# fasion-image-generator-project/discogan_modernized

Measured on AMD Instinct MI355X. Metric: images/sec per DiscoGAN train step, higher is better.
Workload: dtype f32x3; 1 GPU; tops2hanbok discogan image_size=512 batch_size=32 per GPU (BASELINE configs[3]); D,G,G cycle, fwd+bwd+Adam, dead backward work skipped; fp32-accurate conv products on the bf16 matrix path: every fp32 operand carried as three bf16 planes (24 significand bits), exact bf16 x bf16 products, fp32 accumulation (no operand rounding); image_size=512, global_batch=32, parallelism=dp1, hipgraph=True, hip_streams=2, allreduce_overlap=False

## Files before the change

discogan_modernized_amd/_lib.py:

```python
from __future__ import annotations

import ctypes as C
import os

_HERE = os.path.dirname(os.path.abspath(__file__))
LIB_PATH = os.environ.get("DG_LIB") or os.path.join(_HERE, "libdiscogan_hip.so")

_p = C.c_void_p
_i = C.c_int
_f = C.c_float
_d = C.c_double
_z = C.c_size_t
_l = C.c_int64

SIGNATURES = {
    "dg_version": (_i, []),
    "dg_build_flags": (_i, []),
    "dg_last_error": (C.c_char_p, []),
    "dg_set_option": (_i, [C.c_char_p, _i]),
    "dg_conv_workspace_bytes": (_z, [_i, _i, _i, _i, _i, _i, _i, _i]),
    "dg_conv_fwd": (_i, [_p, _p, _p, _i, _i, _i, _i, _i, _i, _i, _p, _z, _p]),
    "dg_conv_dgrad": (_i, [_p, _p, _p, _i, _i, _i, _i, _i, _i, _i, _p, _z, _p]),
    "dg_conv_wgrad": (_i, [_p, _p, _p, _i, _i, _i, _i, _i, _i, _i, _i, _p, _z, _p]),
    "dg_conv_workspace_bytes_p": (_z, [_i, _i, _i, _i, _i, _i, _i, _i, _i, _i]),
    "dg_conv_bnstats_rows_p": (_i, [_i, _i, _i, _i, _i, _i, _i, _i, _i]),
    "dg_conv_plan_splits_p": (_i, [_i, _i, _i, _i, _i, _i, _i, _i, _i, _i]),
    "dg_conv_plan_describe": (_i, [_i, _i, _i, _i, _i, _i, _i, _i, _i, _i, _i, _i, C.POINTER(_i), _i]),
    "dg_conv_fwd_g": (_i, [_i, _p, _p, _p, _i, _i, _i, _i, _i, _i, _i, _i, _i, _p, _z, _p, _z, _p]),
    "dg_conv_dgrad_g": (_i, [_i, _p, _p, _p, _i, _i, _i, _i, _i, _i, _i, _i, _i, _p, _z, _p, _z, _p]),
    "dg_conv_wgrad_g": (_i, [_i, _i, _p, _p, _p, _i, _i, _i, _i, _i, _i, _i, _i, _i, _i, _p, _z, _p]),
    "dg_conv4x4s2_c3_fwd_p": (_i, [_p, _p, _p, _i, _i, _i, _i, _i, _i, _f, _i, _p]),
    "dg_conv4x4s2_c3_dgrad_p": (_i, [_p, _i, _p, _p, _i, _i, _i, _i, _i, _i, _p, _z, _p]),
    "dg_c3_dgrad_act_ok": (_i, [_i, _i, _i, _i, _i]),
    "dg_conv4x4s2_c3_dgrad_act_p": (_i, [_p, _i, _p, _i, _f, _p, _p, _i, _i, _i, _i, _i, _i, _p, _z, _p]),
    "dg_conv4x4s2_c3_wgrad_p": (_i, [_p, _p, _i, _i, _f, _p, _p, _i, _i, _i, _i, _i, _i, _p, _z, _p]),
    "dg_c3_dgrad_bn_ok": (_i, [_i, _i, _i, _i, _i]),
    "dg_conv4x4s2_c3_dgrad_bn_p": (_i, [_p, _p, _p, _p, _i, _p, _p, _i, _i, _i, _i, _i, _i, _p]),
    "dg_c3_wgrad_bn_ok": (_i, [_i, _i, _i, _i, _i]),
    "dg_conv4x4s2_c3_wgrad_bn_p": (_i, [_p, _p, _p, _p, _i, _p, _p, _i, _i, _i, _i, _i, _i, _p, _z, _p]),
    "dg_conv4x4s2_c3_fwd_g": (_i, [_i, _p, _p, _p, _i, _i, _i, _i, _i, _f, _i, _p]),
    "dg_conv4x4s2_c3_dgrad_g": (_i, [_i, _p, _p, _p, _i, _i, _i, _i, _i, _i, _p]),
    "dg_conv4x4s2_c3_wgrad_g": (_i, [_i, _i, _p, _p, _i, _f, _p, _p, _i, _i, _i, _i, _i, _i, _p, _z, _p]),
    "dg_bn_train_stats_g": (_i, [_i, _i, _p, _i, _i, _f, _f, _p, _p, _p, _p, _p, _z, _p]),
    "dg_bn_act_fwd_g": (_i, [_i, _p, _p, _i, _i, _p, _p, _p, _i, _f, _p]),
    "dg_bn_act_bwd_g": (_i, [_i, _i, _p, _p, _p, _i, _i, _p, _p, _p, _i, _f, _p, _p, _i, _p, _z, _p]),
    "dg_act_fwd_g": (_i, [_i, _p, _p, _z, _i, _f, _p]),
    "dg_act_bwd_g": (_i, [_i, _p, _p, _p, _z, _i, _f, _p]),
    "dg_mse_fwd_g": (_i, [_i, _p, _p, _z, _p, _p, _z, _p]),
    "dg_mse_bwd_g": (_i, [_i, _p, _p, _z, _p, _p, _p]),
    "dg_bce_fwd_g": (_i, [_i, _p, _i, _p, _p, _p]),
    "dg_bce_bwd_g": (_i, [_i, _p, _i, _p, _p, _p, _p]),
    "dg_fm_fwd_g": (_i, [_i, _p, _p, _i, _z, _p, _p, _p, _z, _p]),
    "dg_fm_bwd_g": (_i, [_i, _p, _i, _z, _p, _p, _p, _p]),
    "dg_conv_fwd_bias_act": (_i, [_p, _p, _p, _p, _i, _i, _i, _i, _i, _i, _i, _i, _f, _p, _z, _p]),
    "dg_conv_dgrad_bias_act": (_i, [_p, _p, _p, _p, _i, _i, _i, _i, _i, _i, _i, _i, _f, _p, _z, _p]),
    "dg_conv_plan_splits": (_i, [_i, _i, _i, _i, _i, _i, _i, _i]),
    "dg_conv_bnstats_rows": (_i, [_i, _i, _i, _i, _i, _i, _i, _i]),
    "dg_conv_fwd_bnstats": (_i, [_p, _p, _p, _i, _i, _i, _i, _i, _p, _z, _p, _z, _p]),
    "dg_conv_dgrad_bnstats": (_i, [_p, _p, _p, _i, _i, _i, _i, _i, _p, _z, _p, _z, _p]),
    "dg_conv4x4s2_fwd": (_i, [_p, _p, _p, _i, _i, _i, _i, _i, _p, _z, _p]),
    "dg_conv4x4s2_dgrad": (_i, [_p, _p, _p, _i, _i, _i, _i, _i, _p, _z, _p]),
    "dg_conv4x4s2_wgrad": (_i, [_p, _p, _p, _i, _i, _i, _i, _i, _i, _p, _z, _p]),
    "dg_conv4x4_valid_fwd": (_i, [_p, _p, _p, _i, _i, _i, _p, _z, _p]),
    "dg_conv4x4_valid_dgrad": (_i, [_p, _p, _p, _i, _i, _i, _p, _z, _p]),
    "dg_conv4x4_valid_wgrad": (_i, [_p, _p, _p, _i, _i, _i, _i, _p, _z, _p]),
    "dg_convT4x4s2_fwd": (_i, [_p, _p, _p, _i, _i, _i, _i, _i, _p, _z, _p]),
    "dg_convT4x4s2_dgrad": (_i, [_p, _p, _p, _i, _i, _i, _i, _i, _p, _z, _p]),
    "dg_convT4x4s2_wgrad": (_i, [_p, _p, _p, _i, _i, _i, _i, _i, _i, _p, _z, _p]),
    "dg_convT4x4_1to4_fwd": (_i, [_p, _p, _p, _i, _i, _i, _p, _z, _p]),
    "dg_convT4x4_1to4_dgrad": (_i, [_p, _p, _p, _i, _i, _i, _p, _z, _p]),
    "dg_convT4x4_1to4_wgrad": (_i, [_p, _p, _p, _i, _i, _i, _i, _p, _z, _p]),
    "dg_conv4x4s2_c3_fwd": (_i, [_p, _p, _p, _i, _i, _i, _i, _i, _f, _p]),
    "dg_c3_dgrad_workspace_bytes": (_z, [_i]),
    "dg_conv4x4s2_c3_dgrad": (_i, [_p, _p, _p, _i, _i, _i, _i, _i, _p, _z, _p]),
    "dg_c3_wgrad_workspace_bytes": (_z, [_i, _i, _i, _i]),
    "dg_conv4x4s2_c3_wgrad": (_i, [_p, _p, _p, _i, _i, _i, _i, _i, _p, _z, _p]),
    "dg_conv4x4s2_c3_wgrad_act": (_i, [_p, _p, _i, _f, _p, _p, _i, _i, _i, _i, _i, _p, _z, _p]),
    "dg_bn_workspace_bytes": (_z, [_i, _i]),
    "dg_bn_train_stats": (_i, [_p, _i, _i, _f, _f, _p, _p, _p, _p, _p, _z, _p]),
    "dg_bn_partials_workspace_bytes": (_z, [_i, _i]),
    "dg_bn_stats_from_partials": (_i, [_p, _i, _i, _i, _f, _f, _p, _p, _p, _p, _p, _z, _p]),
    "dg_bn_act_fwd": (_i, [_p, _p, _i, _i, _p, _p, _p, _i, _f, _p]),
    "dg_bn_act_bwd": (_i, [_p, _p, _p, _i, _i, _p, _p, _p, _i, _f, _p, _p, _i, _p, _z, _p]),
    "dg_act_fwd": (_i, [_p, _p, _z, _i, _f, _p]),
    "dg_act_bwd": (_i, [_p, _p, _p, _z, _i, _f, _p]),
    "dg_loss_workspace_bytes": (_z, []),
    "dg_mse_fwd": (_i, [_p, _p, _z, _p, _p, _z, _p]),
    "dg_mse_bwd": (_i, [_p, _p, _z, _p, _p, _p]),
    "dg_bce_fwd": (_i, [_p, _i, _f, _p, _p, _z, _p]),
    "dg_bce_bwd": (_i, [_p, _i, _f, _p, _p, _p]),
    "dg_fm_workspace_bytes": (_z, [_i, _z]),
    "dg_fm_fwd": (_i, [_p, _p, _i, _z, _p, _p, _p, _z, _p]),
    "dg_fm_bwd": (_i, [_p, _i, _z, _p, _p, _p, _p]),
    "dg_debug_igemm_stamps": (_i, [_p, _z]),
    "dg_device_cu_count": (_i, []),
    "dg_loss_mix_fwd": (_i, [_p, _p, _i, _f, _i, _p]),
    "dg_loss_mix_bwd": (_i, [_p, _p, _i, _f, _i, _i, _p]),
    "dg_adam_advance": (_i, [_p, _d, _d, _d, _p]),
    "dg_adam_step_flat": (_i, [_p, _p, _p, _p, _z, _p, _f, _f, _f, _f, _f, _p]),
    "dg_ema_update_flat": (_i, [_p, _p, _z, _f, _p]),
    "dg_swap_flat": (_i, [_p, _p, _z, _p]),
    "dg_grad_stats_workspace_bytes": (_z, []),
    "dg_grad_sumsq_partial": (_i, [_p, _z, _p, _z, _i, C.POINTER(_i), _p]),
    "dg_grad_clip_finalize": (_i, [_p, _i, _d, _d, _i, _p, _p]),
    "dg_adam_advance_c": (_i, [_p, _d, _d, _d, _p, _p]),
    "dg_adam_step_flat_c": (_i, [_p, _p, _p, _p, _z, _p, _f, _f, _f, _f, _p, _p, _i, _z, _p]),
    "dg_bce_target_fwd": (_i, [_p, _p, _i, _p, _p]),
    "dg_bce_target_bwd": (_i, [_p, _p, _i, _p, _p, _p]),
    "dg_hinge_fwd": (_i, [_p, _p, _z, _f, _p, _p, _z, _p]),
    "dg_hinge_bwd": (_i, [_p, _p, _z, _f, _p, _p, _p]),
    "dg_dp_ready": (_i, [_p]),
    "dg_dp_unique_id_bytes": (_i, []),
    "dg_dp_get_unique_id": (_i, [_p, _z]),
    "dg_dp_init": (_i, [_i, _i, _p, _z]),
    "dg_dp_world_size": (_i, []),
    "dg_dp_rank": (_i, []),
    "dg_dp_allreduce_sum": (_i, [_p, _z, _p]),
    "dg_dp_allreduce_max": (_i, [_p, _z, _p]),
    "dg_dp_broadcast": (_i, [_p, _z, _i, _p]),
    "dg_dp_barrier": (_i, [_p, _p]),
    "dg_dp_destroy": (_i, []),
    "dg_u8hwc_to_f32chw": (_i, [_p, _p, _i, _i, _i, _i, _p]),
    "dg_image_prep": (_i, [_p, _p, _i, _i, _i, _i, _i, _i, _i, _i, _p]),
    "dg_sample_grid_u8": (_i, [_p, _i, _i, _i, _i, _i, _p, _p]),
    "dg_image_metrics_workspace_bytes": (_z, [_i, _i]),
    "dg_image_metrics": (_i, [_p, _p, _i, _i, _p, _p, _z, _p]),
    "dg_adam_step_flat_bf16": (_i, [_p, _p, _p, _p, _z, _p, _f, _f, _f, _f, _f, _p, _p]),
    "dg_f32_to_bf16": (_i, [_p, _p, _z, _p]),
    "dg_bn_act_fwd_bf16": (_i, [_p, _p, _p, _i, _i, _p, _p, _p, _i, _f, _p]),
    "dg_bn_act_bwd_bf16": (_i, [_p, _p, _p, _p, _i, _i, _p, _p, _p, _i, _f, _p, _p, _i, _p, _z, _p]),
    "dg_conv_bf16_operands_ok": (_i, [_i, _i, _i, _i, _i, _i, _i, _i]),
    "dg_f32_to_bf16x3": (_i, [_p, _p, _z, _z, _p]),
    "dg_adam_step_flat_x3": (_i, [_p, _p, _p, _p, _z, _p, _f, _f, _f, _f, _f, _p, _z, _p]),
    "dg_conv4x4s2_c3_fwd_x3": (_i, [_p, _p, _p, _p, _z, _i, _i, _i, _i, _i, _f, _p]),
    "dg_conv_x3_planes_ok": (_i, [_i, _i, _i, _i, _i, _i, _i, _i]),
    "dg_bn_act_fwd_x3": (_i, [_p, _p, _p, _z, _i, _i, _i, _p, _p, _p, _i, _f, _p]),
    "dg_bn_act_bwd_x3": (_i, [_p, _p, _p, _p, _z, _i, _i, _i, _p, _p, _p, _i, _f, _p, _p, _i, _p, _z, _p]),
    "dg_conv_x3_bnstats_rows": (_i, [_i, _i, _i, _i, _i, _i, _i, _i]),
    "dg_conv_fwd_x3": (_i, [_p, _l, _p, _l, _i, _p, _i, _i, _i, _i, _i, _i, _i, _p, _z, _p, _z, _p]),
    "dg_x3_transpose_planes": (_i, [_p, _p, _z, _p, _p, _p, _i, _p]),
    "dg_conv_dgrad_x3": (_i, [_p, _l, _i, _p, _l, _p, _i, _i, _i, _i, _i, _i, _i, _p, _z, _p, _z, _p]),
    "dg_conv_wgrad_x3": (_i, [_p, _l, _i, _p, _l, _p, _i, _i, _i, _i, _i, _i, _i, _i, _p, _z, _p]),
    "dg_conv_mixed_bnstats_rows": (_i, [_i, _i, _i, _i, _i, _i, _i, _i, _i, _i]),
    "dg_conv_fwd_mixed": (_i, [_p, _i, _p, _i, _p, _i, _i, _i, _i, _i, _i, _i, _i, _p, _z, _p, _z, _p]),
    "dg_conv_dgrad_mixed": (_i, [_p, _i, _p, _i, _p, _i, _i, _i, _i, _i, _i, _i, _i, _p, _z, _p, _z, _p]),
    "dg_bn_train_stats_t": (_i, [_p, _i, _i, _i, _f, _f, _p, _p, _p, _p, _p, _z, _p]),
    "dg_bn_act_fwd_t": (_i, [_p, _p, _i, _i, _i, _p, _p, _p, _i, _f, _p]),
    "dg_bn_act_bwd_t": (_i, [_p, _p, _p, _i, _i, _i, _p, _p, _p, _i, _f, _p, _p, _i, _p, _z, _p]),
    "dg_act_bwd_t": (_i, [_p, _p, _p, _i, _z, _i, _f, _p]),
    "dg_conv4x4s2_c3_fwd_t": (_i, [_p, _p, _p, _i, _i, _i, _i, _i, _i, _f, _p]),
    "dg_conv4x4s2_c3_dgrad_t": (_i, [_p, _i, _p, _p, _i, _i, _i, _i, _i, _p, _z, _p]),
    "dg_conv4x4s2_c3_wgrad_t": (_i, [_p, _p, _i, _i, _f, _p, _p, _i, _i, _i, _i, _i, _p, _z, _p]),
    "dg_fm_fwd_t": (_i, [_p, _p, _i, _i, _z, _p, _p, _p, _z, _p]),
    "dg_fm_bwd_t": (_i, [_p, _i, _z, _p, _p, _p, _i, _p]),
    "dg_conv_wgrad_mixed": (_i, [_p, _i, _p, _i, _p, _i, _i, _i, _i, _i, _i, _i, _i, _p, _z, _p]),
    "dg_nchw_to_nhwc": (_i, [_p, _p, _i, _i, _i, _i, _p]),
    "dg_nhwc_to_nchw": (_i, [_p, _p, _i, _i, _i, _i, _p]),
}

_lib = None


class DiscoganHipError(RuntimeError):
    pass


def load():
    global _lib
    if _lib is not None:
        return _lib
    if not os.path.exists(LIB_PATH):
        raise DiscoganHipError(
            f"{LIB_PATH} not found: the HIP kernel library is not built. "
            "Run `python -m discogan_modernized_amd.build` (hipcc --offload-arch=gfx950). "
            "There is no CPU fallback for the product path.")
    import torch
    lib = C.CDLL(LIB_PATH)
    for name, (res, args) in SIGNATURES.items():
        fn = getattr(lib, name)
        fn.restype = res
        fn.argtypes = args
    _lib = lib
    for key, val in os.environ.items():
        if key.startswith("DG_OPT_"):
            rc = lib.dg_set_option(key[7:].lower().encode(), int(val))
            if rc != 0:
                raise DiscoganHipError(f"bad option {key}: " + lib.dg_last_error().decode())
    return lib


def check(rc, what=""):
    if rc != 0:
        msg = load().dg_last_error().decode("utf-8", "replace")
        raise DiscoganHipError(f"{what} failed (code {rc}): {msg}")


def set_option(name: str, value: int):
    check(load().dg_set_option(name.encode(), int(value)), "dg_set_option")
```

discogan_modernized_amd/csrc/igemm_dma_x3.hip:

```cpp
#include "igemm_args.h"
#include <type_traits>
#include <utility>

typedef __bf16 bf16x8 __attribute__((ext_vector_type(8)));
typedef __bf16 bf16x4 __attribute__((ext_vector_type(4)));
typedef __attribute__((address_space(3))) bf16x4* lds_bf4_ptr;
typedef __attribute__((address_space(3))) void* lds_void_ptr;

template <int... Q, typename F>
__device__ __forceinline__ void dg_x3_static_for(std::integer_sequence<int, Q...>, F&& f) {
    (f(std::integral_constant<int, Q>{}), ...);
}
#define DG_X3T_MAX 48
constexpr int G16_I[24] = {0, 0, 0, 1, 1, 1, 2, 2, 2, 3, 3, 3, 4, 4, 4, 5, 5, 5, 6, 7, 6, 6, 7, 7};
constexpr int G16_T[24] = {0, 1, 2, 0, 1, 2, 0, 1, 2, 0, 1, 2, 0, 1, 2, 0, 1, 2, 0, 0, 1, 2, 1, 2};

template <int MODE, bool BT, int WM, int WN, int NS, bool M16 = false>
__global__ __launch_bounds__(64 * WM * WN, 2) void igemm_dma_x3_kernel(const IgemmArgs p) {
    static_assert(MODE == MODE_FWD || MODE == MODE_DGRAD_S2 || MODE == MODE_WGRAD, "modes with an LDS-DMA form");
    static_assert(!BT || MODE == MODE_FWD, "the transposed weight copy serves the forward form");
    constexpr int NW = WM * WN, FM = 4, FN = 2;
    constexpr int BM = 32 * FM * WM, BN = 32 * FN * WN, KT = 16;
    static_assert((BM == 256 || BM == 128) && (BN == 256 || BN == 128), "tile");
    constexpr bool A_KM = MODE == MODE_WGRAD;
    constexpr bool B_KM = MODE != MODE_FWD || BT;
    constexpr int PLA = BM * KT * 2, PLB = BN * KT * 2;
    constexpr int OPA = 3 * PLA, STAGE = OPA + 3 * PLB;
    constexpr int NPA = PLA / 1024 / NW, NPB = PLB / 1024 / NW;
    static_assert(NPA * NW * 1024 == PLA && NPB * NW * 1024 == PLB, "pieces must divide over the waves");
    constexpr int NPC = 3 * (NPA + NPB);
    constexpr int LDS_BYTES = NS * STAGE;
    static_assert((NS == 2 || NS == 3) && LDS_BYTES <= 160 * 1024, "LDS");
    static_assert(!M16 || (NS == 3 && WM == 2 && WN == 4), "the 16x16x32 body: 256 x 256 tile, three stages");
    constexpr int EPI_BYTES = NW * 32 * 68 * 4;
    static_assert(EPI_BYTES <= LDS_BYTES, "epilogue transpose regions live in the operand stages");
    __shared__ __attribute__((aligned(1024))) char smem[LDS_BYTES];

    const int tid = threadIdx.x;
    const int lane = tid & 63;
    const int wave = __builtin_amdgcn_readfirstlane(tid >> 6);
    long long* const stp = (p.stamps != nullptr && tid == 0) ? p.stamps + (long)blockIdx.x * 8 : nullptr;
    if (stp) {
        stp[0] = wall_clock64();
        stp[1] = clock64();
        unsigned hwid, xcc;
        asm volatile("s_getreg_b32 %0, hwreg(HW_REG_HW_ID)" : "=s"(hwid));
        asm volatile("s_getreg_b32 %0, hwreg(HW_REG_XCC_ID)" : "=s"(xcc));
        stp[6] = ((long long)xcc << 32) | hwid;
    }
    const int wm = wave / WN, wn = wave % WN;
    const int l31 = lane & 31, lh = lane >> 5;

    int bid = blockIdx.x;
    int tn, tm, parity = 0, split;
    if (p.xcd_group == 2) {
        const int G = p.tilesM;
        tm = (bid >> 3) % G;
        int rest = (bid / (8 * G)) * 8 + (bid & 7);
        if (MODE == MODE_DGRAD_S2) {
            parity = rest & 3;
            rest >>= 2;
        }
        tn = rest % p.tilesN;
        split = rest / p.tilesN;
    } else if (p.xcd_group) {
        const int G = p.tilesN * (MODE == MODE_DGRAD_S2 ? 4 : 1);
        int inner = (bid >> 3) % G;
        int rest = (bid / (8 * G)) * 8 + (bid & 7);
        if (MODE == MODE_DGRAD_S2) {
            parity = inner & 3;
            inner >>= 2;
        }
        tn = inner;
        tm = rest % p.tilesM;
        split = rest / p.tilesM;
    } else {
        tn = bid % p.tilesN;
        bid /= p.tilesN;
        tm = bid % p.tilesM;
        bid /= p.tilesM;
        split = bid;
        if (MODE == MODE_DGRAD_S2) {
            parity = bid & 3;
            split = bid >> 2;
        }
    }
    const int ph = parity >> 1, pw = parity & 1;
    const int m0 = tm * BM, n0 = tn * BN;
    const int it_begin = split * p.itPerSplit;
    const int it_end = min(p.nIt, it_begin + p.itPerSplit);

    const int H = p.H, W = p.W, Cc = p.Cc, K = p.K, Ho = p.Ho, Wo = p.Wo;
    const int lgWo = p.lgWo, lgHW = p.lgWo + p.lgHo;

    constexpr int OOR = (int)0x80000000;
    __amdgpu_buffer_rsrc_t rA[3], rB[3];
#pragma unroll
    for (int pl = 0; pl < 3; ++pl) {
        rA[pl] = __builtin_amdgcn_make_buffer_rsrc((void*)((const char*)p.A + pl * p.a_plane), 0, (p.dbg_zero & 1) ? 0 : (int)p.abytes, 0x00020000);
        rB[pl] = __builtin_amdgcn_make_buffer_rsrc((void*)((const char*)p.B + pl * p.b_plane), 0, (p.dbg_zero & 2) ? 0 : (int)p.bbytes, 0x00020000);
    }

    auto kmswz = [](int k) -> int { return M16 ? (((k & 3) << 2) | (((k >> 3) & 1) << 1)) : ((k & 3) << 2); };
    int a_ob[NPA], a_inv[NPA];
#pragma unroll
    for (int i = 0; i < NPA; ++i) {
        const int pq = wave * NPA + i;
        a_ob[i] = 0;
        a_inv[i] = 0;
        if (!A_KM) {
            const int row = pq * 32 + (lane >> 1);
            const int g = (lane & 1) ^ (M16 ? 0 : ((row >> 3) & 1));
            const int m = m0 + row;
            if (MODE == MODE_FWD) {
                a_inv[i] = 0xFFFF;
                if (m < p.M) {
                    const int ox = m & (Wo - 1), oy = (m >> lgWo) & (Ho - 1), n = m >> lgHW;
                    const int ay = oy * p.stride - p.pad, ax = ox * p.stride - p.pad;
                    a_ob[i] = (((n * H + ay) * W + ax) * Cc + g * 8) * 2;
#ifdef DG_TIMING_KNOBS
                    if (p.dbg_zero & 16) a_ob[i] = (m * 16 + g * 8) * 2;
#endif
                    int colok = 0, okmask = 0;
#pragma unroll
                    for (int sx = 0; sx < 4; ++sx) colok |= ((unsigned)(ax + sx) < (unsigned)W) ? (1 << sx) : 0;
#pragma unroll
                    for (int r = 0; r < 4; ++r) okmask |= ((unsigned)(ay + r) < (unsigned)H) ? (colok << (4 * r)) : 0;
                    a_inv[i] = ~okmask & 0xFFFF;
                }
            } else {
                a_inv[i] = 0xF;
                if (m < p.M) {
                    const int bx = m & (Wo - 1), ay = (m >> lgWo) & (Ho - 1);
                    a_ob[i] = (m * K + g * 8) * 2;
                    a_inv[i] = 0;
#pragma unroll
                    for (int t = 0; t < 4; ++t) {
                        const int ty = t >> 1, tx = t & 1;
                        const int dyo = ph == 0 ? (ty == 0 ? 0 : -1) : (ty == 0 ? 0 : 1);
                        const int dxo = pw == 0 ? (tx == 0 ? 0 : -1) : (tx == 0 ? 0 : 1);
                        const bool ok = (unsigned)(ay + dyo) < (unsigned)Ho && (unsigned)(bx + dxo) < (unsigned)Wo;
                        a_inv[i] |= ok ? 0 : (1 << t);
                    }
                }
            }
        } else {
            constexpr int GR = BM / 8, RP = 64 / GR;
            const int krow = pq * RP + lane / GR;
            const int gc = (lane % GR) ^ kmswz(krow);
            const int col = m0 + gc * 8;
            a_ob[i] = col < K ? (p.a_cm ? (((krow >> 2) * (K >> 4) + (col >> 4)) * 64 + (krow & 3) * 16 + (col & 15)) * 2 : (krow * K + col) * 2) : OOR;
        }
    }
    int b_ob[NPB];
    int wg_c[NPB], wg_cst[NPB], wg_ybad[NPB], wg_xbad[NPB], wg_colbad[NPB], wg_krow[NPB];
    const bool wg_s2 = p.stride == 2;
    const int wg_lpm = wg_s2 ? 2 : 4, wg_pxm = wg_s2 ? -1 : 0;
#pragma unroll
    for (int i = 0; i < NPB; ++i) {
        const int pq = wave * NPB + i;
        b_ob[i] = 0;
        wg_c[i] = wg_cst[i] = wg_colbad[i] = wg_krow[i] = 0;
        wg_ybad[i] = wg_xbad[i] = -1;
        if (MODE == MODE_FWD && !BT) {
            const int row = pq * 32 + (lane >> 1);
            const int g = (lane & 1) ^ (M16 ? 0 : ((row >> 3) & 1));
// ... 284 lines not shown
        });
    }
    asm volatile("s_waitcnt vmcnt(0) lgkmcnt(0)" ::: "memory");
    __builtin_amdgcn_s_barrier();
    if (stp) stp[3] = clock64();

    if ((MODE == MODE_FWD || MODE == MODE_DGRAD_S2) && p.stat != nullptr && p.part == nullptr) {
        const int row0 = m0 + wm * (32 * FM);
        const int nrows = min(32 * FM, p.M - row0);
        const int prow = ((MODE == MODE_DGRAD_S2 ? parity : 0) * p.tilesM + tm) * WM + wm;
        float* srow = p.stat + (long)prow * p.stat_rs;
        if (wn == 0 && tn == 0 && lane == 0) srow[0] = (float)max(nrows, 0);
        if constexpr (M16) {
            if (nrows > 0) {
#pragma unroll
                for (int bj = 0; bj < BNB; ++bj) {
                    const float sh = __shfl(acc16[0][bj][0], l15, 64);
                    float ssum = 0.f, ssq = 0.f;
#pragma unroll
                    for (int bi = 0; bi < AM; ++bi)
#pragma unroll
                        for (int e = 0; e < 4; ++e) {
                            const int lr = bi * 16 + 4 * l4 + e;
                            if (lr < nrows) {
                                const float d = acc16[bi][bj][e] - sh;
                                ssum += d;
                                ssq += d * d;
                            }
                        }
                    ssum += __shfl_xor(ssum, 16, 64);
                    ssq += __shfl_xor(ssq, 16, 64);
                    ssum += __shfl_xor(ssum, 32, 64);
                    ssq += __shfl_xor(ssq, 32, 64);
                    const int n = n0 + wn * (32 * FN) + bj * 16 + l15;
                    if (l4 == 0 && n < p.Ng) {
                        srow[4 + n] = sh;
                        srow[4 + p.Ng + n] = ssum;
                        srow[4 + 2 * p.Ng + n] = ssq;
                    }
                }
            }
        } else
        if (nrows > 0) {
#pragma unroll
            for (int jn = 0; jn < FN; ++jn) {
                const float sh = __shfl(acc[0][jn][0], l31, 64);
                float ssum = 0.f, ssq = 0.f;
#pragma unroll
                for (int i = 0; i < FM; ++i)
#pragma unroll
                    for (int r = 0; r < 16; ++r) {
                        const int lr = i * 32 + (r & 3) + 8 * (r >> 2) + 4 * lh;
                        if (lr < nrows) {
                            const float d = acc[i][jn][r] - sh;
                            ssum += d;
                            ssq += d * d;
                        }
                    }
                ssum += __shfl_xor(ssum, 32, 64);
                ssq += __shfl_xor(ssq, 32, 64);
                const int n = n0 + wn * (32 * FN) + jn * 32 + l31;
                if (lh == 0 && n < p.Ng) {
                    srow[4 + n] = sh;
                    srow[4 + p.Ng + n] = ssum;
                    srow[4 + 2 * p.Ng + n] = ssq;
                }
            }
        }
    }

    const bool to_part = p.part != nullptr;
    float* const eps = (float*)smem + wave * (32 * 68);
    const int erow = lane >> 4, ec4 = (lane & 15) * 4;
    const int ncol = n0 + wn * (32 * FN) + ec4;
#pragma unroll
    for (int i = 0; i < FM; ++i) {
        if constexpr (M16) {
#pragma unroll
            for (int bi = 0; bi < 2; ++bi)
#pragma unroll
                for (int bj = 0; bj < BNB; ++bj)
#pragma unroll
                    for (int e = 0; e < 4; ++e) eps[(bi * 16 + 4 * l4 + e) * 68 + bj * 16 + l15] = acc16[2 * i + bi][bj][e];
        } else {
#pragma unroll
            for (int r = 0; r < 16; ++r) {
                const int lr = (r & 3) + 8 * (r >> 2) + 4 * lh;
                eps[lr * 68 + l31] = acc[i][0][r];
                eps[lr * 68 + 32 + l31] = acc[i][1][r];
            }
        }
#pragma unroll
        for (int t = 0; t < 8; ++t) {
            const int row = t * 4 + erow;
            f32x4 v = *(const f32x4*)(eps + row * 68 + ec4);
            const int m = m0 + wm * (32 * FM) + i * 32 + row;
            if (m >= p.M || ncol >= p.Ng) continue;
            float* dst;
            long eoff;
            if (to_part) {
                const long srow = (MODE == MODE_DGRAD_S2) ? ((long)split * 4 + parity) * p.M + m : (long)split * p.M + m;
                dst = p.part;
                eoff = srow * p.Ng + ncol;
            } else if (MODE == MODE_DGRAD_S2) {
                const int b = m & (Wo - 1), a = (m >> lgWo) & (Ho - 1), n = m >> lgHW;
                dst = p.C;
                eoff = (long)((n * H + 2 * a + ph) * W + 2 * b + pw) * Cc + ncol;
            } else {
                dst = p.C;
                eoff = (long)m * p.Ng + ncol;
            }
            if (!to_part && p.accumulate) v += *(const f32x4*)(dst + eoff);
            *(f32x4*)(dst + eoff) = v;
        }
    }
    if (stp) {
        stp[4] = clock64();
        asm volatile("s_waitcnt vmcnt(0)" ::: "memory");
        stp[5] = wall_clock64();
        stp[7] = clock64();
    }
}

template <int WM, int WN, int NS, bool M16>
static int x3_launch_tile(int mode, const IgemmArgs& a, int grid, hipStream_t st) {
    const dim3 blk(64 * WM * WN);
    switch (mode) {
        case MODE_FWD:
            if (a.b_transposed) hipLaunchKernelGGL((igemm_dma_x3_kernel<MODE_FWD, true, WM, WN, NS, M16>), dim3(grid), blk, 0, st, a);
            else hipLaunchKernelGGL((igemm_dma_x3_kernel<MODE_FWD, false, WM, WN, NS, M16>), dim3(grid), blk, 0, st, a);
            return 1;
        case MODE_DGRAD_S2: hipLaunchKernelGGL((igemm_dma_x3_kernel<MODE_DGRAD_S2, false, WM, WN, NS, M16>), dim3(grid), blk, 0, st, a); return 1;
        case MODE_WGRAD: hipLaunchKernelGGL((igemm_dma_x3_kernel<MODE_WGRAD, false, WM, WN, NS, M16>), dim3(grid), blk, 0, st, a); return 1;
        default: return 0;
    }
}
int dg_igemm_dma_x3_launch(int mode, int wm, int wn, const IgemmArgs& a, int zmul, hipStream_t st) {
    const int grid = a.tilesM * a.tilesN * zmul * a.splits;
#ifdef DG_EXPERIMENTS
    const int body = dg_get_option(DG_OPT_X3_MFMA) == 16 ? 16 : 32;
    if (wm == 2 && wn == 4 && body == 16) return x3_launch_tile<2, 4, 3, true>(mode, a, grid, st);
#endif
    if (wm == 2 && wn == 4) return x3_launch_tile<2, 4, 2, false>(mode, a, grid, st);
#ifdef DG_TIMING_KNOBS
    if (wm == 2 && wn == 2 && mode == MODE_FWD) return x3_launch_tile<2, 2, 2, false>(mode, a, grid, st);
#endif
    if (wm == 1 && wn == 4 && mode == MODE_WGRAD) {
        hipLaunchKernelGGL((igemm_dma_x3_kernel<MODE_WGRAD, false, 1, 4, 2>), dim3(grid), dim3(256), 0, st, a);
        return 1;
    }
    return 0;
}

struct X3TransposeTable {
    int n;
    int tile0[DG_X3T_MAX + 1];
    int K[DG_X3T_MAX], J[DG_X3T_MAX];
    long off[DG_X3T_MAX];
};
__global__ __launch_bounds__(256) void x3_transpose_kernel(const __bf16* __restrict__ src, __bf16* __restrict__ dst, long plane, X3TransposeTable t) {
    __shared__ unsigned tile[64][33];
    typedef unsigned u32x4 __attribute__((ext_vector_type(4)));
    int wi = 0;
    while (wi + 1 < t.n && (int)blockIdx.x >= t.tile0[wi + 1]) ++wi;
    const int K = t.K[wi], J = t.J[wi];
    const int tj = (J + 63) / 64;
    const int b = blockIdx.x - t.tile0[wi];
    const int k0 = (b / tj) * 64, j0 = (b % tj) * 64;
    const bool vec = (K % 8 == 0) && (J % 8 == 0) && (t.off[wi] % 8 == 0);
    const int lk = threadIdx.x >> 2, lv = threadIdx.x & 3;
    const int sq = threadIdx.x & 7, sjp = threadIdx.x >> 3;
    for (int pl = 0; pl < 3; ++pl) {
        const unsigned short* s = (const unsigned short*)src + pl * plane + t.off[wi];
        unsigned short* d = (unsigned short*)dst + pl * plane + t.off[wi];
#pragma unroll
        for (int h = 0; h < 2; ++h) {
            const int k = k0 + lk, j = j0 + (lv + 4 * h) * 8;
            u32x4 v = (u32x4){0u, 0u, 0u, 0u};
            if (k < K) {
                if (vec && j < J) v = *(const u32x4*)(s + (long)k * J + j);
                else if (!vec) {
#pragma unroll
                    for (int e = 0; e < 8; ++e)
                        if (j + e < J) v[e >> 1] |= (unsigned)s[(long)k * J + j + e] << (16 * (e & 1));
                }
            }
#pragma unroll
            for (int e = 0; e < 4; ++e) tile[lk][(lv + 4 * h) * 4 + e] = v[e];
        }
        __syncthreads();
        unsigned w[8];
#pragma unroll
        for (int e = 0; e < 8; ++e) w[e] = tile[8 * sq + e][sjp];
        u32x4 lo, hi;
#pragma unroll
        for (int e = 0; e < 4; ++e) {
            lo[e] = (w[2 * e] & 0xffffu) | (w[2 * e + 1] << 16);
            hi[e] = (w[2 * e] >> 16) | (w[2 * e + 1] & 0xffff0000u);
        }
        const int j = j0 + 2 * sjp, k = k0 + 8 * sq;
        if (vec) {
            if (k < K && j < J) {
                *(u32x4*)(d + (long)j * K + k) = lo;
                *(u32x4*)(d + (long)(j + 1) * K + k) = hi;
            }
        } else {
#pragma unroll
            for (int e = 0; e < 8; ++e) {
                if (k + e < K && j < J) d[(long)j * K + k + e] = (unsigned short)(lo[e >> 1] >> (16 * (e & 1)));
                if (k + e < K && j + 1 < J) d[(long)(j + 1) * K + k + e] = (unsigned short)(hi[e >> 1] >> (16 * (e & 1)));
            }
        }
        __syncthreads();
    }
}
extern "C" int dg_x3_transpose_planes(const void* src_planes, void* dst_planes, size_t plane_elems, const int64_t* w_off,
                                      const int* w_K, const int* w_J, int n, dg_stream_t stream) {
    DG_CHECK_ARG(src_planes && dst_planes && w_off && w_K && w_J, "dg_x3_transpose_planes: null pointer");
    DG_CHECK_ARG(n >= 0, "dg_x3_transpose_planes: n=%d", n);
    for (int i0 = 0; i0 < n; i0 += DG_X3T_MAX) {
        X3TransposeTable t;
        t.n = n - i0 < DG_X3T_MAX ? n - i0 : DG_X3T_MAX;
        int tiles = 0;
        for (int i = 0; i < t.n; ++i) {
            const int K = w_K[i0 + i], J = w_J[i0 + i];
            DG_CHECK_ARG(K >= 1 && J >= 1 && w_off[i0 + i] >= 0 && (size_t)(w_off[i0 + i] + (long)K * J) <= plane_elems,
                         "dg_x3_transpose_planes: weight %d (K=%d, J=%d, offset %ld) outside the plane", i0 + i, K, J, (long)w_off[i0 + i]);
            t.tile0[i] = tiles;
            t.K[i] = K; t.J[i] = J; t.off[i] = w_off[i0 + i];
            tiles += ((K + 63) / 64) * ((J + 63) / 64);
        }
        t.tile0[t.n] = tiles;
        if (tiles == 0) continue;
        hipLaunchKernelGGL(x3_transpose_kernel, dim3(tiles), dim3(256), 0, (hipStream_t)stream, (const __bf16*)src_planes,
                           (__bf16*)dst_planes, (long)plane_elems, t);
        DG_CHECK_LAUNCH("x3_transpose");
    }
    return DG_OK;
}
```

discogan_modernized_amd/csrc/optim.hip:

```cpp
#include "dg_common.h"

__global__ void adam_advance_kernel(double* state, double lr, double b1, double b2, const double* ctl) {
    if (ctl != nullptr && ctl[3] != 0.0) return;
    const double t = state[0] + 1.0;
    state[0] = t;
    state[1] = lr / (1.0 - pow(b1, t));
    state[2] = sqrt(1.0 - pow(b2, t));
}

typedef __bf16 bf16x4_t __attribute__((ext_vector_type(4)));
__device__ __forceinline__ void adam_one(float& p, float g, float& m, float& v, float gscale, float wd, float omb1, float b2, float omb2,
                                         float bc2_sqrt, float eps, float step_size) {
#pragma clang fp contract(off)
    const float gr = g * gscale + wd * p;
    m = m + (gr - m) * omb1;
    v = v * b2 + omb2 * gr * gr;
    const float denom = sqrtf(v) / bc2_sqrt + eps;
    p = p - step_size * (m / denom);
}
template <int P16>
__global__ __launch_bounds__(256) void adam_step_kernel(float* __restrict__ p, const float* __restrict__ g,
                                                        float* __restrict__ m, float* __restrict__ v, long n,
                                                        const double* __restrict__ state, float b1, float b2, float eps,
                                                        float wd, float gscale, __bf16* __restrict__ p16, long pstride,
                                                        const double* __restrict__ ctl) {
    if (ctl != nullptr) {
        if (ctl[3] != 0.0) return;
        gscale = (float)ctl[2];
    }
    const float step_size = (float)state[1];
    const float bc2_sqrt = (float)state[2];
    const float omb1 = 1.f - b1, omb2 = 1.f - b2;
    const long n4 = n >> 2;
    long i0 = (long)blockIdx.x * 256 + threadIdx.x;
    if constexpr (P16 == 3) {
        typedef __bf16 bf16x8_a __attribute__((ext_vector_type(8)));
        const long n8 = (((size_t)p16 | (size_t)(pstride * 2)) & 15) == 0 ? n >> 3 : 0;
        for (long i = i0; i < n8; i += (long)gridDim.x * 256) {
            f32x4 pp[2], gg[2], mm[2], vv[2];
#pragma unroll
            for (int h = 0; h < 2; ++h) {
                pp[h] = *(const f32x4*)(p + i * 8 + 4 * h);
                gg[h] = *(const f32x4*)(g + i * 8 + 4 * h);
                mm[h] = *(const f32x4*)(m + i * 8 + 4 * h);
                vv[h] = *(const f32x4*)(v + i * 8 + 4 * h);
            }
            dg_bf16x4_t hh[2], md[2], ll[2];
#pragma unroll
            for (int h = 0; h < 2; ++h) {
#pragma unroll
                for (int j = 0; j < 4; ++j) {
                    float a = pp[h][j], b = mm[h][j], c = vv[h][j];
                    adam_one(a, gg[h][j], b, c, gscale, wd, omb1, b2, omb2, bc2_sqrt, eps, step_size);
                    pp[h][j] = a; mm[h][j] = b; vv[h][j] = c;
                }
                *(f32x4*)(p + i * 8 + 4 * h) = pp[h];
                *(f32x4*)(m + i * 8 + 4 * h) = mm[h];
                *(f32x4*)(v + i * 8 + 4 * h) = vv[h];
                dg_split3(pp[h], hh[h], md[h], ll[h]);
            }
            *(bf16x8_a*)(p16 + i * 8) = __builtin_shufflevector(hh[0], hh[1], 0, 1, 2, 3, 4, 5, 6, 7);
            *(bf16x8_a*)(p16 + pstride + i * 8) = __builtin_shufflevector(md[0], md[1], 0, 1, 2, 3, 4, 5, 6, 7);
            *(bf16x8_a*)(p16 + 2 * pstride + i * 8) = __builtin_shufflevector(ll[0], ll[1], 0, 1, 2, 3, 4, 5, 6, 7);
        }
        i0 += n8 * 2;
    }
    for (long i = i0; i < n4; i += (long)gridDim.x * 256) {
        f32x4 pp = *(const f32x4*)(p + i * 4);
        const f32x4 gg = *(const f32x4*)(g + i * 4);
        f32x4 mm = *(const f32x4*)(m + i * 4);
        f32x4 vv = *(const f32x4*)(v + i * 4);
#pragma unroll
        for (int j = 0; j < 4; ++j) {
            float a = pp[j], b = mm[j], c = vv[j];
            adam_one(a, gg[j], b, c, gscale, wd, omb1, b2, omb2, bc2_sqrt, eps, step_size);
            pp[j] = a; mm[j] = b; vv[j] = c;
        }
        *(f32x4*)(p + i * 4) = pp;
        *(f32x4*)(m + i * 4) = mm;
        *(f32x4*)(v + i * 4) = vv;
        if (P16 == 1) *(bf16x4_t*)(p16 + i * 4) = __builtin_convertvector(pp, bf16x4_t);
        if (P16 == 3) {
            dg_bf16x4_t h, md, l;
            dg_split3(pp, h, md, l);
            *(dg_bf16x4_t*)(p16 + i * 4) = h;
            *(dg_bf16x4_t*)(p16 + pstride + i * 4) = md;
            *(dg_bf16x4_t*)(p16 + 2 * pstride + i * 4) = l;
        }
    }
    if (blockIdx.x == 0 && threadIdx.x == 0) {
        for (long e = n4 * 4; e < n; ++e) {
            float a = p[e], b = m[e], c = v[e];
            adam_one(a, g[e], b, c, gscale, wd, omb1, b2, omb2, bc2_sqrt, eps, step_size);
            p[e] = a; m[e] = b; v[e] = c;
            if (P16 == 1) p16[e] = (__bf16)p[e];
            if (P16 == 3) {
                const __bf16 h = (__bf16)p[e];
                const float r = p[e] - (float)h;
                const __bf16 md = (__bf16)r;
                p16[e] = h;
                p16[pstride + e] = md;
                p16[2 * pstride + e] = (__bf16)(r - (float)md);
            }
        }
    }
}

extern "C" int dg_adam_advance(double* state, double lr, double beta1, double beta2, dg_stream_t stream) {
    DG_CHECK_ARG(state, "dg_adam_advance: null state");
    hipLaunchKernelGGL(adam_advance_kernel, dim3(1), dim3(1), 0, (hipStream_t)stream, state, lr, beta1, beta2, (const double*)nullptr);
    DG_CHECK_LAUNCH("adam_advance");
    return DG_OK;
}
extern "C" int dg_adam_step_flat(float* p, const float* g, float* m, float* v, size_t n, const double* state, float beta1,
                                 float beta2, float eps, float weight_decay, float grad_scale, dg_stream_t stream) {
    DG_CHECK_ARG(p && g && m && v && state, "dg_adam_step_flat: null pointer");
    if (n == 0) return DG_OK;
    long grid = ((long)(n / 4) + 255) / 256;
    if (grid > 4096) grid = 4096;
    if (grid < 1) grid = 1;
    hipLaunchKernelGGL(adam_step_kernel<0>, dim3((int)grid), dim3(256), 0, (hipStream_t)stream, p, g, m, v, (long)n, state,
                       beta1, beta2, eps, weight_decay, grad_scale, (__bf16*)nullptr, 0L, (const double*)nullptr);
    DG_CHECK_LAUNCH("adam_step");
    return DG_OK;
}
extern "C" int dg_adam_step_flat_bf16(float* p, const float* g, float* m, float* v, size_t n, const double* state, float beta1,
                                      float beta2, float eps, float weight_decay, float grad_scale, void* p16, dg_stream_t stream) {
    DG_CHECK_ARG(p && g && m && v && state && p16, "dg_adam_step_flat_bf16: null pointer");
    if (n == 0) return DG_OK;
    long grid = ((long)(n / 4) + 255) / 256;
    if (grid > 4096) grid = 4096;
    if (grid < 1) grid = 1;
    hipLaunchKernelGGL(adam_step_kernel<1>, dim3((int)grid), dim3(256), 0, (hipStream_t)stream, p, g, m, v, (long)n, state,
                       beta1, beta2, eps, weight_decay, grad_scale, (__bf16*)p16, 0L, (const double*)nullptr);
    DG_CHECK_LAUNCH("adam_step_bf16");
    return DG_OK;
}
extern "C" int dg_adam_step_flat_x3(float* p, const float* g, float* m, float* v, size_t n, const double* state, float beta1,
                                    float beta2, float eps, float weight_decay, float grad_scale, void* p3, size_t plane_elems,
                                    dg_stream_t stream) {
    DG_CHECK_ARG(p && g && m && v && state && p3, "dg_adam_step_flat_x3: null pointer");
    DG_CHECK_ARG(plane_elems >= n && plane_elems % 8 == 0, "dg_adam_step_flat_x3: plane distance %zu for %zu parameters", plane_elems, n);
    if (n == 0) return DG_OK;
    long grid = ((long)(n / 4) + 255) / 256;
    if (grid > 4096) grid = 4096;
    if (grid < 1) grid = 1;
    hipLaunchKernelGGL(adam_step_kernel<3>, dim3((int)grid), dim3(256), 0, (hipStream_t)stream, p, g, m, v, (long)n, state,
                       beta1, beta2, eps, weight_decay, grad_scale, (__bf16*)p3, (long)plane_elems, (const double*)nullptr);
    DG_CHECK_LAUNCH("adam_step_x3");
    return DG_OK;
}
__global__ __launch_bounds__(256) void f32_to_bf16_kernel(const float* __restrict__ x, __bf16* __restrict__ y, long n) {
    const long n4 = n >> 2;
    for (long i = (long)blockIdx.x * 256 + threadIdx.x; i < n4; i += (long)gridDim.x * 256)
        *(bf16x4_t*)(y + i * 4) = __builtin_convertvector(*(const f32x4*)(x + i * 4), bf16x4_t);
    if (blockIdx.x == 0 && threadIdx.x == 0)
        for (long e = n4 * 4; e < n; ++e) y[e] = (__bf16)x[e];
}
extern "C" int dg_f32_to_bf16(const float* x, void* y, size_t n, dg_stream_t stream) {
    DG_CHECK_ARG(x && y, "dg_f32_to_bf16: null pointer");
    if (n == 0) return DG_OK;
    long grid = ((long)(n / 4) + 255) / 256;
    if (grid > 4096) grid = 4096;
    if (grid < 1) grid = 1;
    hipLaunchKernelGGL(f32_to_bf16_kernel, dim3((int)grid), dim3(256), 0, (hipStream_t)stream, x, (__bf16*)y, (long)n);
    DG_CHECK_LAUNCH("f32_to_bf16");
    return DG_OK;
}
__global__ __launch_bounds__(256) void f32_to_bf16x3_kernel(const float* __restrict__ x, __bf16* __restrict__ y, long n, long pstride) {
    const long n4 = n >> 2;
    for (long i = (long)blockIdx.x * 256 + threadIdx.x; i < n4; i += (long)gridDim.x * 256) {
        dg_bf16x4_t h, md, l;
        dg_split3(*(const f32x4*)(x + i * 4), h, md, l);
        *(dg_bf16x4_t*)(y + i * 4) = h;
        *(dg_bf16x4_t*)(y + pstride + i * 4) = md;
        *(dg_bf16x4_t*)(y + 2 * pstride + i * 4) = l;
    }
    if (blockIdx.x == 0 && threadIdx.x == 0)
        for (long e = n4 * 4; e < n; ++e) {
            const __bf16 h = (__bf16)x[e];
            const float r = x[e] - (float)h;
            const __bf16 md = (__bf16)r;
            y[e] = h;
            y[pstride + e] = md;
            y[2 * pstride + e] = (__bf16)(r - (float)md);
        }
}
extern "C" int dg_f32_to_bf16x3(const float* x, void* y3, size_t n, size_t plane_elems, dg_stream_t stream) {
    DG_CHECK_ARG(x && y3, "dg_f32_to_bf16x3: null pointer");
    DG_CHECK_ARG(plane_elems >= n && plane_elems % 8 == 0, "dg_f32_to_bf16x3: plane distance %zu for %zu elements", plane_elems, n);
    if (n == 0) return DG_OK;
    long grid = ((long)(n / 4) + 255) / 256;
    if (grid > 8192) grid = 8192;
    if (grid < 1) grid = 1;
    hipLaunchKernelGGL(f32_to_bf16x3_kernel, dim3((int)grid), dim3(256), 0, (hipStream_t)stream, x, (__bf16*)y3, (long)n, (long)plane_elems);
    DG_CHECK_LAUNCH("f32_to_bf16x3");
    return DG_OK;
}

__device__ __forceinline__ float ema_one(float e, float p, float w) {
#pragma clang fp contract(off)
    const float d = p - e;
    const float s = d * w;
    return e + s;
}
__global__ __launch_bounds__(256) void ema_update_kernel(float* __restrict__ ema, const float* __restrict__ p, long n, float w) {
    const long n4 = n >> 2;
    for (long i = (long)blockIdx.x * 256 + threadIdx.x; i < n4; i += (long)gridDim.x * 256) {
        f32x4 ee = *(const f32x4*)(ema + i * 4);
        const f32x4 pp = *(const f32x4*)(p + i * 4);
#pragma unroll
        for (int j = 0; j < 4; ++j) ee[j] = ema_one(ee[j], pp[j], w);
        *(f32x4*)(ema + i * 4) = ee;
    }
    if (blockIdx.x == 0 && threadIdx.x == 0)
        for (long e = n4 * 4; e < n; ++e) ema[e] = ema_one(ema[e], p[e], w);
}
typedef unsigned int u32x4 __attribute__((ext_vector_type(4)));
__global__ __launch_bounds__(256) void swap_flat_kernel(unsigned int* __restrict__ a, unsigned int* __restrict__ b, long n) {
    const long n4 = n >> 2;
    for (long i = (long)blockIdx.x * 256 + threadIdx.x; i < n4; i += (long)gridDim.x * 256) {
        const u32x4 x = *(const u32x4*)(a + i * 4);
        const u32x4 y = *(const u32x4*)(b + i * 4);
        *(u32x4*)(a + i * 4) = y;
        *(u32x4*)(b + i * 4) = x;
    }
    if (blockIdx.x == 0 && threadIdx.x == 0)
        for (long e = n4 * 4; e < n; ++e) {
            const unsigned int x = a[e];
            a[e] = b[e];
            b[e] = x;
        }
}
static inline int flat_grid(size_t n) {
    size_t grid = (n / 4 + 255) / 256;
    if (grid > 4096) grid = 4096;
    if (grid < 1) grid = 1;
    return (int)grid;
}
extern "C" int dg_ema_update_flat(float* ema, const float* p, size_t n, float w, dg_stream_t stream) {
    DG_CHECK_ARG(ema && p, "dg_ema_update_flat: null pointer");
    DG_CHECK_ARG((((size_t)ema | (size_t)p) & 15) == 0, "dg_ema_update_flat: pointers must be 16-byte aligned (ema %p, p %p)", (void*)ema,
                 (const void*)p);
    DG_CHECK_ARG(w >= 0.f && w <= 1.f, "dg_ema_update_flat: weight %g outside [0, 1]", (double)w);
    if (n == 0) return DG_OK;
    hipLaunchKernelGGL(ema_update_kernel, dim3(flat_grid(n)), dim3(256), 0, (hipStream_t)stream, ema, p, (long)n, w);
    DG_CHECK_LAUNCH("ema_update");
    return DG_OK;
}
extern "C" int dg_swap_flat(float* a, float* b, size_t n, dg_stream_t stream) {
    DG_CHECK_ARG(a && b, "dg_swap_flat: null pointer");
    DG_CHECK_ARG((((size_t)a | (size_t)b) & 15) == 0, "dg_swap_flat: pointers must be 16-byte aligned (a %p, b %p)", (void*)a, (void*)b);
    if (n == 0 || a == b) return DG_OK;
    const size_t lo = (size_t)a < (size_t)b ? (size_t)a : (size_t)b, hi = (size_t)a < (size_t)b ? (size_t)b : (size_t)a;
    DG_CHECK_ARG((hi - lo) / sizeof(float) >= n, "dg_swap_flat: the two ranges of %zu floats overlap", n);
    hipLaunchKernelGGL(swap_flat_kernel, dim3(flat_grid(n)), dim3(256), 0, (hipStream_t)stream, (unsigned int*)a, (unsigned int*)b, (long)n);
    DG_CHECK_LAUNCH("swap_flat");
    return DG_OK;
}

#define DG_GRAD_STATS_SLOTS 16384
static_assert(DG_GRAD_STATS_SLOTS >= 4096, "one full-grid range must fit");

__device__ __forceinline__ void sumsq4(double (&a)[4], const f32x4& x) {
#pragma unroll
    for (int j = 0; j < 4; ++j) a[j] += (double)x[j] * (double)x[j];
}
__global__ __launch_bounds__(256) void grad_sumsq_partial_kernel(const float* __restrict__ g, long n, double* __restrict__ ws) {
    __shared__ double red[4];
    const long n4 = n >> 2;
    const long stride = (long)gridDim.x * 256;
    double a[4] = {0.0, 0.0, 0.0, 0.0};
    long i = (long)blockIdx.x * 256 + threadIdx.x;
    for (; i + 3 * stride < n4; i += 4 * stride) {
        const f32x4 x0 = *(const f32x4*)(g + i * 4);
        const f32x4 x1 = *(const f32x4*)(g + (i + stride) * 4);
        const f32x4 x2 = *(const f32x4*)(g + (i + 2 * stride) * 4);
        const f32x4 x3 = *(const f32x4*)(g + (i + 3 * stride) * 4);
        sumsq4(a, x0);
        sumsq4(a, x1);
        sumsq4(a, x2);
        sumsq4(a, x3);
    }
    for (; i < n4; i += stride) sumsq4(a, *(const f32x4*)(g + i * 4));
    double s = (a[0] + a[1]) + (a[2] + a[3]);
    if (blockIdx.x == 0 && threadIdx.x == 0)
        for (long e = n4 * 4; e < n; ++e) s += (double)g[e] * (double)g[e];
    s = dg_wave_sum_d(s);
    if ((threadIdx.x & 63) == 0) red[threadIdx.x >> 6] = s;
    __syncthreads();
    if (threadIdx.x == 0) ws[blockIdx.x] = (red[0] + red[1]) + (red[2] + red[3]);
}
__global__ __launch_bounds__(256) void grad_clip_finalize_kernel(const double* __restrict__ ws, int slots, double pre_scale,
                                                                 double max_norm, int guard, double* __restrict__ ctl) {
    __shared__ double red[4];
    double s = 0.0;
    for (int i = threadIdx.x; i < slots; i += 256) s += ws[i];
    s = dg_wave_sum_d(s);
    if ((threadIdx.x & 63) == 0) red[threadIdx.x >> 6] = s;
    __syncthreads();
    if (threadIdx.x != 0) return;
    const double sumsq = (red[0] + red[1]) + (red[2] + red[3]);
    const double norm = sqrt(sumsq) * pre_scale;
    double scale = pre_scale;
    bool clipped = false;
    if (max_norm > 0.0) {
        const double coef = max_norm / (norm + 1e-6);
        if (!(coef >= 1.0)) {
            scale = pre_scale * coef;
            clipped = coef < 1.0;
        }
    }
    const bool finite = (sumsq - sumsq) == 0.0;
    const bool skip = guard != 0 && !finite;
    ctl[0] = sumsq;
    ctl[1] = norm;
    ctl[2] = scale;
    ctl[3] = skip ? 1.0 : 0.0;
    ctl[4] += 1.0;
    if (clipped && !skip) ctl[5] += 1.0;
    if (skip) ctl[6] += 1.0;
    if ((norm - norm) == 0.0 && norm > ctl[7]) ctl[7] = norm;
}

extern "C" size_t dg_grad_stats_workspace_bytes(void) { return (size_t)DG_GRAD_STATS_SLOTS * sizeof(double); }
extern "C" int dg_grad_sumsq_partial(const float* g, size_t n, double* ws, size_t ws_bytes, int slot0, int* slots_used, dg_stream_t stream) {
    DG_CHECK_ARG(slots_used, "dg_grad_sumsq_partial: null slots_used");
    *slots_used = 0;
    if (n == 0) return DG_OK;
    DG_CHECK_ARG(g && ws, "dg_grad_sumsq_partial: null pointer");
    DG_CHECK_ARG(((size_t)g & 15) == 0, "dg_grad_sumsq_partial: the gradient must be 16-byte aligned (%p)", (const void*)g);
    DG_CHECK_ARG(((size_t)ws & 7) == 0, "dg_grad_sumsq_partial: the workspace must be 8-byte aligned (%p)", (void*)ws);
    DG_CHECK_ARG(slot0 >= 0, "dg_grad_sumsq_partial: first slot %d", slot0);
    const int grid = flat_grid(n);
    DG_CHECK_ARG(((size_t)slot0 + (size_t)grid) * sizeof(double) <= ws_bytes,
                 "dg_grad_sumsq_partial: workspace of %zu bytes too small for slots %d..%ld (dg_grad_stats_workspace_bytes)", ws_bytes, slot0,
                 (long)slot0 + grid - 1);
    hipLaunchKernelGGL(grad_sumsq_partial_kernel, dim3(grid), dim3(256), 0, (hipStream_t)stream, g, (long)n, ws + slot0);
    DG_CHECK_LAUNCH("grad_sumsq_partial");
    *slots_used = grid;
    return DG_OK;
}
extern "C" int dg_grad_clip_finalize(const double* ws, int slots, double pre_scale, double max_norm, int guard, double* ctl,
                                     dg_stream_t stream) {
    DG_CHECK_ARG(ctl, "dg_grad_clip_finalize: null ctl");
    DG_CHECK_ARG(slots >= 0 && slots <= DG_GRAD_STATS_SLOTS && (slots == 0 || ws), "dg_grad_clip_finalize: %d slots (workspace %p)", slots,
                 (const void*)ws);
    DG_CHECK_ARG(pre_scale == pre_scale && max_norm == max_norm, "dg_grad_clip_finalize: NaN pre_scale or max_norm");
    hipLaunchKernelGGL(grad_clip_finalize_kernel, dim3(1), dim3(256), 0, (hipStream_t)stream, ws, slots, pre_scale, max_norm, guard, ctl);
    DG_CHECK_LAUNCH("grad_clip_finalize");
    return DG_OK;
}
extern "C" int dg_adam_advance_c(double* state, double lr, double beta1, double beta2, const double* ctl, dg_stream_t stream) {
    DG_CHECK_ARG(state && ctl, "dg_adam_advance_c: null pointer");
    hipLaunchKernelGGL(adam_advance_kernel, dim3(1), dim3(1), 0, (hipStream_t)stream, state, lr, beta1, beta2, ctl);
    DG_CHECK_LAUNCH("adam_advance_c");
    return DG_OK;
}
extern "C" int dg_adam_step_flat_c(float* p, const float* g, float* m, float* v, size_t n, const double* state, float beta1, float beta2,
                                   float eps, float weight_decay, const double* ctl, void* out, int form, size_t plane_elems,
                                   dg_stream_t stream) {
    DG_CHECK_ARG(p && g && m && v && state && ctl, "dg_adam_step_flat_c: null pointer");
    DG_CHECK_ARG(form == 0 || form == 1 || form == 3, "dg_adam_step_flat_c: form %d (0 plain, 1 bf16 shadow, 3 planes)", form);
    DG_CHECK_ARG(form == 0 || out, "dg_adam_step_flat_c: form %d without an output", form);
    DG_CHECK_ARG(form != 3 || (plane_elems >= n && plane_elems % 8 == 0), "dg_adam_step_flat_c: plane distance %zu for %zu parameters",
                 plane_elems, n);
    if (n == 0) return DG_OK;
    const dim3 grid(flat_grid(n)), block(256);
    const hipStream_t s = (hipStream_t)stream;
    if (form == 0)
        hipLaunchKernelGGL(adam_step_kernel<0>, grid, block, 0, s, p, g, m, v, (long)n, state, beta1, beta2, eps, weight_decay, 1.f,
                           (__bf16*)nullptr, 0L, ctl);
    else if (form == 1)
        hipLaunchKernelGGL(adam_step_kernel<1>, grid, block, 0, s, p, g, m, v, (long)n, state, beta1, beta2, eps, weight_decay, 1.f,
                           (__bf16*)out, 0L, ctl);
    else
        hipLaunchKernelGGL(adam_step_kernel<3>, grid, block, 0, s, p, g, m, v, (long)n, state, beta1, beta2, eps, weight_decay, 1.f,
                           (__bf16*)out, (long)plane_elems, ctl);
    DG_CHECK_LAUNCH("adam_step_c");
    return DG_OK;
}
```

discogan_modernized_amd/functional.py:

```python
from __future__ import annotations

import functools

import torch
from torch.autograd import Function

from . import ops


def _fwd(f):
    @functools.wraps(f)
    def w(ctx, *a, **k):
        ctx.dgc = ops.current()
        return f(ctx, *a, **k)
    return staticmethod(w)


def _bwd(f):
    @functools.wraps(f)
    def w(ctx, *g):
        with ops.use(ctx.dgc):
            return f(ctx, *g)
    return staticmethod(w)


FUSE_C3_DGRAD_ACT = __import__("os").environ.get("DG_FUSE_C3_DGRAD_ACT", "1") != "0"


def _flat_grad_of(param):
    fg = getattr(param, "_dg_flat_grad", None)
    if fg is not None and param.grad is fg:
        return fg
    return None


FINAL_PASS = False
FINAL_HOOK = None


def _final(ctx_flag, *params):
    if ctx_flag and FINAL_HOOK is not None:
        for p in params:
            FINAL_HOOK(p)


def _release_unless_wgrad(ctx, x):
    if not ctx.needs_input_grad[1]:
        ops.derived_release(x)


def _release_after_backward(dy, x):
    ops.derived_release(dy, x)


def _conv_forward(ctx, transposed, x, w, stride, pad, want_stats):
    x = ops.as_nhwc(x)
    ctx.save_for_backward(x, w)
    ctx.sp = (stride, pad)
    ctx.wref = w
    ctx.final = FINAL_PASS
    if transposed:
        hw = ((x.shape[2] - 1) * stride - 2 * pad + 4, (x.shape[3] - 1) * stride - 2 * pad + 4)
        y = ops.conv_dgrad(x, w, hw, stride, pad, want_stats=want_stats)
    else:
        y = ops.conv_fwd(x, w, stride, pad, want_stats=want_stats)
    _release_unless_wgrad(ctx, x)
    if not want_stats:
        return y
    y, stat = y
    if stat is None:
        stat = torch.empty(0, device=y.device)
    ctx.mark_non_differentiable(stat)
    ctx.set_materialize_grads(False)
    return y, stat


def _conv_backward(ctx, transposed, dy):
    if dy is None:
        return None, None, None, None, None
    x, _ = ctx.saved_tensors
    w = ctx.wref
    stride, pad = ctx.sp
    dy = ops.as_nhwc(dy)
    dx = None
    if ctx.needs_input_grad[0]:
        dx = ops.conv_fwd(dy, w, stride, pad) if transposed else ops.conv_dgrad(dy, w, (x.shape[2], x.shape[3]), stride, pad)
    wg = (x, dy) if transposed else (dy, x)
    dw = None
    if ctx.needs_input_grad[1]:
        fg = _flat_grad_of(w)
        if fg is not None:
            ops.conv_wgrad(*wg, stride, pad, out=fg, accumulate=True)
            _final(ctx.final, w)
        else:
            dw = ops.conv_wgrad(*wg, stride, pad)
    _release_after_backward(dy, x)
    return dx, dw, None, None, None


class ConvFn(Function):

    @_fwd
    def forward(ctx, x, w, stride, pad, want_stats=False):
        return _conv_forward(ctx, False, x, w, stride, pad, want_stats)

    @_bwd
    def backward(ctx, dy, dstat=None):
        return _conv_backward(ctx, False, dy)


class ConvTransposeFn(Function):

    @_fwd
    def forward(ctx, x, w, stride, pad, want_stats=False):
        return _conv_forward(ctx, True, x, w, stride, pad, want_stats)

    @_bwd
    def backward(ctx, dy, dstat=None):
        return _conv_backward(ctx, True, dy)


class ConvC3Fn(Function):

    @_fwd
    def forward(ctx, x, w, act, slope, want_planes=False):
        y = ops.c3_fwd(x, w, act, slope, want_planes=want_planes)
        ctx.save_for_backward(x, w, y)
        ctx.act = (act, slope)
        ctx.wref = w
        ctx.final = FINAL_PASS
        return y

    @_bwd
    def backward(ctx, dy):
        x, w, y = ctx.saved_tensors
        act, slope = ctx.act
        fused_dgrad = FUSE_C3_DGRAD_ACT and act == ops.ACT_LEAKY and ops.c3_dgrad_act_ok(w.shape[0], x.shape[0], x.shape[2], x.shape[3],
                                                                                          dy.dtype == torch.bfloat16)
        if act == ops.ACT_NONE or (ctx.needs_input_grad[0] and not fused_dgrad):
            g = ops.act_bwd(dy, y, act, slope) if act != ops.ACT_NONE else ops.as_nhwc(dy)
            fuse = {}
        else:
            g = ops.as_nhwc(dy)
            fuse = dict(act_out=y, act=act, slope=slope)
        dx = None
        if ctx.needs_input_grad[0]:
            dx = ops.c3_dgrad(g, w, ops.ACT_NONE, act_out=y, in_act=act, slope=slope) if fuse else ops.c3_dgrad(g, w, ops.ACT_NONE)
        dw = None
        if ctx.needs_input_grad[1]:
            fg = _flat_grad_of(ctx.wref)
            if fg is not None and fg.is_contiguous():
                ops.c3_wgrad(g, x, out=fg, accumulate=True, **fuse)
                _final(ctx.final, ctx.wref)
            else:
                dw = ops.c3_wgrad(g, x, **fuse)
        return dx, dw, None, None, None


class ConvTransposeC3Fn(Function):

    @_fwd
    def forward(ctx, x, w, act):
        x = ops.as_nhwc(x)
        out = ops.c3_dgrad(x, w, act)
        ctx.save_for_backward(x, w, out)
        ctx.act = act
        ctx.wref = w
        ctx.final = FINAL_PASS
        return out

    @_bwd
    def backward(ctx, dout):
        x, w, out = ctx.saved_tensors
        g = ops.act_bwd(dout, out, ctx.act) if ctx.act != ops.ACT_NONE else dout.contiguous()
        dx = ops.c3_fwd(g, w, ops.ACT_NONE) if ctx.needs_input_grad[0] else None
        dw = None
        if ctx.needs_input_grad[1]:
            fg = _flat_grad_of(ctx.wref)
            if fg is not None and fg.is_contiguous():
                ops.c3_wgrad(x, g, out=fg, accumulate=True)
                _final(ctx.final, ctx.wref)
            else:
                dw = ops.c3_wgrad(x, g)
        return dx, dw, None


def _bn_saved(y, partials, running_mean, running_var, nbt, training, eps, momentum):
    if training and partials is not None and partials.numel() > 0:
        return ops.bn_stats_from_partials(partials, y, running_mean, running_var, nbt, eps, momentum)
    if training:
        return ops.bn_train_stats(y, running_mean, running_var, nbt, eps, momentum)
    return torch.stack([running_mean, torch.rsqrt(running_var + eps)])


class BatchNormActFn(Function):

    @_fwd
    def forward(ctx, y, gamma, beta, running_mean, running_var, nbt, training, eps, momentum, act, slope,
                partials=None, z_cm=False, dy_cm=False, z_po=False, dy_po=False):
        y = ops.as_nhwc(y)
        saved = _bn_saved(y, partials, running_mean, running_var, nbt, training, eps, momentum)
        z = ops.bn_act_fwd(y, saved, gamma, beta, act, slope, planes_cm=z_cm, planes_only=z_po and training)
        ctx.save_for_backward(y, saved, gamma, beta)
        ctx.cfg = (act, slope, training)
        ctx.dy_cm = bool(dy_cm)
        ctx.dy_po = bool(dy_po)
        ctx.prefs = (gamma, beta)
        ctx.final = FINAL_PASS
        return z

    @_bwd
    def backward(ctx, dz):
        y, saved, gamma, beta = ctx.saved_tensors
        act, slope, training = ctx.cfg
        if not training:
            raise RuntimeError("BatchNormActFn: backward in eval mode is not supported")
        need_p = ctx.needs_input_grad[1] or ctx.needs_input_grad[2]
        fg, fb = _flat_grad_of(ctx.prefs[0]), _flat_grad_of(ctx.prefs[1])
        if need_p and fg is not None and fb is not None:
            dy, _, _ = ops.bn_act_bwd(dz, y, saved, gamma, beta, act, slope, out_grads=(fg, fb), planes_cm=ctx.dy_cm, planes_only=ctx.dy_po)
            _final(ctx.final, ctx.prefs[0], ctx.prefs[1])
            return (dy,) + (None,) * 15
        dy, dgamma, dbeta = ops.bn_act_bwd(dz, y, saved, gamma, beta, act, slope, need_param_grads=need_p, planes_cm=ctx.dy_cm,
                                           planes_only=ctx.dy_po)
        return (dy, dgamma if ctx.needs_input_grad[1] else None, dbeta if ctx.needs_input_grad[2] else None,
                None, None, None, None, None, None, None, None, None, None, None, None, None)


class BatchNormActConvTransposeC3Fn(Function):

    @_fwd
    def forward(ctx, y, gamma, beta, running_mean, running_var, nbt, training, eps, momentum, bn_act, partials, w, act, dy_cm=False, dy_po=False):
        y = ops.as_nhwc(y)
        saved = _bn_saved(y, partials, running_mean, running_var, nbt, training, eps, momentum)
        out = ops.c3_dgrad_bn(y, saved, gamma, beta, w, act, bn_act)
        ctx.save_for_backward(y, saved, gamma, beta, w, out)
        ctx.cfg = (bn_act, act, training, bool(dy_cm), bool(dy_po))
        ctx.prefs = (gamma, beta)
        ctx.wref = w
        ctx.final = FINAL_PASS
        return out

    @_bwd
    def backward(ctx, dout):
        y, saved, gamma, beta, w, out = ctx.saved_tensors
        bn_act, act, training, dy_cm, dy_po = ctx.cfg
        if not training:
            raise RuntimeError("BatchNormActConvTransposeC3Fn: backward in eval mode is not supported")
        none = (None,) * 15
        g = ops.act_bwd(dout, out, act) if act != ops.ACT_NONE else dout.contiguous()
        need_p = ctx.needs_input_grad[1] or ctx.needs_input_grad[2]
        dz = ops.c3_fwd(g, w, ops.ACT_NONE) if ctx.needs_input_grad[0] or need_p else None
        dw = None
        if ctx.needs_input_grad[11]:
            fg = _flat_grad_of(ctx.wref)
            if fg is not None and fg.is_contiguous():
                ops.c3_wgrad_bn(y, saved, gamma, beta, g, out=fg, accumulate=True, bn_act=bn_act)
                _final(ctx.final, ctx.wref)
            else:
                dw = ops.c3_wgrad_bn(y, saved, gamma, beta, g, bn_act=bn_act)
        if dz is None:
            return none[:11] + (dw,) + none[12:]
        fgm, fb = _flat_grad_of(ctx.prefs[0]), _flat_grad_of(ctx.prefs[1])
        if need_p and fgm is not None and fb is not None:
            dy, _, _ = ops.bn_act_bwd(dz, y, saved, gamma, beta, bn_act, 0.0, out_grads=(fgm, fb), planes_cm=dy_cm, planes_only=dy_po)
            _final(ctx.final, ctx.prefs[0], ctx.prefs[1])
            return (dy,) + none[1:11] + (dw,) + none[12:]
        dy, dgamma, dbeta = ops.bn_act_bwd(dz, y, saved, gamma, beta, bn_act, 0.0, need_param_grads=need_p, planes_cm=dy_cm, planes_only=dy_po)
        return (dy, dgamma if ctx.needs_input_grad[1] else None, dbeta if ctx.needs_input_grad[2] else None) + none[3:11] + (dw,) + none[12:]


class ActFn(Function):

    @_fwd
    def forward(ctx, x, act, slope):
        out = ops.act_fwd(x, act, slope)
        ctx.save_for_backward(out)
        ctx.cfg = (act, slope)
        return out

    @_bwd
    def backward(ctx, dy):
        (out,) = ctx.saved_tensors
        act, slope = ctx.cfg
        return ops.act_bwd(dy, out, act, slope), None, None


class MSELossFn(Function):
    @_fwd
    def forward(ctx, x, t, out=None):
        loss, xd, td = ops.mse_fwd(x, t, out)
        ctx.save_for_backward(xd, td)
        ctx.in_strides = x.stride()
        return loss

    @_bwd
    def backward(ctx, gout):
        xd, td = ctx.saved_tensors
        gout = gout.contiguous()
        dx = ops.mse_bwd(xd, td, gout) if ctx.needs_input_grad[0] else None
        dt = None
        if ctx.needs_input_grad[1]:
            dt = ops.mse_bwd(td, xd, gout)
        return dx, dt, None


class BCELossFn(Function):

    @_fwd
    def forward(ctx, p, label, out=None):
        shape = p.shape
        loss, pc = ops.bce_fwd(p.reshape(-1), label, out)
        ctx.save_for_backward(pc)
        ctx.cfg = (label, shape)
        return loss

    @_bwd
    def backward(ctx, gout):
        (pc,) = ctx.saved_tensors
        label, shape = ctx.cfg
        return ops.bce_bwd(pc, label, gout.contiguous()).reshape(shape), None, None


class BCETargetLossFn(Function):

    @_fwd
    def forward(ctx, p, target):
        shape = p.shape
        loss, pc, tc = ops.bce_target_fwd(p.reshape(-1), target.detach().reshape(-1))
        ctx.save_for_backward(pc, tc)
        ctx.shape = shape
        return loss

    @_bwd
    def backward(ctx, gout):
        pc, tc = ctx.saved_tensors
        return ops.bce_target_bwd(pc, tc, gout.contiguous()).reshape(ctx.shape), None


class HingeEmbeddingLossFn(Function):

    @_fwd
    def forward(ctx, x, y, margin):
        loss, xd, yd = ops.hinge_fwd(x, y.detach(), margin)
        ctx.save_for_backward(xd, yd)
        ctx.margin = margin
        ctx.in_shape = x.shape
        return loss

    @_bwd
    def backward(ctx, gout):
        xd, yd = ctx.saved_tensors
        return ops.hinge_bwd(xd, yd, ctx.margin, gout.contiguous()), None, None


class FeatureMatchFn(Function):

    @_fwd
    def forward(ctx, real, fake, out=None):
        loss, diff, rd, fd = ops.fm_fwd(real, fake, out)
        ctx.save_for_backward(diff, rd, fd)
        return loss

    @_bwd
    def backward(ctx, gout):
        diff, rd, fd = ctx.saved_tensors
        dreal, dfake = ops.fm_bwd(diff, rd, fd, gout.contiguous(), ctx.needs_input_grad[0], ctx.needs_input_grad[1])
        return dreal, dfake, None


class LossMixFn(Function):

    @_fwd
    def forward(ctx, lossvec, nfm, rate, arch, which, idx, *slots):
        out = ops.loss_mix_fwd(lossvec, nfm, rate, arch)
        ctx.cfg = (lossvec.numel(), nfm, rate, arch, which, idx)
        ctx.set_materialize_grads(False)
        return tuple(out.unbind(0))

    @_bwd
    def backward(ctx, *gouts):
        nslots, nfm, rate, arch, which, idx = ctx.cfg
        gout = gouts[which]
        if gout is None:
            return (None,) * (6 + len(idx))
        gv = ops.loss_mix_bwd(gout.contiguous(), nslots, nfm, rate, arch, which)
        return (None, None, None, None, None, None) + tuple(gv[i] for i in idx)


def _all_or_none(grads, who):
    live = [g_ is not None for g_ in grads]
    if any(live) and not all(live):
        raise RuntimeError(f"{who}: gradients arrived for some problems of a grouped node only")
    return all(live)


def _flat_grads_of(params):
    fgs = [_flat_grad_of(p) for p in params]
    if any(f is None for f in fgs):
        raise RuntimeError("grouped launches need parameters whose .grad is the optimiser's flat gradient view (optim.Adam)")
    return fgs


class ConvGroupFn(Function):

    @_fwd
    def forward(ctx, g, stride, pad, transposed, *xw):
        xs = [ops.as_nhwc(x) for x in xw[:g]]
        ws = list(xw[g:])
        ctx.g, ctx.sp, ctx.tr = g, (stride, pad), transposed
        ctx.wrefs = ws
        ctx.final = FINAL_PASS
        ctx.save_for_backward(*xs, *ws)
        if transposed:
            hin, win = xs[0].shape[2], xs[0].shape[3]
            hw = ((hin - 1) * stride - 2 * pad + 4, (win - 1) * stride - 2 * pad + 4)
            ys = ops.conv_dgrad_g(xs, ws, hw, stride, pad)
        else:
            ys = ops.conv_fwd_g(xs, ws, stride, pad)
        ctx.set_materialize_grads(False)
        return tuple(ys)

    @_bwd
    def backward(ctx, *dys):
        g = ctx.g
        if not _all_or_none(dys, "ConvGroupFn"):
            return (None,) * (4 + 2 * g)
        saved = ctx.saved_tensors
        xs, ws = list(saved[:g]), ctx.wrefs
        stride, pad = ctx.sp
        dys = [ops.as_nhwc(d) for d in dys]
        need_x = [ctx.needs_input_grad[4 + i] for i in range(g)]
        need_w = [ctx.needs_input_grad[4 + g + i] for i in range(g)]
        if any(need_x) != all(need_x) or any(need_w) != all(need_w):
            raise RuntimeError("ConvGroupFn: the problems of a grouped node must need the same gradients")
        dxs = [None] * g
        if need_x[0]:
            dxs = ops.conv_fwd_g(dys, ws, stride, pad) if ctx.tr else ops.conv_dgrad_g(dys, ws, (xs[0].shape[2], xs[0].shape[3]), stride, pad)
        if need_w[0]:
            fgs = _flat_grads_of(ws)
            share = ops._share_of(ws)
            if ctx.tr:
                ops.conv_wgrad_g(xs, dys, stride, pad, fgs, True, share)
            else:
                ops.conv_wgrad_g(dys, xs, stride, pad, fgs, True, share)
            _final(ctx.final, *ws)
        return (None, None, None, None) + tuple(dxs) + (None,) * g


class ConvC3GroupFn(Function):

    @_fwd
    def forward(ctx, g, act, slope, *xw):
        xs, ws = list(xw[:g]), list(xw[g:])
        ys = ops.c3_fwd_g(xs, ws, act, slope)
        ctx.g, ctx.act = g, (act, slope)
        ctx.wrefs = ws
        ctx.final = FINAL_PASS
        ctx.save_for_backward(*xs, *ws, *ys)
        ctx.set_materialize_grads(False)
        return tuple(ys)

    @_bwd
    def backward(ctx, *dys):
        g = ctx.g
        if not _all_or_none(dys, "ConvC3GroupFn"):
            return (None,) * (3 + 2 * g)
        saved = ctx.saved_tensors
        xs, ws, ys = list(saved[:g]), ctx.wrefs, list(saved[2 * g:])
        act, slope = ctx.act
        need_x = [ctx.needs_input_grad[3 + i] for i in range(g)]
        need_w = [ctx.needs_input_grad[3 + g + i] for i in range(g)]
        if any(need_x) != all(need_x) or any(need_w) != all(need_w):
            raise RuntimeError("ConvC3GroupFn: the problems of a grouped node must need the same gradients")
        dxs = [None] * g
        if need_x[0] or act == ops.ACT_NONE:
            gs = ops.act_bwd_g(dys, ys, act, slope) if act != ops.ACT_NONE else [ops.as_nhwc(d) for d in dys]
            fuse = {}
        else:
            gs = [ops.as_nhwc(d) for d in dys]
            fuse = dict(act_outs=ys, act=act, slope=slope)
        if need_x[0]:
            dxs = ops.c3_dgrad_g(gs, ws, ops.ACT_NONE)
        if need_w[0]:
            fgs = _flat_grads_of(ws)
            ops.c3_wgrad_g(gs, xs, fgs, True, share=ops._share_of(ws), **fuse)
            _final(ctx.final, *ws)
        return (None, None, None) + tuple(dxs) + (None,) * g


class ConvTransposeC3GroupFn(Function):

    @_fwd
    def forward(ctx, g, act, *xw):
        xs = [ops.as_nhwc(x) for x in xw[:g]]
        ws = list(xw[g:])
        outs = ops.c3_dgrad_g(xs, ws, act)
        ctx.g, ctx.act = g, act
        ctx.wrefs = ws
        ctx.final = FINAL_PASS
        ctx.save_for_backward(*xs, *ws, *outs)
        ctx.set_materialize_grads(False)
        return tuple(outs)

    @_bwd
    def backward(ctx, *douts):
        g = ctx.g
        if not _all_or_none(douts, "ConvTransposeC3GroupFn"):
            return (None,) * (2 + 2 * g)
        saved = ctx.saved_tensors
        xs, ws, outs = list(saved[:g]), ctx.wrefs, list(saved[2 * g:])
        gs = ops.act_bwd_g(douts, outs, ctx.act) if ctx.act != ops.ACT_NONE else [d.contiguous() for d in douts]
        need_x = [ctx.needs_input_grad[2 + i] for i in range(g)]
        need_w = [ctx.needs_input_grad[2 + g + i] for i in range(g)]
        if any(need_x) != all(need_x) or any(need_w) != all(need_w):
            raise RuntimeError("ConvTransposeC3GroupFn: the problems of a grouped node must need the same gradients")
        dxs = [None] * g
        if need_x[0]:
            dxs = ops.c3_fwd_g(gs, ws, ops.ACT_NONE)
        if need_w[0]:
            fgs = _flat_grads_of(ws)
            ops.c3_wgrad_g(xs, gs, fgs, True, share=ops._share_of(ws))
            _final(ctx.final, *ws)
        return (None, None) + tuple(dxs) + (None,) * g


class BatchNormActGroupFn(Function):

    @_fwd
    def forward(ctx, g, eps, momentum, act, slope, *t):
        ys = [ops.as_nhwc(y) for y in t[:g]]
        gammas, betas = list(t[g:2 * g]), list(t[2 * g:3 * g])
        rms, rvs, nbts = list(t[3 * g:4 * g]), list(t[4 * g:5 * g]), list(t[5 * g:6 * g])
        share = ops._share_of(gammas)
        saved = ops.bn_train_stats_g(ys, rms, rvs, nbts, eps, momentum, share)
        zs = ops.bn_act_fwd_g(ys, saved, gammas, betas, act, slope)
        ctx.g, ctx.cfg, ctx.share = g, (act, slope), share
        ctx.prefs = (gammas, betas)
        ctx.final = FINAL_PASS
        ctx.save_for_backward(*ys, *saved, *gammas, *betas)
        ctx.set_materialize_grads(False)
        return tuple(zs)

    @_bwd
    def backward(ctx, *dzs):
        g = ctx.g
        if not _all_or_none(dzs, "BatchNormActGroupFn"):
            return (None,) * (5 + 6 * g)
        sv = ctx.saved_tensors
        ys, saved = list(sv[:g]), list(sv[g:2 * g])
        gammas, betas = ctx.prefs
        act, slope = ctx.cfg
        need_p = [ctx.needs_input_grad[5 + g + i] or ctx.needs_input_grad[5 + 2 * g + i] for i in range(g)]
# ... 98 lines not shown
```

discogan_modernized_amd/model.py:

```python
from __future__ import annotations

import math

import torch
import torch.nn as nn

from . import functional as F
from . import ops


FUSE_BN_STATS = {"auto": "auto", "0": False, "1": True, "split": "split"}[__import__("os").environ.get("DG_FUSE_BN", "auto")]
FUSE_BN_MIN_FLOP = 4e10


def _fuse_stats(conv=None, x=None):
    if ops.SHADOW or ops.ACT16:
        return True if ops.FUSE_STATS16 else False
    if FUSE_BN_STATS != "auto":
        return FUSE_BN_STATS
    if conv is None or x is None:
        return False
    n, _, h, w = x.shape
    pixels = h * w if isinstance(conv, ConvTranspose2d) else (h * w) // 4
    return 2.0 * n * pixels * 16 * conv.in_channels * conv.out_channels >= FUSE_BN_MIN_FLOP


def stage_channels(image_size: int):
    n = int(round(math.log2(image_size))) - 2
    if n < 1 or 2 ** (n + 2) != image_size:
        raise ValueError(f"image_size must be a power of two >= 8, got {image_size}")
    return [min(64 * 2 ** i, 2048) for i in range(n)]


def _init_weight(shape):
    w = torch.empty(shape)
    nn.init.kaiming_uniform_(w, a=math.sqrt(5))
    return w


class _FlatGradMixin:

    def zero_grad(self, set_to_none: bool = True):
        for p in self.parameters():
            flat = getattr(p, "_dg_flat_grad", None)
            if flat is not None:
                flat.zero_()
                p.grad = flat
            elif p.grad is not None:
                if set_to_none:
                    p.grad = None
                else:
                    p.grad.detach_()
                    p.grad.zero_()


class Conv2d(nn.Module):

    def __init__(self, in_channels, out_channels, kernel_size=4, stride=2, padding=1, bias=False):
        super().__init__()
        if kernel_size != 4 or bias or (stride, padding) not in ((2, 1), (1, 0)):
            raise ValueError("only Conv2d(k=4, (s,p) in {(2,1),(1,0)}, bias=False) exists in the DiscoGAN path")
        self.in_channels, self.out_channels = in_channels, out_channels
        self.stride, self.padding = stride, padding
        w = _init_weight((out_channels, in_channels, 4, 4))
        if in_channels != 3:
            w = ops.krsc_param(w)
        self.weight = nn.Parameter(w)

    def forward(self, x, fused_act=ops.ACT_NONE, slope=0.2, want_stats=False, want_planes=False):
        if self.in_channels == 3:
            return F.ConvC3Fn.apply(x, self.weight, fused_act, slope, want_planes)
        if want_stats:
            return F.ConvFn.apply(x, self.weight, self.stride, self.padding, want_stats)
        return F.ConvFn.apply(x, self.weight, self.stride, self.padding)

    @property
    def emits_bn_stats(self):
        return self.in_channels != 3 and self.stride == 2

    def extra_repr(self):
        return f"{self.in_channels}, {self.out_channels}, kernel_size=(4, 4), stride={self.stride}, padding={self.padding}, bias=False"


class ConvTranspose2d(nn.Module):

    def __init__(self, in_channels, out_channels, kernel_size=4, stride=2, padding=1, bias=False):
        super().__init__()
        if kernel_size != 4 or bias or (stride, padding) not in ((2, 1), (1, 0)):
            raise ValueError("only ConvTranspose2d(k=4, (s,p) in {(2,1),(1,0)}, bias=False) exists in the DiscoGAN path")
        self.in_channels, self.out_channels = in_channels, out_channels
        self.stride, self.padding = stride, padding
        w = _init_weight((in_channels, out_channels, 4, 4))
        if out_channels != 3:
            w = ops.krsc_param(w)
        self.weight = nn.Parameter(w)

    def forward(self, x, fused_act=ops.ACT_NONE, want_stats=False):
        if self.out_channels == 3:
            return F.ConvTransposeC3Fn.apply(x, self.weight, fused_act)
        if want_stats:
            return F.ConvTransposeFn.apply(x, self.weight, self.stride, self.padding, want_stats)
        return F.ConvTransposeFn.apply(x, self.weight, self.stride, self.padding)

    @property
    def emits_bn_stats(self):
        return self.out_channels != 3 and self.stride == 2

    def extra_repr(self):
        return f"{self.in_channels}, {self.out_channels}, kernel_size=(4, 4), stride={self.stride}, padding={self.padding}, bias=False"


class BatchNorm2d(nn.Module):

    def __init__(self, num_features, eps=1e-5, momentum=0.1):
        super().__init__()
        self.num_features, self.eps, self.momentum = num_features, eps, momentum
        self.weight = nn.Parameter(torch.ones(num_features))
        self.bias = nn.Parameter(torch.zeros(num_features))
        self.register_buffer("running_mean", torch.zeros(num_features))
        self.register_buffer("running_var", torch.ones(num_features))
        self.register_buffer("num_batches_tracked", torch.tensor(0, dtype=torch.long))

    def forward(self, y, fused_act=ops.ACT_NONE, slope=0.2, partials=None, z_cm=False, dy_cm=False, z_po=False, dy_po=False):
        if self.training and y.shape[0] * y.shape[2] * y.shape[3] <= 1:
            raise ValueError(f"Expected more than 1 value per channel when training, got input size {tuple(y.shape)}")
        return F.BatchNormActFn.apply(y, self.weight, self.bias, self.running_mean, self.running_var,
                                      self.num_batches_tracked, self.training, self.eps, self.momentum, fused_act, slope,
                                      partials, z_cm, dy_cm, z_po, dy_po)

    def extra_repr(self):
        return f"{self.num_features}, eps={self.eps}, momentum={self.momentum}, affine=True, track_running_stats=True"


class _Act(nn.Module):
    act = ops.ACT_NONE

    def __init__(self, slope=0.0, inplace=False):
        super().__init__()
        self.negative_slope, self.inplace = slope, inplace

    def forward(self, x):
        return F.ActFn.apply(x, self.act, self.negative_slope)


class LeakyReLU(_Act):
    act = ops.ACT_LEAKY

    def __init__(self, negative_slope=0.01, inplace=False):
        super().__init__(negative_slope, inplace)


class ReLU(_Act):
    act = ops.ACT_RELU

    def __init__(self, inplace=False):
        super().__init__(0.0, inplace)


class Sigmoid(_Act):
    act = ops.ACT_SIGMOID

    def __init__(self):
        super().__init__(0.0, False)


def _plane_hints(conv, x, nxt, z_is_output=False):
    if not ops.X3:
        return False, False, False, False
    n, _, h, w = x.shape
    dy_cm = z_cm = dy_po = z_po = False
    s2conv = isinstance(conv, Conv2d) and conv.stride == 2 and conv.in_channels != 3
    s2convT = isinstance(conv, ConvTranspose2d) and conv.stride == 2 and conv.out_channels != 3
    if s2conv:
        dy_cm = ops.x3_window_dgrad(n, h, w, conv.in_channels, conv.out_channels)
        dy_po = ops.x3_all_plane_readers(n, h, w, conv.in_channels, conv.out_channels, forward_is_dgrad=True)
        ho, wo = h // 2, w // 2
    elif s2convT:
        dy_po = ops.x3_all_plane_readers(n, 2 * h, 2 * w, conv.out_channels, conv.in_channels, forward_is_dgrad=False)
        ho, wo = 2 * h, 2 * w
    else:
        ho, wo = (4, 4) if isinstance(conv, ConvTranspose2d) else (1, 1)
    if not z_is_output and isinstance(nxt, ConvTranspose2d) and nxt.stride == 2 and nxt.out_channels != 3:
        z_cm = ops.x3_window_dgrad(n, 2 * ho, 2 * wo, nxt.out_channels, nxt.in_channels)
        z_po = ops.x3_all_plane_readers(n, 2 * ho, 2 * wo, nxt.out_channels, nxt.in_channels, forward_is_dgrad=True)
    elif not z_is_output and isinstance(nxt, Conv2d) and nxt.stride == 2 and nxt.in_channels != 3:
        z_po = ops.x3_all_plane_readers(n, ho, wo, nxt.in_channels, nxt.out_channels, forward_is_dgrad=False)
    return z_cm and ops.X3_CM, dy_cm and ops.X3_CM, z_po, dy_po


C3_PLANES = __import__("os").environ.get("DG_X3_C3_PLANES", "1") != "0"


def _first_layer_planes(x, nxt):
    if not (ops.X3 and C3_PLANES and isinstance(nxt, Conv2d) and nxt.stride == 2):
        return False
    n, _, h, w = x.shape
    geom = (n, h // 2, w // 2, nxt.in_channels, nxt.out_channels, 2, 1)
    planes = ops.x3_fwd_weight_planes(*geom, nxt.weight)
    if planes == 1 or (planes == 0 and ops.X3_RSP):
        return True
# ... 245 lines not shown
```

discogan_modernized_amd/ops.py:

```python
from __future__ import annotations

import collections
import ctypes
import os

import torch

from . import _lib

ACT_NONE, ACT_LEAKY, ACT_RELU, ACT_SIGMOID = 0, 1, 2, 3
PREC_DEFAULT, PREC_F32, PREC_BF16, PREC_F32X3 = -1, 0, 1, 2


class Context:

    def __init__(self, prec=None, shadow=False, act16=False, x3=False, group_plan="launch"):
        self.prec = prec
        self.group_plan = group_plan
        self.shadow, self.act16, self.x3 = bool(shadow), bool(act16), bool(x3)
        self.shadow_tab, self.plane_tab = {}, {}

    @property
    def cprec(self):
        return PREC_DEFAULT if self.prec is None else int(self.prec)
# ... 632 lines not shown
        ao = as_nhwc(act_out)
        if ao.shape != dy.shape or ao.dtype != dy.dtype or ao.stride() != dy.stride():
            raise _lib.DiscoganHipError("c3_dgrad: act_out must have dy's shape, type and layout")
        with _hbm("edge_c3_dgrad", 2.0 * dy.numel() * dy.element_size() + 4.0 * dx.numel()):
            _lib.check(L.dg_conv4x4s2_c3_dgrad_act_p(_ptr(dy), int(_is16(dy)), _ptr(ao), in_act, float(slope), _ptr(w), _ptr(dx), n, 2 * ho, 2 * wo, k,
                                                     act, _CUR.cprec, _ptr(ws), wsb, _stream()), "dg_conv4x4s2_c3_dgrad_act_p")
        return dx
    if _is16(dy) and not L.dg_c3_dgrad_act_ok(n, 2 * ho, 2 * wo, k, 1):
        dyf = torch.empty_like(dy, dtype=torch.float32)
        dyf.copy_(dy)
        dy = dyf
    with _hbm("edge_c3_dgrad", dy.numel() * dy.element_size() + 4.0 * dx.numel()):
        _lib.check(L.dg_conv4x4s2_c3_dgrad_p(_ptr(dy), int(_is16(dy)), _ptr(w), _ptr(dx), n, 2 * ho, 2 * wo, k, act, _CUR.cprec, _ptr(ws), wsb,
                                             _stream()), "dg_conv4x4s2_c3_dgrad_p")
    return dx


def c3_wgrad(dy, x_nchw, out=None, accumulate=False, act_out=None, act=ACT_NONE, slope=0.0):
    _check_dev(dy, act_out, allow16=True)
    _check_dev(x_nchw)
    dy = as_nhwc(dy)
    x = x_nchw.contiguous()
    n, k, ho, wo = dy.shape
    h, wd = x.shape[2], x.shape[3]
    dw = out if out is not None else torch.empty((k, 3, 4, 4), device=dy.device, dtype=torch.float32)
    L = _lib.load()
    ws, wsb = _ws(L.dg_c3_wgrad_workspace_bytes(n, h, wd, k), dy.device)
    fuse = act_out is not None and act != ACT_NONE
    ao = None
    if fuse:
        ao = as_nhwc(act_out)
        assert ao.shape == dy.shape and ao.dtype == dy.dtype
    with _hbm("edge_c3_wgrad", float(dy.element_size()) * ((2 if fuse else 1) * dy.numel()) + 4.0 * x.numel()):
        _lib.check(L.dg_conv4x4s2_c3_wgrad_p(_ptr(dy), _ptr(ao), int(_is16(dy)), act if fuse else ACT_NONE, float(slope), _ptr(x), _ptr(dw),
                                             n, h, wd, k, _CUR.cprec, int(accumulate), _ptr(ws), wsb, _stream()), "dg_conv4x4s2_c3_wgrad_p")
    return dw


def c3_tail_bn_ok(y, need_wgrad=True):
    if _is16(y) or _CUR.act16 or _CUR.shadow:
        return False
    n, k, ho, wo = y.shape
    L = _lib.load()
    return bool(L.dg_c3_dgrad_bn_ok(n, 2 * ho, 2 * wo, k, _CUR.cprec)) and \
        (not need_wgrad or bool(L.dg_c3_wgrad_bn_ok(n, 2 * ho, 2 * wo, k, _CUR.cprec)))


def c3_dgrad_bn(y, saved, gamma, beta, w, act=ACT_NONE, bn_act=ACT_RELU):
    _check_dev(y, saved, gamma, beta, w)
    y = as_nhwc(y)
    w = w.contiguous()
    n, k, ho, wo = y.shape
    dx = torch.empty((n, 3, 2 * ho, 2 * wo), device=y.device, dtype=torch.float32)
    with _hbm("edge_c3_dgrad", 4.0 * y.numel() + 4.0 * dx.numel()):
        _lib.check(_lib.load().dg_conv4x4s2_c3_dgrad_bn_p(_ptr(y), _ptr(saved), _ptr(gamma), _ptr(beta), bn_act, _ptr(w), _ptr(dx), n, 2 * ho, 2 * wo,
                                                          k, act, _CUR.cprec, _stream()), "dg_conv4x4s2_c3_dgrad_bn_p")
    return dx


def c3_wgrad_bn(y, saved, gamma, beta, x_nchw, out=None, accumulate=False, bn_act=ACT_RELU):
    _check_dev(y, saved, gamma, beta, x_nchw)
    y = as_nhwc(y)
    x = x_nchw.contiguous()
    n, k, ho, wo = y.shape
    h, wd = x.shape[2], x.shape[3]
    dw = out if out is not None else torch.empty((k, 3, 4, 4), device=y.device, dtype=torch.float32)
    L = _lib.load()
    ws, wsb = _ws(L.dg_c3_wgrad_workspace_bytes(n, h, wd, k), y.device)
    with _hbm("edge_c3_wgrad", 4.0 * y.numel() + 4.0 * x.numel()):
        _lib.check(L.dg_conv4x4s2_c3_wgrad_bn_p(_ptr(y), _ptr(saved), _ptr(gamma), _ptr(beta), bn_act, _ptr(x), _ptr(dw), n, h, wd, k, _CUR.cprec,
                                                int(accumulate), _ptr(ws), wsb, _stream()), "dg_conv4x4s2_c3_wgrad_bn_p")
    return dw


def bn_train_stats(y, running_mean, running_var, nbt, eps, momentum):
    _check_dev(y, allow16=True)
    y = as_nhwc(y)
    n, c, h, w = y.shape
    m = n * h * w
    saved = torch.empty((2, c), device=y.device, dtype=torch.float32)
    L = _lib.load()
    ws, wsb = _ws(L.dg_bn_workspace_bytes(m, c), y.device)
    with _hbm("bn_stats", float(y.element_size()) * m * c):
        _lib.check(L.dg_bn_train_stats_t(_ptr(y), int(_is16(y)), m, c, eps, momentum, _ptr(running_mean), _ptr(running_var), _ptr(nbt),
                                         _ptr(saved), _ptr(ws), wsb, _stream()), "dg_bn_train_stats")
    return saved


_PARTIALS_ONE_LAUNCH = _env_flag("DG_BN_PARTIALS_ONE_LAUNCH", False)


def bn_stats_from_partials(stat, y, running_mean, running_var, nbt, eps, momentum):
    _check_dev(stat)
    n, c, h, w = y.shape
    saved = torch.empty((2, c), device=y.device, dtype=torch.float32)
    L = _lib.load()
    ws, wsb = (None, 0) if _PARTIALS_ONE_LAUNCH else _ws(L.dg_bn_partials_workspace_bytes(stat.shape[0], c), y.device)
    _lib.check(L.dg_bn_stats_from_partials(_ptr(stat), stat.shape[0], n * h * w, c, eps, momentum,
                                           _ptr(running_mean), _ptr(running_var), _ptr(nbt), _ptr(saved),
                                           _ptr(ws), wsb, _stream()), "dg_bn_stats_from_partials")
    return saved


def _bn_out(y, planes_cm, planes_only):
    n, c, h, w = y.shape
    if _is16(y):
        return "bf16", empty_nhwc(n, c, h, w, y.device, torch.bfloat16), None, 0, False
    out = empty_nhwc(n, c, h, w, y.device)
    if _CUR.x3 and c % 8 == 0:
        extra = torch.empty((3, out.numel()), device=y.device, dtype=torch.bfloat16)
        cm = int(bool(planes_cm) and c % 64 == 0 and (n * h * w) % 4 == 0)
        return "planes", out, extra, cm, bool(planes_only) and X3_PLANES_ONLY
    if _CUR.shadow and c % 8 == 0:
        return "shadow", out, empty_nhwc_bf16(n, c, h, w, y.device), 0, False
    return "plain", out, None, 0, False


def _bn_publish(form, out, extra, cm, plane_only):
    if form == "planes":
        planes_put(out, extra, cm)
        if plane_only:
            out._dg_planes_only = True
            if POISON_PLANES_ONLY:
                out.fill_(float("nan"))
    elif form == "shadow":
        shadow_put(out, extra)
    return out


_BN_FWD_BYTES = {"bf16": 4.0, "planes": 14.0, "planes_only": 10.0, "shadow": 10.0, "plain": 8.0}
_BN_BWD_BYTES = {"bf16": 10.0, "planes": 26.0, "planes_only": 22.0, "shadow": 22.0, "plain": 20.0}


def bn_act_fwd(y, saved, gamma, beta, act, slope=0.2, planes_cm=False, planes_only=False):
    _check_dev(y, allow16=True)
    y = as_nhwc(y)
    n, c, h, w = y.shape
    m = n * h * w
    form, z, extra, cm, po = _bn_out(y, planes_cm, planes_only)
    L = _lib.load()
    rest = (m, c, _ptr(saved), _ptr(gamma), _ptr(beta), act, slope, _stream())
    with _hbm("bn_apply", _BN_FWD_BYTES["planes_only" if po else form] * m * c):
        if form == "bf16":
            _lib.check(L.dg_bn_act_fwd_t(_ptr(y), _ptr(z), 1, *rest), "dg_bn_act_fwd_t")
        elif form == "planes":
            _lib.check(L.dg_bn_act_fwd_x3(_ptr(y), None if po else _ptr(z), _ptr(extra), extra.stride(0), cm, *rest), "dg_bn_act_fwd_x3")
        elif form == "shadow":
            _lib.check(L.dg_bn_act_fwd_bf16(_ptr(y), _ptr(z), _ptr(extra), *rest), "dg_bn_act_fwd_bf16")
        else:
            _lib.check(L.dg_bn_act_fwd(_ptr(y), _ptr(z), *rest), "dg_bn_act_fwd")
    return _bn_publish(form, z, extra, cm, po)


def bn_act_bwd(dz, y, saved, gamma, beta, act, slope=0.2, need_param_grads=True, out_grads=None, planes_cm=False, planes_only=False):
    _check_dev(dz, y, allow16=True)
    dz = as_nhwc(dz)
    y = as_nhwc(y)
    n, c, h, w = y.shape
    m = n * h * w
    acc = 0
    if out_grads is not None:
        dgamma, dbeta = out_grads
        acc = 1
    else:
        dgamma = torch.empty(c, device=y.device, dtype=torch.float32) if need_param_grads else None
        dbeta = torch.empty(c, device=y.device, dtype=torch.float32) if need_param_grads else None
    L = _lib.load()
    ws, wsb = _ws(L.dg_bn_workspace_bytes(m, c), y.device)
    if _is16(y) and not _is16(dz):
        raise _lib.DiscoganHipError("bn_act_bwd: bf16 y needs a bf16 dz")
    form, dy, extra, cm, po = _bn_out(y, planes_cm, planes_only)
    rest = (m, c, _ptr(saved), _ptr(gamma), _ptr(beta), act, slope, _ptr(dgamma), _ptr(dbeta), acc, _ptr(ws), wsb, _stream())
    with _hbm("bn_backward", _BN_BWD_BYTES["planes_only" if po else form] * m * c):
        if form == "bf16":
            _lib.check(L.dg_bn_act_bwd_t(_ptr(dz), _ptr(y), _ptr(dy), 1, *rest), "dg_bn_act_bwd_t")
        elif form == "planes":
            _lib.check(L.dg_bn_act_bwd_x3(_ptr(dz), _ptr(y), None if po else _ptr(dy), _ptr(extra), extra.stride(0), cm, *rest), "dg_bn_act_bwd_x3")
        elif form == "shadow":
            _lib.check(L.dg_bn_act_bwd_bf16(_ptr(dz), _ptr(y), _ptr(dy), _ptr(extra), *rest), "dg_bn_act_bwd_bf16")
        else:
            _lib.check(L.dg_bn_act_bwd(_ptr(dz), _ptr(y), _ptr(dy), *rest), "dg_bn_act_bwd")
    return _bn_publish(form, dy, extra, cm, po), dgamma, dbeta


def _dense_like(x):
    return torch.empty_like(x, memory_format=torch.preserve_format)


def _dense(x):
    if x.is_contiguous() or is_nhwc(x):
        return x
    return x.contiguous()


def act_fwd(x, act, slope=0.2):
    _check_dev(x)
    x = _dense(x)
    y = _dense_like(x)
    _lib.check(_lib.load().dg_act_fwd(_ptr(x), _ptr(y), x.numel(), act, slope, _stream()), "dg_act_fwd")
    return y


def act_bwd(dy, out, act, slope=0.2):
    _check_dev(dy, out, allow16=True)
    out = _dense(out)
    if dy.stride() != out.stride():
        dyl = _dense_like(out)
        dyl.copy_(dy)
        dy = dyl
    dx = _dense_like(out)
    if _is16(out) or _is16(dy):
        if dy.dtype != out.dtype:
            raise _lib.DiscoganHipError("act_bwd: dy and out must have the same dtype")
        _lib.check(_lib.load().dg_act_bwd_t(_ptr(dy), _ptr(out), _ptr(dx), 1, out.numel(), act, slope, _stream()), "dg_act_bwd_t")
        return dx
    _lib.check(_lib.load().dg_act_bwd(_ptr(dy), _ptr(out), _ptr(dx), out.numel(), act, slope, _stream()), "dg_act_bwd")
    return dx


def _loss_ws(device):
    L = _lib.load()
    return _ws(L.dg_loss_workspace_bytes(), device)


def same_layout_pair(a, b):
    a = _dense(a)
    if b.stride() != a.stride():
        bl = _dense_like(a)
        bl.copy_(b)
        b = bl
    return a, b


def mse_fwd(x, t, out=None):
    _check_dev(x, t)
    x, t = same_layout_pair(x, t)
    loss = out if out is not None else torch.empty((), device=x.device, dtype=torch.float32)
    ws, wsb = _loss_ws(x.device)
    _lib.check(_lib.load().dg_mse_fwd(_ptr(x), _ptr(t), x.numel(), _ptr(loss), _ptr(ws), wsb, _stream()), "dg_mse_fwd")
    return loss, x, t


def mse_bwd(x, t, gout):
    _check_dev(x, t, gout)
    dx = _dense_like(x)
    _lib.check(_lib.load().dg_mse_bwd(_ptr(x), _ptr(t), x.numel(), _ptr(gout), _ptr(dx), _stream()), "dg_mse_bwd")
    return dx


def bce_fwd(p, label, out=None):
    _check_dev(p)
    p = p.contiguous()
    loss = out if out is not None else torch.empty((), device=p.device, dtype=torch.float32)
    _lib.check(_lib.load().dg_bce_fwd(_ptr(p), p.numel(), float(label), _ptr(loss), None, 0, _stream()), "dg_bce_fwd")
    return loss, p


def bce_bwd(p, label, gout):
    dp = torch.empty_like(p)
    _lib.check(_lib.load().dg_bce_bwd(_ptr(p), p.numel(), float(label), _ptr(gout), _ptr(dp), _stream()), "dg_bce_bwd")
    return dp


def bce_target_fwd(p, target, out=None):
    _check_dev(p, target)
    p, target = p.contiguous(), target.contiguous()
    if p.numel() != target.numel():
        raise ValueError(f"Using a target size ({tuple(target.shape)}) that is different to the input size ({tuple(p.shape)}) is deprecated. Please ensure they have the same size.")
    loss = out if out is not None else torch.empty((), device=p.device, dtype=torch.float32)
    _lib.check(_lib.load().dg_bce_target_fwd(_ptr(p), _ptr(target), p.numel(), _ptr(loss), _stream()), "dg_bce_target_fwd")
    return loss, p, target


def bce_target_bwd(p, target, gout):
    dp = torch.empty_like(p)
    _lib.check(_lib.load().dg_bce_target_bwd(_ptr(p), _ptr(target), p.numel(), _ptr(gout), _ptr(dp), _stream()), "dg_bce_target_bwd")
    return dp


def hinge_fwd(x, y, margin=1.0):
    _check_dev(x, y)
    x, y = same_layout_pair(x, y)
    loss = torch.empty((), device=x.device, dtype=torch.float32)
    ws, wsb = _loss_ws(x.device)
    _lib.check(_lib.load().dg_hinge_fwd(_ptr(x), _ptr(y), x.numel(), float(margin), _ptr(loss), _ptr(ws), wsb, _stream()), "dg_hinge_fwd")
    return loss, x, y


def hinge_bwd(x, y, margin, gout):
    dx = _dense_like(x)
    _lib.check(_lib.load().dg_hinge_bwd(_ptr(x), _ptr(y), x.numel(), float(margin), _ptr(gout), _ptr(dx), _stream()), "dg_hinge_bwd")
    return dx


def fm_fwd(real, fake, out=None):
    _check_dev(real, fake, allow16=True)
    real, fake = same_layout_pair(real, fake)
    n = real.shape[0]
    j = real.numel() // n
    diff = torch.empty(j, device=real.device, dtype=torch.float32)
    loss = out if out is not None else torch.empty((), device=real.device, dtype=torch.float32)
    ws, wsb = _ws(_lib.load().dg_fm_workspace_bytes(n, j), real.device)
    if real.dtype != fake.dtype:
        raise _lib.DiscoganHipError("fm_fwd: real and fake features must have the same dtype")
    _lib.check(_lib.load().dg_fm_fwd_t(_ptr(real), _ptr(fake), int(_is16(real)), n, j, _ptr(diff), _ptr(loss), _ptr(ws), wsb, _stream()),
               "dg_fm_fwd")
    return loss, diff, real, fake


def fm_bwd(diff, like_real, like_fake, gout, need_real, need_fake):
    n = like_fake.shape[0]
    j = diff.numel()
    dreal = _dense_like(like_real) if need_real else None
    dfake = _dense_like(like_fake) if need_fake else None
    _lib.check(_lib.load().dg_fm_bwd_t(_ptr(diff), n, j, _ptr(gout), _ptr(dreal), _ptr(dfake), int(_is16(like_fake)), _stream()), "dg_fm_bwd")
    return dreal, dfake


def loss_mix_fwd(lossvec, nfm, rate, arch):
    out = torch.empty(8, device=lossvec.device, dtype=torch.float32)
    _lib.check(_lib.load().dg_loss_mix_fwd(_ptr(lossvec), _ptr(out), nfm, float(rate), arch, _stream()), "dg_loss_mix_fwd")
    return out


def loss_mix_bwd(gout, nslots, nfm, rate, arch, which):
    gv = torch.empty(nslots, device=gout.device, dtype=torch.float32)
    _lib.check(_lib.load().dg_loss_mix_bwd(_ptr(gout), _ptr(gv), nfm, float(rate), arch, which, _stream()), "dg_loss_mix_bwd")
    return gv


def adam_advance(state, lr, beta1, beta2, ctl=None):
    if ctl is not None:
        _check_ctl(ctl, "adam_advance")
        _lib.check(_lib.load().dg_adam_advance_c(_ptr(state), lr, beta1, beta2, _ptr(ctl), _stream()), "dg_adam_advance_c")
        return
    _lib.check(_lib.load().dg_adam_advance(_ptr(state), lr, beta1, beta2, _stream()), "dg_adam_advance")


def adam_step_flat(p, g, m, v, state, beta1, beta2, eps, weight_decay, grad_scale=1.0, p16=None, p3=None, ctl=None):
    if ctl is not None:
        _check_ctl(ctl, "adam_step_flat")
        form, out, dist = (3, p3[0], p3[1]) if p3 is not None else ((1, _ptr(p16), 0) if p16 is not None else (0, None, 0))
        with _hbm("adam", (28.0 + 2.0 * form) * p.numel()):
            _lib.check(_lib.load().dg_adam_step_flat_c(_ptr(p), _ptr(g), _ptr(m), _ptr(v), p.numel(), _ptr(state), beta1, beta2, eps,
                                                       weight_decay, _ptr(ctl), out, form, dist, _stream()), "dg_adam_step_flat_c")
        return
    if p3 is not None:
        with _hbm("adam", 34.0 * p.numel()):
            _lib.check(_lib.load().dg_adam_step_flat_x3(_ptr(p), _ptr(g), _ptr(m), _ptr(v), p.numel(), _ptr(state), beta1, beta2,
                                                        eps, weight_decay, grad_scale, p3[0], p3[1], _stream()), "dg_adam_step_flat_x3")
        return
    if p16 is not None:
        with _hbm("adam", 30.0 * p.numel()):
            _lib.check(_lib.load().dg_adam_step_flat_bf16(_ptr(p), _ptr(g), _ptr(m), _ptr(v), p.numel(), _ptr(state), beta1, beta2,
                                                          eps, weight_decay, grad_scale, _ptr(p16), _stream()), "dg_adam_step_flat_bf16")
        return
    with _hbm("adam", 28.0 * p.numel()):
        _lib.check(_lib.load().dg_adam_step_flat(_ptr(p), _ptr(g), _ptr(m), _ptr(v), p.numel(), _ptr(state), beta1,
                                                 beta2,
                                                 eps, weight_decay, grad_scale, _stream()), "dg_adam_step_flat")


GRAD_STATS_MAX_GRID = 4096


def _check_ctl(ctl, who):
    if not (ctl.is_cuda and ctl.dtype == torch.float64 and ctl.dim() == 1 and ctl.numel() >= 8 and ctl.is_contiguous()):
        raise _lib.DiscoganHipError(f"{who}: ctl must be a contiguous float64 HIP tensor of 8 elements")


def grad_stats_workspace(device):
    return torch.zeros(_lib.load().dg_grad_stats_workspace_bytes() // 8, device=device, dtype=torch.float64)


def grad_sumsq_partial(g, ws, slot0=0):
    _check_dev(g)
    if g.dim() != 1 or not g.is_contiguous():
        raise _lib.DiscoganHipError(f"grad_sumsq_partial: a contiguous 1-D fp32 tensor required, got {tuple(g.shape)}")
    if not (ws.is_cuda and ws.dtype == torch.float64 and ws.dim() == 1 and ws.is_contiguous()):
        raise _lib.DiscoganHipError("grad_sumsq_partial: the workspace must be a contiguous float64 HIP tensor")
    import ctypes as C
    used = C.c_int(0)
    with _hbm("gradnorm", 4.0 * g.numel()):
        _lib.check(_lib.load().dg_grad_sumsq_partial(_ptr(g), g.numel(), _ptr(ws), ws.numel() * 8, int(slot0), C.byref(used), _stream()),
                   "dg_grad_sumsq_partial")
    return used.value


def grad_clip_finalize(ws, slots, pre_scale, max_norm, guard, ctl):
    _check_ctl(ctl, "grad_clip_finalize")
    if not (ws.is_cuda and ws.dtype == torch.float64 and ws.is_contiguous()) or slots > ws.numel():
        raise _lib.DiscoganHipError(f"grad_clip_finalize: {slots} slots of a float64 HIP workspace of {ws.numel()}")
    _lib.check(_lib.load().dg_grad_clip_finalize(_ptr(ws), int(slots), float(pre_scale), float(max_norm), int(bool(guard)), _ptr(ctl),
                                                 _stream()), "dg_grad_clip_finalize")


def _flat_pair(a, b, who):
    _check_dev(a, b)
    if a.dim() != 1 or b.dim() != 1 or a.numel() != b.numel() or not (a.is_contiguous() and b.is_contiguous()):
        raise _lib.DiscoganHipError(f"{who}: two contiguous 1-D fp32 tensors of one length required, got {tuple(a.shape)} and {tuple(b.shape)}")


def ema_update_flat(ema, p, w):
    _flat_pair(ema, p, "ema_update_flat")
    with _hbm("ema", 12.0 * p.numel()):
        _lib.check(_lib.load().dg_ema_update_flat(_ptr(ema), _ptr(p), p.numel(), float(w), _stream()), "dg_ema_update_flat")


def swap_flat(a, b):
    _flat_pair(a, b, "swap_flat")
    with _hbm("swap", 16.0 * a.numel()):
        _lib.check(_lib.load().dg_swap_flat(_ptr(a), _ptr(b), a.numel(), _stream()), "dg_swap_flat")


def group_ok():
    return not (_CUR.shadow or _CUR.act16 or _CUR.x3)


def _plan_groups(g):
    return 1 if getattr(_CUR, "group_plan", "launch") == "single" else g


def _same_shape(ts, who):
    for t in ts[1:]:
        if t.shape != ts[0].shape:
            raise _lib.DiscoganHipError(f"{who}: the problems of a grouped launch must have identical shapes")


def _ws_g(nbytes, g, device):
    if nbytes == 0:
        return [None] * g, 0
    per = (nbytes + 255) // 256 * 64
    t = torch.empty(g * per, device=device, dtype=torch.float32)
    return [t[i * per:(i + 1) * per] for i in range(g)], per * 4


def _share_of(params):
    g = len(params)
    run = 1
    while run < g and params[run] is params[0]:
        run += 1
    if g % run != 0 or any(params[i] is not params[i // run * run] for i in range(g)) or \
            any(params[i] is params[i - run] for i in range(run, g, run)):
        raise _lib.DiscoganHipError("grouped launch: problems sharing a parameter must form runs of equal length")
    return run


def _conv_g(op, as_, bs, stride, pad, x_hw=None, outs=None, accumulate=False, share=1):
    who = _CONV_NAME[op] + "_g"
    g = len(as_)
    _check_dev(*as_, *bs)
    as_ = [as_nhwc(t) for t in as_]
    bs = [as_nhwc(t) if op == 2 else _krsc(t) for t in bs]
    _same_shape(as_, who)
    _same_shape(bs, who)
    rq = _ConvReq(op, as_[0], bs[0], stride, pad, x_hw)
    pg = _plan_groups(g)
    wsl, wsb = _ws_g(rq.workspace_bytes(pg), g, as_[0].device)
    if outs is None:
        outs = [empty_nhwc(*rq.out_shape, as_[0].device) for _ in range(g)]
    _launch_g(rq, as_, bs, outs, pg, None, wsl, wsb, share, accumulate)
    return outs


def conv_fwd_g(xs, ws_, stride, pad):
    return _conv_g(0, xs, ws_, stride, pad)


def conv_dgrad_g(dys, ws_, x_hw, stride, pad):
    return _conv_g(1, dys, ws_, stride, pad, x_hw)


def conv_wgrad_g(dys, xs, stride, pad, outs, accumulate, share=1):
    _conv_g(2, dys, xs, stride, pad, None, outs, accumulate, share)


def c3_fwd_g(xs, ws_, act=ACT_NONE, slope=0.2):
    g = len(xs)
    _check_dev(*xs, *ws_)
    xs = [x.contiguous() for x in xs]
    ws_ = [w.contiguous() for w in ws_]
    _same_shape(xs, "c3_fwd_g")
    n, _, h, wd = xs[0].shape
    k = ws_[0].shape[0]
    ys = [empty_nhwc(n, k, h // 2, wd // 2, xs[0].device) for _ in range(g)]
    with _prof("c3_fwd", 2.0 * g * n * (h // 2) * (wd // 2) * k * 48), _hbm("edge_c3_fwd", g * (4.0 * xs[0].numel() + 4.0 * ys[0].numel())):
        _lib.check(_lib.load().dg_conv4x4s2_c3_fwd_g(g, _tab(xs), _tab(ws_), _tab(ys), n, h, wd, k, act, slope, _CUR.cprec, _stream()),
                   "dg_conv4x4s2_c3_fwd_g")
    return ys


def c3_dgrad_g(dys, ws_, act=ACT_NONE):
    g = len(dys)
    _check_dev(*dys, *ws_)
    dys = [as_nhwc(d) for d in dys]
    ws_ = [w.contiguous() for w in ws_]
    _same_shape(dys, "c3_dgrad_g")
    n, k, ho, wo = dys[0].shape
    dxs = [torch.empty((n, 3, 2 * ho, 2 * wo), device=dys[0].device, dtype=torch.float32) for _ in range(g)]
    with _hbm("edge_c3_dgrad", g * (4.0 * dys[0].numel() + 4.0 * dxs[0].numel())):
        _lib.check(_lib.load().dg_conv4x4s2_c3_dgrad_g(g, _tab(dys), _tab(ws_), _tab(dxs), n, 2 * ho, 2 * wo, k, act, _CUR.cprec, _stream()),
                   "dg_conv4x4s2_c3_dgrad_g")
    return dxs


def c3_wgrad_g(dys, xs, outs, accumulate, act_outs=None, act=ACT_NONE, slope=0.0, share=1):
    g = len(dys)
    _check_dev(*dys, *xs)
    dys = [as_nhwc(d) for d in dys]
    xs = [x.contiguous() for x in xs]
    _same_shape(dys, "c3_wgrad_g")
    n, k, ho, wo = dys[0].shape
    h, wd = xs[0].shape[2], xs[0].shape[3]
    fuse = act_outs is not None and act != ACT_NONE
    aos = [as_nhwc(a) for a in act_outs] if fuse else None
# ... 172 lines not shown
```

discogan_modernized_amd/optim.py:

```python
from __future__ import annotations

import torch

from . import ops

_ALIGN = 64


class Adam:
    def __init__(self, params, lr=1e-3, betas=(0.9, 0.999), eps=1e-8, weight_decay=0.0):
        self.params = [p for p in params]
        if not self.params:
            raise ValueError("optimizer got an empty parameter list")
        dev = self.params[0].device
        if dev.type != "cuda":
            raise RuntimeError("discogan_modernized_amd.optim.Adam needs parameters on a HIP device (no CPU fallback)")
        self.defaults = dict(lr=lr, betas=betas, eps=eps, weight_decay=weight_decay)
        self.param_groups = [dict(params=self.params, **self.defaults)]
        offs, total = [], 0
        for p in self.params:
            if p.dtype != torch.float32 or p.device != dev:
                raise RuntimeError("all parameters must be fp32 on one device")
            offs.append(total)
            total += (p.numel() + _ALIGN - 1) // _ALIGN * _ALIGN
        self.numel = total
        self.flat_p = torch.zeros(total, device=dev)
        self.flat_g = torch.zeros(total, device=dev)
        self.exp_avg = torch.zeros(total, device=dev)
        self.exp_avg_sq = torch.zeros(total, device=dev)
        self.state = torch.zeros(4, device=dev, dtype=torch.float64)
        self.offsets = offs
        self.ctl = None
        with torch.no_grad():
            for p, off in zip(self.params, offs):
                n = p.numel()
                view = self.flat_p[off:off + n].as_strided(p.shape, p.stride())
                view.copy_(p.data)
                p.data = view
                gview = self.flat_g[off:off + n].as_strided(p.shape, p.stride())
                p._dg_flat_grad = gview
                p.grad = gview

    def enable_bf16_shadow(self):
        if getattr(self, "flat_p16", None) is not None:
            return
        self.flat_p16 = torch.empty(self.numel, device=self.flat_p.device, dtype=torch.bfloat16)
        ops.f32_to_bf16(self.flat_p, self.flat_p16)
        for p, off in zip(self.params, self.offsets):
            p._dg_bf16 = self.flat_p16[off:off + p.numel()].as_strided(p.shape, p.stride())
            p._dg_bf16_ver = p._version

    def enable_x3_planes(self):
        if getattr(self, "flat_p3", None) is not None:
            return
        self.flat_p3 = torch.empty((3, self.numel), device=self.flat_p.device, dtype=torch.bfloat16)
        ops.f32_to_bf16x3(self.flat_p, self.flat_p3)
        convs = [(off, p.shape[0], 16 * p.shape[1]) for p, off in zip(self.params, self.offsets)
                 if p.dim() == 4 and tuple(p.shape[2:]) == (4, 4) and p.shape[0] > 1 and ops.is_krsc(p)]
        self.flat_p3t = torch.zeros((3, self.numel), device=self.flat_p.device, dtype=torch.bfloat16) if convs else None
        self._x3t_table = ops.x3_transpose_table(convs)
        conv_offs = {c[0] for c in convs}
        for p, off in zip(self.params, self.offsets):
            p._dg_x3 = (self.flat_p3, off, self.flat_p3t if off in conv_offs else None)
            p._dg_x3_ver = p._version
        if convs:
            ops.x3_transpose_planes(self.flat_p3, self.flat_p3t, self._x3t_table)

    def enable_grad_control(self, max_norm=0.0, guard=False):
        max_norm = float(max_norm)
        if not max_norm >= 0.0:
            raise ValueError(f"max_norm must be >= 0 (0 = no clipping), got {max_norm}")
        self.max_norm, self.guard = max_norm, bool(guard)
        if self.ctl is None:
            self.ctl = torch.zeros(8, device=self.flat_p.device, dtype=torch.float64)
            self._stats_ws = ops.grad_stats_workspace(self.flat_p.device)

    def grad_stats(self):
        if self.ctl is None:
            raise RuntimeError("grad_stats(): gradient control is off (enable_grad_control)")
        c = self.ctl.cpu().tolist()
        return dict(sumsq=c[0], norm=c[1], scale=c[2], skip=bool(c[3]), steps=int(c[4]), clipped=int(c[5]), skipped=int(c[6]),
                    max_norm=c[7])

    def refresh_derived(self):
        if getattr(self, "flat_p16", None) is not None:
            ops.f32_to_bf16(self.flat_p, self.flat_p16)
        if getattr(self, "flat_p3", None) is not None:
            ops.f32_to_bf16x3(self.flat_p, self.flat_p3)
            if self.flat_p3t is not None:
                ops.x3_transpose_planes(self.flat_p3, self.flat_p3t, self._x3t_table)

    def zero_grad(self, set_to_none: bool = True):
        self.flat_g.zero_()
        for p in self.params:
            if p.grad is not p._dg_flat_grad:
                p.grad = p._dg_flat_grad

    def _sync_foreign_grads(self):
        for p in self.params:
            if p.grad is None:
                p._dg_flat_grad.zero_()
                p.grad = p._dg_flat_grad
            elif p.grad is not p._dg_flat_grad and p.grad.data_ptr() != p._dg_flat_grad.data_ptr():
                p._dg_flat_grad.copy_(p.grad)
                p.grad = p._dg_flat_grad

    def ranges_of(self, modules):
        ids = {id(p) for m in modules for p in m.parameters()}
        out = []
        for p, off in zip(self.params, self.offsets):
            if id(p) in ids:
                end = off + (p.numel() + _ALIGN - 1) // _ALIGN * _ALIGN
                if out and out[-1][1] == off:
                    out[-1][1] = end
                else:
                    out.append([off, end])
        return [tuple(r) for r in out]

    @torch.no_grad()
    def step(self, grad_scale: float = 1.0, active=None):
        g = self.param_groups[0]
        self._sync_foreign_grads()
        ranges = active if active is not None else [(0, self.numel)]
        ctl = self.ctl
        if ctl is not None:
            slots = 0
            for b, e in ranges:
                slots += ops.grad_sumsq_partial(self.flat_g[b:e], self._stats_ws, slots)
            ops.grad_clip_finalize(self._stats_ws, slots, float(grad_scale), self.max_norm, self.guard, ctl)
        ops.adam_advance(self.state, float(g["lr"]), float(g["betas"][0]), float(g["betas"][1]), ctl=ctl)
        p16 = getattr(self, "flat_p16", None)
        p3 = getattr(self, "flat_p3", None)
        for b, e in ranges:
            ops.adam_step_flat(self.flat_p[b:e], self.flat_g[b:e], self.exp_avg[b:e], self.exp_avg_sq[b:e], self.state,
                               float(g["betas"][0]), float(g["betas"][1]), float(g["eps"]), float(g["weight_decay"]),
                               float(grad_scale), p16=None if p16 is None else p16[b:e],
                               p3=None if p3 is None else (p3.data_ptr() + 2 * b, self.numel), ctl=ctl)
        if p3 is not None and self.flat_p3t is not None:
            ops.x3_transpose_planes(p3, self.flat_p3t, self._x3t_table)

    def state_dict(self):
        sd = dict(step=self.state[0:1].clone(), exp_avg=self.exp_avg.clone(), exp_avg_sq=self.exp_avg_sq.clone(),
                  param_groups=[{k: v for k, v in self.param_groups[0].items() if k != "params"}])
        if self.ctl is not None:
            sd["grad_control"] = self.ctl[4:8].clone()
        return sd

    def load_state_dict(self, sd):
        self.state.zero_()
        self.state[0:1].copy_(sd["step"])
        self.exp_avg.copy_(sd["exp_avg"])
        self.exp_avg_sq.copy_(sd["exp_avg_sq"])
        if self.ctl is not None:
            self.ctl.zero_()
            if "grad_control" in sd:
                self.ctl[4:8].copy_(sd["grad_control"])
        for k, v in sd["param_groups"][0].items():
            self.param_groups[0][k] = v


class EMA:

    def __init__(self, opt, decay):
        decay = float(decay)
        if not 0.0 < decay < 1.0:
            raise ValueError(f"EMA decay must be in (0, 1), got {decay}")
        self.opt = opt
        self.decay = decay
        self.flat = torch.zeros_like(opt.flat_p)
        self.updates = 0
        self.ready = False

    @torch.no_grad()
    def update(self):
        if not self.ready:
            self.flat.copy_(self.opt.flat_p)
            self.ready = True
            return
        ops.ema_update_flat(self.flat, self.opt.flat_p, float(1.0 - self.decay))
        self.updates += 1

    @torch.no_grad()
    def swap(self):
        ops.swap_flat(self.flat, self.opt.flat_p)
        self.opt.refresh_derived()

    def view_of(self, param):
        for p, off in zip(self.opt.params, self.opt.offsets):
            if p is param:
                return self.flat[off:off + p.numel()].as_strided(p.shape, p.stride())
        raise KeyError("not a parameter of this EMA's optimiser")

    def state_dict(self):
        return dict(flat=self.flat.clone(), updates=int(self.updates), ready=bool(self.ready), decay=float(self.decay))

    def load_state_dict(self, sd):
        self.flat.copy_(sd["flat"])
        self.updates = int(sd["updates"])
        self.ready = bool(sd["ready"])
        self.decay = float(sd["decay"])
```

discogan_modernized_amd/trainer.py:

```python
from __future__ import annotations

import contextlib
from itertools import chain
from types import SimpleNamespace

import torch

from . import dp
from . import functional as F_
from . import losses as L
from . import optim
from .model import Discriminator, Generator

LOG_KEYS = ("gen_loss_A", "gen_loss_B", "fm_loss_A", "fm_loss_B", "recon_loss_A", "recon_loss_B",
            "dis_loss_A", "dis_loss_B", "gen_loss", "dis_loss")

DEFAULTS = dict(learning_rate=2e-4, beta1=0.5, beta2=0.999, weight_decay=0.00001, gan_curriculum=10000,
                starting_rate=0.01, default_rate=0.5, update_interval=3, model_arch="discogan",
                ema_decay=0.0, ema_start_iter=0, grad_clip=0.0, nonfinite_guard=False, log_grad_norm=False)


def check_ema_decay(decay):
    decay = float(decay)
    if not 0.0 <= decay < 1.0:
# ... 224 lines not shown
            dis_loss_A=dis_loss_A, dis_loss_B=dis_loss_B, AB=AB, BA=BA, ABA=ABA, BAB=BAB,
            A_dis_real=A_dis_real, A_dis_fake=A_dis_fake, B_dis_real=B_dis_real, B_dis_fake=B_dis_fake,
            A_feats_real=A_feats_real, B_feats_fake=B_feats_fake, lossvec=lv)

    def _two_chain_forward(self, A, B, lv, pair, gen_ctx, main, side, want_recon):
        F_.FINAL_PASS = True
        try:
            with gen_ctx():
                BA, AB = pair(self.generator_A.forward_steps(B), self.generator_B.forward_steps(A))
        finally:
            F_.FINAL_PASS = False
        if self.two_streams:
            AB.record_stream(side)
            BA.record_stream(main)
        if self.graph_overlap:
            if self.two_streams:
                main.wait_stream(side)
            self._cut("dis_ready")
            if self.two_streams:
                side.wait_stream(main)
        elif self.two_streams:
            ev_ab, ev_ba = torch.cuda.Event(), torch.cuda.Event()
            ev_ab.record(main)
            ev_ba.record(side)
            side.wait_event(ev_ab)
            main.wait_event(ev_ba)
        if self._ev_dis_ready is not None:
            main.wait_event(self._ev_dis_ready)
            if self.two_streams:
                side.wait_event(self._ev_dis_ready)
            self._ev_dis_ready = None
        ABA = BAB = None
        if want_recon:
            with gen_ctx():
                ABA, BAB = pair(self.generator_A.forward_steps(AB), self.generator_B.forward_steps(BA))
        else:
            lv[:2].fill_(float("nan"))
        (A_dis_real, A_feats_real), (B_dis_real, B_feats_real) = pair(
            self.discriminator_A.forward_steps(A), self.discriminator_B.forward_steps(B))
        (A_dis_fake, A_feats_fake), (B_dis_fake, B_feats_fake) = pair(
            self.discriminator_A.forward_steps(BA), self.discriminator_B.forward_steps(AB))
        return BA, AB, ABA, BAB, A_dis_real, A_feats_real, B_dis_real, B_feats_real, A_dis_fake, A_feats_fake, B_dis_fake, B_feats_fake

    def _forward_losses_grouped(self, A, B, iters, need_losses=True):
        from .model import group_discriminators, group_generators
        a = self.args
        dstep = self.is_dis_step(iters)
        gen_ctx = torch.no_grad if dstep else torch.enable_grad
        main = torch.cuda.current_stream(self.device)
        side = self.side_stream if self.two_streams else main
        on_side = (lambda: torch.cuda.stream(side)) if self.two_streams else contextlib.nullcontext
        gA, gB, dA, dB = self.generator_A, self.generator_B, self.discriminator_A, self.discriminator_B
        nfm = dA.n_stages - 1
        lv = torch.empty(8 + 2 * nfm, device=self.device, dtype=torch.float32)
        sl = [lv[i] for i in range(8 + 2 * nfm)]
        terms = {}
        F_.FINAL_PASS = True
        try:
            cut = None
            with gen_ctx():
                if self.graph_overlap and not dstep and self._split_backward:
                    (BA, AB), hs, leaves = group_generators([gA, gB], [B, A], cut_at_bottleneck=True)
                    cut = (hs, leaves)
                else:
                    BA, AB = group_generators([gA, gB], [B, A])
        finally:
            F_.FINAL_PASS = False
        if self.graph_overlap:
            self._cut("dis_ready")
        elif self._ev_dis_ready is not None:
            main.wait_event(self._ev_dis_ready)
            self._ev_dis_ready = None
        if self.two_streams:
            side.wait_stream(main)
            for t_ in (A, B, lv, AB, BA):
                t_.record_stream(side)
        want_recon = need_losses or not dstep
        ABA = BAB = None
        if want_recon:
            with gen_ctx():
                ABA, BAB = group_generators([gA, gB], [AB, BA])
                terms[0], terms[1] = F_.MSELossGroupFn.apply(2, ABA, BAB, A, B, sl[0], sl[1])
        else:
            lv[:2].fill_(float("nan"))
            terms[0], terms[1] = sl[0], sl[1]
        with on_side():
            if dstep:
                (A_dis_real, A_feats_real), (A_dis_fake, A_feats_fake), (B_dis_real, B_feats_real), (B_dis_fake, B_feats_fake) = \
                    group_discriminators([dA, dA, dB, dB], [A, BA, B, AB])
            else:
                with torch.no_grad():
                    (A_dis_real, A_feats_real), (B_dis_real, B_feats_real) = group_discriminators([dA, dB], [A, B])
                (A_dis_fake, A_feats_fake), (B_dis_fake, B_feats_fake) = group_discriminators([dA, dB], [BA, AB])
            terms[2], terms[4], terms[5], terms[7] = F_.BCELossGroupFn.apply(
                4, (1.0, 1.0, 1.0, 1.0), A_dis_real, A_dis_fake, B_dis_real, B_dis_fake, sl[2], sl[4], sl[5], sl[7])
            terms[3], terms[6] = F_.BCELossGroupFn.apply(2, (0.0, 0.0), A_dis_fake, B_dis_fake, sl[3], sl[6])
            for l in range(nfm):
                terms[8 + l], terms[8 + nfm + l] = F_.FeatureMatchGroupFn.apply(
                    2, A_feats_real[l], B_feats_real[l], A_feats_fake[l], B_feats_fake[l], sl[8 + l], sl[8 + nfm + l])
        if self.two_streams:
            main.wait_stream(side)
        rate = self.rate(iters)
        fmA, fmB = list(range(8, 8 + nfm)), list(range(8 + nfm, 8 + 2 * nfm))
        which, idx = (7, (2, 3, 5, 6)) if dstep else (6, tuple([0, 1, 4, 7] + fmA + fmB))
        (gen_loss_A, gen_loss_B, fm_loss_A, fm_loss_B, dis_loss_A, dis_loss_B, gen_loss, dis_loss) = \
            F_.LossMixFn.apply(lv, nfm, rate, 0, which, idx, *[terms[i] for i in idx])
        return SimpleNamespace(
            gen_loss=gen_loss, dis_loss=dis_loss, gen_loss_A=gen_loss_A, gen_loss_B=gen_loss_B,
            fm_loss_A=fm_loss_A, fm_loss_B=fm_loss_B, recon_loss_A=terms[0], recon_loss_B=terms[1],
            dis_loss_A=dis_loss_A, dis_loss_B=dis_loss_B, AB=AB, BA=BA, ABA=ABA, BAB=BAB,
            A_dis_real=A_dis_real, A_dis_fake=A_dis_fake, B_dis_real=B_dis_real, B_dis_fake=B_dis_fake,
            A_feats_real=A_feats_real, B_feats_fake=B_feats_fake, lossvec=lv, backward_cut=cut)

    def _cut(self, name):
        if self._cap is not None:
            self._cap.cut(name)
        else:
            self._gap(name)

    def _gap(self, name):
        main = torch.cuda.current_stream(self.device)
        if name == "dis_ready":
            if self._ev_dis_ready is not None:
                main.wait_event(self._ev_dis_ready)
                self._ev_dis_ready = None
        elif name == "dec_bucket":
            opt = self.optim_gen
            ev = torch.cuda.Event()
            ev.record(main)
            self.comm_stream.wait_event(ev)
            with torch.cuda.stream(self.comm_stream):
                self._adam_begin(opt)
                self._exchange_and_step_ranges(opt, self._gen_ranges()[1], "G")
            self._dec_done = True
        else:
            raise ValueError(name)

    def _gen_ranges(self):
        if getattr(self, "_gen_rng", None) is None:
            enc = self.optim_gen.ranges_of([self.generator_A.encoder, self.generator_B.encoder])
            dec = self.optim_gen.ranges_of([self.generator_A.decoder, self.generator_B.decoder])
            self._gen_rng = (enc, dec)
        return self._gen_rng

    def _adam_begin(self, opt):
        g = opt.param_groups[0]
        opt._sync_foreign_grads()
        from . import ops
        ops.adam_advance(opt.state, float(g["lr"]), float(g["betas"][0]), float(g["betas"][1]))

    def _exchange_and_step_ranges(self, opt, ranges, kind):
        from . import ops
        g = opt.param_groups[0]
        for b, e in ranges:
            scale = 1.0
            if self.xg is not None:
                if self.time_comm:
                    e0, e1 = torch.cuda.Event(enable_timing=True), torch.cuda.Event(enable_timing=True)
                    e0.record()
                    scale = self.xg.all_reduce_sum_(opt.flat_g[b:e])
                    e1.record()
                    self.comm_events[kind].append((e0, e1))
                else:
                    scale = self.xg.all_reduce_sum_(opt.flat_g[b:e])
            ops.adam_step_flat(opt.flat_p[b:e], opt.flat_g[b:e], opt.exp_avg[b:e], opt.exp_avg_sq[b:e], opt.state,
                               float(g["betas"][0]), float(g["betas"][1]), float(g["eps"]), float(g["weight_decay"]), float(scale))

    def _fwd_bwd(self, A, B, iters, need_losses=True):
        dstep = self.is_dis_step(iters)
        self._set_requires_grad(dstep)
        if self.skip_dead_work:
            if dstep and self._ev_dis_ready is not None and self._cap is None:
                torch.cuda.current_stream(self.device).wait_event(self._ev_dis_ready)
            (self.optim_dis if dstep else self.optim_gen).zero_grad()
        else:
            self.optim_gen.zero_grad()
            self.optim_dis.zero_grad()
        from . import ops as _ops
        self.ctx.prec = {"f32": _ops.PREC_F32, "bf16": _ops.PREC_BF16, "f32x3": _ops.PREC_F32X3}[self.mfma_dtype]
        self.ctx.shadow, self.ctx.act16, self.ctx.x3 = bool(self.bf16_shadow), self.act_dtype == "bf16", bool(self.x3_planes)
        self.ctx.clear()
        try:
            with _ops.use(self.ctx):
                out = self.forward_losses(A, B, iters, need_losses)
                cut = getattr(out, "backward_cut", None)
                if cut is not None:
                    out.gen_loss.backward(gradient=self._one)
                    if self.two_streams:
                        torch.cuda.current_stream(self.device).wait_stream(self.side_stream)
                    self._cut("dec_bucket")
                    hs, leaves = cut
                    torch.autograd.backward(list(hs), [l.grad for l in leaves])
                    out.backward_cut = None
                else:
                    (out.dis_loss if dstep else out.gen_loss).backward(gradient=self._one)
        finally:
            self.ctx.clear()
        if self.skip_dead_work and not dstep:
            for p in self.optim_dis.params:
                p.requires_grad_(True)
        if self.two_streams:
            torch.cuda.current_stream(self.device).wait_stream(self.side_stream)
        return out

    def _graph_key(self, A, B, iters, need_losses=True):
        return ("D" if self.is_dis_step(iters) else "G", self.rate(iters), bool(need_losses) or not self.is_dis_step(iters),
                tuple(A.shape), tuple(B.shape))

    def _fwd_bwd_graphed(self, A, B, iters, need_losses=True):
        shp = (tuple(A.shape), tuple(B.shape))
        if self._static is None:
            self._static = {}
        if shp not in self._static:
            self._static[shp] = (torch.empty_like(A), torch.empty_like(B))
        sA, sB = self._static[shp]
        sA.copy_(A)
        sB.copy_(B)
        key = self._graph_key(A, B, iters, need_losses)
        ent = self._graphs.get(key)
        if ent is None:
            if self.graph_overlap:
                cap = _SegCapture(self)
                self._cap = cap
                try:
                    with cap:
                        out = self._fwd_bwd(sA, sB, iters, need_losses)
                finally:
                    self._cap = None
                ent = (cap, out)
            else:
                g = torch.cuda.CUDAGraph()
                torch.cuda.synchronize()
                with torch.cuda.graph(g):
                    out = self._fwd_bwd(sA, sB, iters, need_losses)
                ent = (g, out)
            self._graphs[key] = ent
        ent[0].replay()
        return ent[1]

    def _exchange(self, opt, kind):
        if self.xg is None:
            return 1.0
        if self.time_comm:
            e0, e1 = torch.cuda.Event(enable_timing=True), torch.cuda.Event(enable_timing=True)
            e0.record()
            scale = self.xg.all_reduce_sum_(opt.flat_g)
            e1.record()
            self.comm_events[kind].append((e0, e1))
            return scale
        return self.xg.all_reduce_sum_(opt.flat_g)

    def train_iteration(self, A, B, iters, do_step=True, need_losses=True):
        dstep = self.is_dis_step(iters)
        opt = self.optim_dis if dstep else self.optim_gen
        if self.graph_overlap:
            return self._train_iteration_graph_overlap(A, B, iters, do_step, need_losses)
        bucketed = self._buckets is not None and not dstep and do_step and self.xg is not None and not self.grad_control
        if self.time_comm:
            self.comm_steps["D" if dstep else "G"] += 1
        if bucketed:
            self._buckets.begin(opt, self.active_ranges(dstep))
        try:
            if self.use_graph and iters >= self._eager_until:
                out = self._fwd_bwd_graphed(A, B, iters, need_losses)
            else:
                out = self._fwd_bwd(A, B, iters, need_losses)
        finally:
            if bucketed:
                F_.FINAL_HOOK = None
        if bucketed:
            self._buckets.finish()
            self._ema_update(iters)
            return out
        if do_step:
            self.apply_step(iters)
        return out

    def apply_step(self, iters):
        dstep = self.is_dis_step(iters)
        opt = self.optim_dis if dstep else self.optim_gen
        if dstep and (self.overlap_comm or self.graph_overlap):
            main = torch.cuda.current_stream(self.device)
            ev = torch.cuda.Event()
            ev.record(main)
            self.comm_stream.wait_event(ev)
            with torch.cuda.stream(self.comm_stream):
                scale = self._exchange(opt, "D")
                opt.step(grad_scale=scale, active=self.active_ranges(dstep))
                self._ev_dis_ready = torch.cuda.Event()
                self._ev_dis_ready.record(self.comm_stream)
            return
        scale = self._exchange(opt, "D" if dstep else "G")
        opt.step(grad_scale=scale, active=self.active_ranges(dstep))
        if not dstep:
            self._ema_update(iters)

    def _ema_update(self, iters):
        if self.ema is not None and iters >= self.args.ema_start_iter:
            self.ema.update()

    def _train_iteration_graph_overlap(self, A, B, iters, do_step, need_losses):
        dstep = self.is_dis_step(iters)
        opt = self.optim_dis if dstep else self.optim_gen
        main = torch.cuda.current_stream(self.device)
        if self.time_comm:
            self.comm_steps["D" if dstep else "G"] += 1
        if dstep and self._ev_dis_ready is not None:
            main.wait_event(self._ev_dis_ready)
            self._ev_dis_ready = None
        self._split_backward, self._dec_done = bool(do_step) and not self.grad_control, False
        if self.use_graph and iters >= self._eager_until and do_step:
            out = self._fwd_bwd_graphed(A, B, iters, need_losses)
        else:
            out = self._fwd_bwd(A, B, iters, need_losses)
        if not do_step:
            return out
        if dstep or not self._dec_done:
            self.apply_step(iters)
            return out
        ev = torch.cuda.Event()
        ev.record(main)
        self.comm_stream.wait_event(ev)
        with torch.cuda.stream(self.comm_stream):
            self._exchange_and_step_ranges(opt, self._gen_ranges()[0], "G")
        main.wait_stream(self.comm_stream)
        self._ema_update(iters)
        return out

    def comm_ms(self):
        torch.cuda.synchronize(self.device)
        out = {}
        for k, evs in self.comm_events.items():
            if evs and self.comm_steps[k]:
                out[k] = sum(a.elapsed_time(b) for a, b in evs) / self.comm_steps[k]
        return out

    def finish(self):
        if self._ev_dis_ready is not None:
            torch.cuda.current_stream(self.device).wait_event(self._ev_dis_ready)

    def sample(self, test_A, test_B):
        if test_A.dim() != 4 or test_B.dim() != 4 or test_A.shape[0] < 2 or test_B.shape[0] < 2:
            raise ValueError("sample() needs two batches [n,3,S,S] with n >= 2 (train-mode BatchNorm needs more than one value per "
                             f"channel at the bottleneck), got {tuple(test_A.shape)} and {tuple(test_B.shape)}")
        self.finish()
        from . import ops as _ops
        self.ctx.prec = {"f32": _ops.PREC_F32, "bf16": _ops.PREC_BF16, "f32x3": _ops.PREC_F32X3}[self.mfma_dtype]
        self.ctx.shadow, self.ctx.act16, self.ctx.x3 = bool(self.bf16_shadow), self.act_dtype == "bf16", bool(self.x3_planes)
        self.ctx.clear()
        try:
            with torch.no_grad(), _ops.use(self.ctx):
                AB = self.generator_B(test_A)
                BA = self.generator_A(test_B)
                ABA = self.generator_A(AB)
                BAB = self.generator_B(BA)
        finally:
            self.ctx.clear()
        return AB, BA, ABA, BAB

    @contextlib.contextmanager
    def ema_weights(self):
        if self.ema is None:
            raise RuntimeError("ema_weights(): this trainer keeps no EMA (ema_decay = 0)")
        if not self.ema.ready:
            raise RuntimeError("ema_weights(): the EMA holds nothing yet (no generator step at iteration >= ema_start_iter so far)")
        self.finish()
        saved = [(b, b.clone()) for net in (self.generator_A, self.generator_B) for b in net.buffers()]
        self.ema.swap()
        try:
            yield self
        finally:
            self.ema.swap()
            with torch.no_grad():
                for b, old in saved:
                    b.copy_(old)

    def ema_state_dicts(self):
        if self.ema is None or not self.ema.ready:
            raise RuntimeError("ema_state_dicts(): no EMA weights (ema_decay = 0, or no qualifying generator step yet)")
        self.finish()
        out = {}
        for key, net in (("gen_A", self.generator_A), ("gen_B", self.generator_B)):
            params = dict(net.named_parameters())
            out[key] = {n: (self.ema.view_of(params[n]) if n in params else t).detach().contiguous().cpu()
                        for n, t in net.state_dict().items()}
        return out

    def losses_to_floats(self, out):
        vals = torch.stack([getattr(out, k).detach().reshape(()) for k in LOG_KEYS]).cpu().tolist()
        return dict(zip(LOG_KEYS, vals))

    def format_log(self, iters, total, out):
        f = self.losses_to_floats(out)
        return (f"Iter [{iters}/{total}] "
                f"GEN: {f['gen_loss_A']:.4f}/{f['gen_loss_B']:.4f}, "
                f"FM: {f['fm_loss_A']:.4f}/{f['fm_loss_B']:.4f}, "
                f"RECON: {f['recon_loss_A']:.4f}/{f['recon_loss_B']:.4f}, "
                f"DIS: {f['dis_loss_A']:.4f}/{f['dis_loss_B']:.4f}" + self.grad_log_suffix())

    def grad_log_suffix(self):
        if not self.grad_control:
            return ""
        self.finish()
        return format_grad_suffix(self.optim_dis.grad_stats(), self.optim_gen.grad_stats())

    def state_dicts(self):
        return {k: v.state_dict() for k, v in self.nets.items()}

    def train_state(self, next_iter, extra=None):
        self.finish()
        torch.cuda.synchronize(self.device)
        st = dict(iters=int(next_iter), nets={k: {n: t.detach().contiguous().cpu() for n, t in v.state_dict().items()}
                                              for k, v in self.nets.items()},
                  optim_gen=self.optim_gen.state_dict(), optim_dis=self.optim_dis.state_dict())
        if self.ema is not None:
            st["ema"] = self.ema.state_dict()
        if extra:
            st["loader"] = dict(extra)
        return st

    def load_train_state(self, st):
        for k, v in self.nets.items():
            v.load_state_dict(st["nets"][k])
        self.optim_gen.load_state_dict(st["optim_gen"])
        self.optim_dis.load_state_dict(st["optim_dis"])
        if self.ema is not None:
            if "ema" in st:
                self.ema.load_state_dict(st["ema"])
            else:
                self.ema.ready, self.ema.updates = False, 0
        self._graphs = {}
        start = int(st["iters"])
        self._eager_until = start + self.args.update_interval
        return start

    def close(self):
        if self.xg is not None:
            self.finish()
            torch.cuda.synchronize(self.device)
            self.xg.close()
            self.xg = None


class _SegCapture:

    def __init__(self, trainer):
        self.tr = trainer
        self.graphs, self.gaps = [], []
        self.pool = torch.cuda.graph_pool_handle()
        self.stream = torch.cuda.Stream(device=trainer.device)
        self._ctx = None

    def _begin(self):
        g = torch.cuda.CUDAGraph()
        g.capture_begin(pool=self.pool, capture_error_mode="global")
        self.graphs.append(g)

    def __enter__(self):
        import gc
        torch.cuda.synchronize(self.tr.device)
        gc.collect()
        torch.cuda.empty_cache()
        self.stream.wait_stream(torch.cuda.current_stream(self.tr.device))
        self._ctx = torch.cuda.stream(self.stream)
        self._ctx.__enter__()
        self._begin()
        return self

    def cut(self, name):
        self.graphs[-1].capture_end()
        self.gaps.append(name)
        self._begin()

    def __exit__(self, et, ev, tb):
        try:
            self.graphs[-1].capture_end()
        finally:
            self._ctx.__exit__(et, ev, tb)
        torch.cuda.current_stream(self.tr.device).wait_stream(self.stream)
        return False

    def replay(self):
        for i, g in enumerate(self.graphs):
            g.replay()
            if i < len(self.gaps):
                self.tr._gap(self.gaps[i])


class _GradBuckets:

    def __init__(self, trainer, bucket_mb):
        self.tr = trainer
        opt = trainer.optim_gen
        target = int(bucket_mb * 1024 * 1024 / 4)
        self.buckets = []
        self.of_param = {}
        for net in (trainer.generator_A, trainer.generator_B):
            ids = {id(p) for p in net.parameters()}
            cur = None
            for p, off in zip(opt.params, opt.offsets):
                if id(p) not in ids:
                    continue
                end = off + (p.numel() + optim._ALIGN - 1) // optim._ALIGN * optim._ALIGN
                if cur is None or cur["end"] - cur["begin"] >= target:
                    cur = dict(begin=off, end=end, nparams=0, pending=0, done=False)
                    self.buckets.append(cur)
                cur["end"] = end
                cur["nparams"] += 1
                self.of_param[id(p)] = cur
        self.opt = opt
        self.launched = 0
        self.active = None

    def begin(self, opt, active=None):
        assert opt is self.opt
        self.active = active
        tr = self.tr
        main = torch.cuda.current_stream(tr.device)
        for b in self.buckets:
            b["pending"], b["done"] = b["nparams"], False
        self.launched = 0
        tr.comm_stream.wait_stream(main)
        with torch.cuda.stream(tr.comm_stream):
            g = opt.param_groups[0]
            opt._sync_foreign_grads()
            from . import ops
            ops.adam_advance(opt.state, float(g["lr"]), float(g["betas"][0]), float(g["betas"][1]))
        F_.FINAL_HOOK = self.notify

    def notify(self, param):
        b = self.of_param.get(id(param))
        if b is None or b["done"]:
            return
        if param.grad is not param._dg_flat_grad:
            raise RuntimeError("bucketed exchange: a parameter's .grad was replaced during the backward pass "
                               "(it must stay the view of the optimiser's flat gradient buffer)")
        b["pending"] -= 1
        if b["pending"] == 0:
            self._launch(b, torch.cuda.current_stream(self.tr.device), early=True, active=self.active)

    def _launch(self, b, producer_stream, early, active=None):
        tr, opt = self.tr, self.opt
        b["done"] = True
        ev = torch.cuda.Event()
        ev.record(producer_stream)
        tr.comm_stream.wait_event(ev)
        with torch.cuda.stream(tr.comm_stream):
            sl = slice(b["begin"], b["end"])
            scale = 1.0
            if tr.xg is not None:
                if tr.time_comm:
                    e0, e1 = torch.cuda.Event(enable_timing=True), torch.cuda.Event(enable_timing=True)
                    e0.record()
                    scale = tr.xg.all_reduce_sum_(opt.flat_g[sl])
                    e1.record()
                    tr.comm_events["G"].append((e0, e1))
                else:
                    scale = tr.xg.all_reduce_sum_(opt.flat_g[sl])
            if active is None or any(lo <= b["begin"] and b["end"] <= hi for lo, hi in active):
                g = opt.param_groups[0]
                from . import ops
                p16 = getattr(opt, "flat_p16", None)
                p3 = getattr(opt, "flat_p3", None)
                ops.adam_step_flat(opt.flat_p[sl], opt.flat_g[sl], opt.exp_avg[sl], opt.exp_avg_sq[sl], opt.state,
                                   float(g["betas"][0]), float(g["betas"][1]), float(g["eps"]), float(g["weight_decay"]),
                                   float(scale), p16=None if p16 is None else p16[sl],
                                   p3=None if p3 is None else (p3.data_ptr() + 2 * b["begin"], opt.numel))
        if early:
            self.launched += 1

    def finish(self):
        tr = self.tr
        main = torch.cuda.current_stream(tr.device)
        for b in self.buckets:
            if not b["done"]:
                self._launch(b, main, early=False, active=self.active)
        opt = tr.optim_gen
        if getattr(opt, "flat_p3t", None) is not None:
            from . import ops
            with torch.cuda.stream(tr.comm_stream):
                ops.x3_transpose_planes(opt.flat_p3, opt.flat_p3t, opt._x3t_table)
        main.wait_stream(tr.comm_stream)


def synthetic_batch(n, image_size, seed, device):
    g = torch.Generator().manual_seed(seed)
    A = torch.rand(n, 3, image_size, image_size, generator=g)
    B = torch.rand(n, 3, image_size, image_size, generator=g)
    return A.to(device), B.to(device)
```

include/discogan_hip.h:

```cpp
#ifndef DISCOGAN_HIP_H
#define DISCOGAN_HIP_H

#include <stddef.h>
#include <stdint.h>

#ifdef __cplusplus
extern "C" {
#endif

#define DG_OK 0
#define DG_ERR_INVALID (-1)
#define DG_ERR_WORKSPACE (-2)
#define DG_ERR_HIP (-3)

#define DG_ACT_NONE 0
#define DG_ACT_LEAKY 1
#define DG_ACT_RELU 2
#define DG_ACT_SIGMOID 3

typedef void* dg_stream_t;

#define DG_PREC_DEFAULT (-1)
#define DG_PREC_F32 0
#define DG_PREC_BF16 1
// ... 67 lines not shown
                           int accumulate, void* ws, size_t ws_bytes, dg_stream_t s);

int dg_conv4x4s2_c3_fwd(const float* x_nchw, const float* w, float* y_nhwc, int N, int H, int W, int K,
                        int act, float slope, dg_stream_t s);
size_t dg_c3_dgrad_workspace_bytes(int K);
int dg_conv4x4s2_c3_dgrad(const float* dy_nhwc, const float* w, float* dx_nchw, int N, int H, int W, int K,
                          int act, void* ws, size_t ws_bytes, dg_stream_t s);
size_t dg_c3_wgrad_workspace_bytes(int N, int H, int W, int K);
int dg_conv4x4s2_c3_wgrad(const float* dy_nhwc, const float* x_nchw, float* dw, int N, int H, int W, int K,
                          int accumulate, void* ws, size_t ws_bytes, dg_stream_t s);
int dg_conv4x4s2_c3_wgrad_act(const float* dy_nhwc, const float* act_out_nhwc, int act, float slope,
                              const float* x_nchw, float* dw, int N, int H, int W, int K, int accumulate,
                              void* ws, size_t ws_bytes, dg_stream_t s);

int dg_conv4x4s2_c3_fwd_p(const float* x_nchw, const float* w, void* y_nhwc, int y_bf16, int N, int H, int W, int K,
                          int act, float slope, int prec, dg_stream_t s);
int dg_conv4x4s2_c3_dgrad_p(const void* dy_nhwc, int dy_bf16, const float* w, float* dx_nchw, int N, int H, int W, int K,
                            int act, int prec, void* ws, size_t ws_bytes, dg_stream_t s);
int dg_conv4x4s2_c3_wgrad_p(const void* dy_nhwc, const void* act_out_nhwc, int io_bf16, int act, float slope,
                            const float* x_nchw, float* dw, int N, int H, int W, int K, int prec, int accumulate,
                            void* ws, size_t ws_bytes, dg_stream_t s);
int dg_c3_dgrad_act_ok(int N, int H, int W, int K, int dy_bf16);
int dg_conv4x4s2_c3_dgrad_act_p(const void* dy_nhwc, int dy_bf16, const void* act_out_nhwc, int in_act, float slope, const float* w,
                                float* dx_nchw, int N, int H, int W, int K, int act, int prec, void* ws, size_t ws_bytes, dg_stream_t s);
int dg_c3_dgrad_bn_ok(int N, int H, int W, int K, int prec);
int dg_conv4x4s2_c3_dgrad_bn_p(const float* y_nhwc, const float* saved, const float* gamma, const float* beta, int bn_act, const float* w,
                               float* dx_nchw, int N, int H, int W, int K, int act, int prec, dg_stream_t s);
int dg_c3_wgrad_bn_ok(int N, int H, int W, int K, int prec);
int dg_conv4x4s2_c3_wgrad_bn_p(const float* y_nhwc, const float* saved, const float* gamma, const float* beta, int bn_act, const float* x_nchw,
                               float* dw, int N, int H, int W, int K, int prec, int accumulate, void* ws, size_t ws_bytes, dg_stream_t s);
int dg_conv4x4s2_c3_fwd_g(int groups, const float* const* x_nchw, const float* const* w, float* const* y_nhwc, int N, int H, int W, int K,
                          int act, float slope, int prec, dg_stream_t s);
int dg_conv4x4s2_c3_dgrad_g(int groups, const float* const* dy_nhwc, const float* const* w, float* const* dx_nchw, int N, int H, int W, int K,
                            int act, int prec, dg_stream_t s);
int dg_conv4x4s2_c3_wgrad_g(int groups, int share, const float* const* dy_nhwc, const float* const* act_out_nhwc, int act, float slope,
                            const float* const* x_nchw, float* const* dw, int N, int H, int W, int K, int prec, int accumulate,
                            void* const* ws, size_t ws_bytes, dg_stream_t s);

size_t dg_bn_workspace_bytes(int M, int C);
int dg_bn_train_stats(const float* y, int M, int C, float eps, float momentum,
                      float* running_mean, float* running_var, int64_t* num_batches_tracked,
                      float* saved, void* ws, size_t ws_bytes, dg_stream_t s);
size_t dg_bn_partials_workspace_bytes(int P, int C);
int dg_bn_stats_from_partials(const float* stat, int P, int M, int C, float eps, float momentum,
                              float* running_mean, float* running_var, int64_t* num_batches_tracked,
                              float* saved, void* ws, size_t ws_bytes, dg_stream_t s);
int dg_bn_act_fwd(const float* y, float* z, int M, int C, const float* saved, const float* gamma,
                  const float* beta, int act, float slope, dg_stream_t s);
int dg_bn_act_bwd(const float* dz, const float* y, float* dy, int M, int C, const float* saved,
                  const float* gamma, const float* beta, int act, float slope,
                  float* dgamma, float* dbeta, int accumulate, void* ws, size_t ws_bytes, dg_stream_t s);

int dg_bn_train_stats_g(int groups, int share, const float* const* y, int M, int C, float eps, float momentum, float* const* running_mean,
                        float* const* running_var, int64_t* const* num_batches_tracked, float* const* saved, void* const* ws, size_t ws_bytes,
                        dg_stream_t s);
int dg_bn_act_fwd_g(int groups, const float* const* y, float* const* z, int M, int C, const float* const* saved, const float* const* gamma,
                    const float* const* beta, int act, float slope, dg_stream_t s);
int dg_bn_act_bwd_g(int groups, int share, const float* const* dz, const float* const* y, float* const* dy, int M, int C,
                    const float* const* saved, const float* const* gamma, const float* const* beta, int act, float slope,
                    float* const* dgamma, float* const* dbeta, int accumulate, void* const* ws, size_t ws_bytes, dg_stream_t s);

int dg_act_fwd(const float* x, float* y, size_t n, int act, float slope, dg_stream_t s);
int dg_act_bwd(const float* dy, const float* out, float* dx, size_t n, int act, float slope, dg_stream_t s);
int dg_act_fwd_g(int groups, const float* const* x, float* const* y, size_t n, int act, float slope, dg_stream_t s);
int dg_act_bwd_g(int groups, const float* const* dy, const float* const* out, float* const* dx, size_t n, int act, float slope, dg_stream_t s);

size_t dg_loss_workspace_bytes(void);
int dg_mse_fwd(const float* x, const float* t, size_t n, float* loss, void* ws, size_t ws_bytes, dg_stream_t s);
int dg_mse_bwd(const float* x, const float* t, size_t n, const float* gout, float* dx, dg_stream_t s);
int dg_bce_fwd(const float* p, int n, float label, float* loss, void* ws, size_t ws_bytes, dg_stream_t s);
int dg_bce_bwd(const float* p, int n, float label, const float* gout, float* dp, dg_stream_t s);
size_t dg_fm_workspace_bytes(int N, size_t J);
int dg_fm_fwd(const float* real, const float* fake, int N, size_t J, float* diff, float* loss,
              void* ws, size_t ws_bytes, dg_stream_t s);
int dg_fm_bwd(const float* diff, int N, size_t J, const float* gout, float* dreal, float* dfake, dg_stream_t s);
int dg_mse_fwd_g(int groups, const float* const* x, const float* const* t, size_t n, float* const* loss, void* const* ws, size_t ws_bytes, dg_stream_t s);
int dg_mse_bwd_g(int groups, const float* const* x, const float* const* t, size_t n, const float* const* gout, float* const* dx, dg_stream_t s);
int dg_bce_fwd_g(int groups, const float* const* p, int n, const float* label, float* const* loss, dg_stream_t s);
int dg_bce_bwd_g(int groups, const float* const* p, int n, const float* label, const float* const* gout, float* const* dp, dg_stream_t s);
int dg_fm_fwd_g(int groups, const float* const* real, const float* const* fake, int N, size_t J, float* const* diff, float* const* loss,
                void* const* ws, size_t ws_bytes, dg_stream_t s);
int dg_fm_bwd_g(int groups, const float* const* diff, int N, size_t J, const float* const* gout, float* const* dreal, float* const* dfake,
                dg_stream_t s);

int dg_debug_igemm_stamps(void* buf, size_t bytes);

int dg_device_cu_count(void);

int dg_loss_mix_fwd(const float* lossvec, float* out8, int nfm, float rate, int arch, dg_stream_t s);
int dg_loss_mix_bwd(const float* gout, float* gvec, int nfm, float rate, int arch, int which, dg_stream_t s);

int dg_adam_advance(double* state, double lr, double beta1, double beta2, dg_stream_t s);
int dg_adam_step_flat(float* p, const float* g, float* m, float* v, size_t n, const double* state,
                      float beta1, float beta2, float eps, float weight_decay, float grad_scale,
                      dg_stream_t s);
int dg_ema_update_flat(float* ema, const float* p, size_t n, float w, dg_stream_t s);
int dg_swap_flat(float* a, float* b, size_t n, dg_stream_t s);

size_t dg_grad_stats_workspace_bytes(void);
int dg_grad_sumsq_partial(const float* g, size_t n, double* ws, size_t ws_bytes, int slot0, int* slots_used, dg_stream_t s);
int dg_grad_clip_finalize(const double* ws, int slots, double pre_scale, double max_norm, int guard, double* ctl, dg_stream_t s);
int dg_adam_advance_c(double* state, double lr, double beta1, double beta2, const double* ctl, dg_stream_t s);
int dg_adam_step_flat_c(float* p, const float* g, float* m, float* v, size_t n, const double* state,
                        float beta1, float beta2, float eps, float weight_decay, const double* ctl,
                        void* out, int form, size_t plane_elems, dg_stream_t s);

int dg_bce_target_fwd(const float* p, const float* target, int n, float* loss, dg_stream_t s);
int dg_bce_target_bwd(const float* p, const float* target, int n, const float* gout, float* dp, dg_stream_t s);
int dg_hinge_fwd(const float* x, const float* y, size_t n, float margin, float* loss, void* ws, size_t ws_bytes, dg_stream_t s);
int dg_hinge_bwd(const float* x, const float* y, size_t n, float margin, const float* gout, float* dx, dg_stream_t s);

int dg_dp_ready(int* device_out );
int dg_dp_unique_id_bytes(void);
int dg_dp_get_unique_id(void* id_out_host, size_t bytes);
int dg_dp_init(int rank, int world, const void* unique_id_host, size_t bytes);
int dg_dp_world_size(void);
int dg_dp_rank(void);
int dg_dp_allreduce_sum(float* buf, size_t n, dg_stream_t stream);
int dg_dp_allreduce_max(float* buf, size_t n, dg_stream_t stream);
int dg_dp_broadcast(float* buf, size_t n, int root, dg_stream_t stream);
int dg_dp_barrier(float* scratch1 , dg_stream_t stream);
int dg_dp_destroy(void);

int dg_u8hwc_to_f32chw(const uint8_t* src, float* dst, int N, int H, int W, int bgr, dg_stream_t s);
int dg_image_prep(const uint8_t* src, float* dst, int N, int H, int W, int x0, int cw, int erode, int mode, int S, dg_stream_t s);
int dg_sample_grid_u8(const float* const* src, int cols, int rows, int S, int gap, int bg, uint8_t* canvas, dg_stream_t s);
size_t dg_image_metrics_workspace_bytes(int n, int S);
int dg_image_metrics(const float* x, const float* y, int n, int S, float* out , void* ws, size_t ws_bytes, dg_stream_t s);

int dg_adam_step_flat_bf16(float* p, const float* g, float* m, float* v, size_t n, const double* state,
                           float beta1, float beta2, float eps, float weight_decay, float grad_scale,
                           void* p_bf16, dg_stream_t s);
int dg_f32_to_bf16(const float* x, void* y_bf16, size_t n, dg_stream_t s);
int dg_bn_act_fwd_bf16(const float* y, float* z, void* z_bf16, int M, int C, const float* saved, const float* gamma,
                       const float* beta, int act, float slope, dg_stream_t stream);
int dg_bn_act_bwd_bf16(const float* dz, const float* y, float* dy, void* dy_bf16, int M, int C, const float* saved,
                       const float* gamma, const float* beta, int act, float slope, float* dgamma, float* dbeta,
                       int accumulate, void* ws, size_t ws_bytes, dg_stream_t stream);
int dg_conv_bf16_operands_ok(int op, int N, int H, int W, int C, int K, int stride, int pad);
int dg_conv_mixed_bnstats_rows(int op, int N, int H, int W, int C, int K, int stride, int pad, int a_bf16, int b_bf16);
int dg_conv_fwd_mixed(const void* x, int x_bf16, const void* w, int w_bf16, void* y, int y_bf16, int N, int H, int W, int C, int K,
                      int stride, int pad, float* stat, size_t stat_floats, void* ws, size_t ws_bytes, dg_stream_t stream);
int dg_conv_dgrad_mixed(const void* dy, int dy_bf16, const void* w, int w_bf16, void* dx, int dx_bf16, int N, int H, int W, int C, int K,
                        int stride, int pad, float* stat, size_t stat_floats, void* ws, size_t ws_bytes, dg_stream_t stream);
int dg_conv_wgrad_mixed(const void* dy, int dy_bf16, const void* x, int x_bf16, float* dw, int N, int H, int W, int C, int K,
                        int stride, int pad, int accumulate, void* ws, size_t ws_bytes, dg_stream_t stream);

int dg_f32_to_bf16x3(const float* x, void* y_planes, size_t n, size_t plane_elems, dg_stream_t s);
int dg_adam_step_flat_x3(float* p, const float* g, float* m, float* v, size_t n, const double* state,
                         float beta1, float beta2, float eps, float weight_decay, float grad_scale,
                         void* p_planes, size_t plane_elems, dg_stream_t s);
int dg_x3_transpose_planes(const void* src_planes, void* dst_planes, size_t plane_elems, const int64_t* w_off, const int* w_K,
                           const int* w_J, int n, dg_stream_t s);
int dg_bn_act_fwd_x3(const float* y, float* z, void* z_planes, size_t plane_elems, int plane_layout, int M, int C, const float* saved,
                     const float* gamma, const float* beta, int act, float slope, dg_stream_t stream);
int dg_bn_act_bwd_x3(const float* dz, const float* y, float* dy, void* dy_planes, size_t plane_elems, int plane_layout, int M, int C,
                     const float* saved, const float* gamma, const float* beta, int act, float slope, float* dgamma,
                     float* dbeta, int accumulate, void* ws, size_t ws_bytes, dg_stream_t stream);
int dg_conv4x4s2_c3_fwd_x3(const float* x_nchw, const float* w, float* y_nhwc, void* y_planes, size_t plane_elems, int N, int H, int W,
                           int K, int act, float slope, dg_stream_t stream);
int dg_conv_x3_planes_ok(int op, int N, int H, int W, int C, int K, int stride, int pad);
int dg_conv_x3_bnstats_rows(int op, int N, int H, int W, int C, int K, int stride, int pad);
int dg_conv_fwd_x3(const void* x_planes, int64_t x_plane, const void* w_planes, int64_t w_plane, int w_transposed, float* y,
                   int N, int H, int W, int C, int K, int stride, int pad, float* stat, size_t stat_floats, void* ws, size_t ws_bytes,
                   dg_stream_t stream);
int dg_conv_dgrad_x3(const void* dy_planes, int64_t dy_plane, int dy_layout, const void* w_planes, int64_t w_plane, float* dx, int N, int H, int W,
                     int C, int K, int stride, int pad, float* stat, size_t stat_floats, void* ws, size_t ws_bytes, dg_stream_t stream);
int dg_conv_wgrad_x3(const void* dy_planes, int64_t dy_plane, int dy_layout, const void* x_planes, int64_t x_plane, float* dw, int N, int H, int W,
                     int C, int K, int stride, int pad, int accumulate, void* ws, size_t ws_bytes, dg_stream_t stream);

int dg_bn_train_stats_t(const void* y, int io_bf16, int M, int C, float eps, float momentum, float* running_mean,
                        float* running_var, int64_t* num_batches_tracked, float* saved, void* ws, size_t ws_bytes,
                        dg_stream_t stream);
int dg_bn_act_fwd_t(const void* y, void* z, int io_bf16, int M, int C, const float* saved, const float* gamma,
                    const float* beta, int act, float slope, dg_stream_t stream);
int dg_bn_act_bwd_t(const void* dz, const void* y, void* dy, int io_bf16, int M, int C, const float* saved,
                    const float* gamma, const float* beta, int act, float slope, float* dgamma, float* dbeta,
                    int accumulate, void* ws, size_t ws_bytes, dg_stream_t stream);
int dg_act_bwd_t(const void* dy, const void* out, void* dx, int io_bf16, size_t n, int act, float slope, dg_stream_t stream);
int dg_conv4x4s2_c3_fwd_t(const float* x_nchw, const float* w, void* y_nhwc, int y_bf16, int N, int H, int W, int K,
                          int act, float slope, dg_stream_t s);
int dg_conv4x4s2_c3_dgrad_t(const void* dy_nhwc, int dy_bf16, const float* w, float* dx_nchw, int N, int H, int W, int K,
                            int act, void* ws, size_t ws_bytes, dg_stream_t s);
int dg_conv4x4s2_c3_wgrad_t(const void* dy_nhwc, const void* act_out_nhwc , int io_bf16, int act,
                            float slope, const float* x_nchw, float* dw, int N, int H, int W, int K, int accumulate,
                            void* ws, size_t ws_bytes, dg_stream_t s);
int dg_fm_fwd_t(const void* real, const void* fake, int io_bf16, int N, size_t J, float* diff, float* loss, void* ws,
                size_t ws_bytes, dg_stream_t stream);
int dg_fm_bwd_t(const float* diff, int N, size_t J, const float* gout, void* dreal, void* dfake, int io_bf16, dg_stream_t stream);

int dg_nchw_to_nhwc(const float* x, float* y, int N, int C, int H, int W, dg_stream_t s);
int dg_nhwc_to_nchw(const float* x, float* y, int N, int C, int H, int W, dg_stream_t s);

#ifdef __cplusplus
}
#endif
#endif
```

Measured before the change: 294.5 images/s.

## Fuse Adam step with x3 plane split and weight transpose; lazy grad zeroing

Adds a grouped Adam kernel that updates tiled conv weights and writes both the three bf16 planes and their transposed copy in one pass through shared memory. Remaining parameters are handled by a multi-range Adam launch, which replaces the per-range flat Adam calls and the separate transpose pass. Separately, zero_grad becomes lazy: the first wgrad writes into a gradient with accumulate off instead of adding onto a zeroed buffer, and grads that are never written are zeroed only when needed. This removes a full gradient memset and a re-read of the planes, at the cost of more bookkeeping state that can go stale and leave gradients unzeroed.

```diff
diff --git a/discogan_modernized_amd/_lib.py b/discogan_modernized_amd/_lib.py
--- a/discogan_modernized_amd/_lib.py
+++ b/discogan_modernized_amd/_lib.py
@@ -139,6 +139,7 @@
     "dg_conv_x3_bnstats_rows": (_i, [_i, _i, _i, _i, _i, _i, _i, _i]),
     "dg_conv_fwd_x3": (_i, [_p, _l, _p, _l, _i, _p, _i, _i, _i, _i, _i, _i, _i, _p, _z, _p, _z, _p]),
     "dg_x3_transpose_planes": (_i, [_p, _p, _z, _p, _p, _p, _i, _p]),
+    "dg_adam_step_group_x3": (_i, [_p, _p, _p, _p, _z, _p, _f, _f, _f, _f, _f, _p, _p, _p, _z, _p, _p, _p, _i, _p, _p, _i, _p]),
     "dg_conv_dgrad_x3": (_i, [_p, _l, _i, _p, _l, _p, _i, _i, _i, _i, _i, _i, _i, _p, _z, _p, _z, _p]),
     "dg_conv_wgrad_x3": (_i, [_p, _l, _i, _p, _l, _p, _i, _i, _i, _i, _i, _i, _i, _i, _p, _z, _p]),
     "dg_conv_mixed_bnstats_rows": (_i, [_i, _i, _i, _i, _i, _i, _i, _i, _i, _i]),
diff --git a/discogan_modernized_amd/csrc/igemm_dma_x3.hip b/discogan_modernized_amd/csrc/igemm_dma_x3.hip
--- a/discogan_modernized_amd/csrc/igemm_dma_x3.hip
+++ b/discogan_modernized_amd/csrc/igemm_dma_x3.hip
@@ -11,7 +11,7 @@
 __device__ __forceinline__ void dg_x3_static_for(std::integer_sequence<int, Q...>, F&& f) {
     (f(std::integral_constant<int, Q>{}), ...);
 }
-#define DG_X3T_MAX 48
+#include "x3_table.h"
 constexpr int G16_I[24] = {0, 0, 0, 1, 1, 1, 2, 2, 2, 3, 3, 3, 4, 4, 4, 5, 5, 5, 6, 7, 6, 6, 7, 7};
 constexpr int G16_T[24] = {0, 1, 2, 0, 1, 2, 0, 1, 2, 0, 1, 2, 0, 1, 2, 0, 1, 2, 0, 0, 1, 2, 1, 2};
 
@@ -602,12 +602,6 @@
     return 0;
 }
 
-struct X3TransposeTable {
-    int n;
-    int tile0[DG_X3T_MAX + 1];
-    int K[DG_X3T_MAX], J[DG_X3T_MAX];
-    long off[DG_X3T_MAX];
-};
 __global__ __launch_bounds__(256) void x3_transpose_kernel(const __bf16* __restrict__ src, __bf16* __restrict__ dst, long plane, X3TransposeTable t) {
     __shared__ unsigned tile[64][33];
     typedef unsigned u32x4 __attribute__((ext_vector_type(4)));
diff --git a/discogan_modernized_amd/csrc/optim.hip b/discogan_modernized_amd/csrc/optim.hip
--- a/discogan_modernized_amd/csrc/optim.hip
+++ b/discogan_modernized_amd/csrc/optim.hip
@@ -19,24 +19,15 @@
     p = p - step_size * (m / denom);
 }
 template <int P16>
-__global__ __launch_bounds__(256) void adam_step_kernel(float* __restrict__ p, const float* __restrict__ g,
-                                                        float* __restrict__ m, float* __restrict__ v, long n,
-                                                        const double* __restrict__ state, float b1, float b2, float eps,
-                                                        float wd, float gscale, __bf16* __restrict__ p16, long pstride,
-                                                        const double* __restrict__ ctl) {
-    if (ctl != nullptr) {
-        if (ctl[3] != 0.0) return;
-        gscale = (float)ctl[2];
-    }
-    const float step_size = (float)state[1];
-    const float bc2_sqrt = (float)state[2];
-    const float omb1 = 1.f - b1, omb2 = 1.f - b2;
+__device__ __forceinline__ void adam_range(float* __restrict__ p, const float* __restrict__ g, float* __restrict__ m,
+                                           float* __restrict__ v, long n, float step_size, float bc2_sqrt, float omb1, float b2, float omb2,
+                                           float eps, float wd, float gscale, __bf16* __restrict__ p16, long pstride, long bid, long nb) {
     const long n4 = n >> 2;
-    long i0 = (long)blockIdx.x * 256 + threadIdx.x;
+    long i0 = bid * 256 + threadIdx.x;
     if constexpr (P16 == 3) {
         typedef __bf16 bf16x8_a __attribute__((ext_vector_type(8)));
         const long n8 = (((size_t)p16 | (size_t)(pstride * 2)) & 15) == 0 ? n >> 3 : 0;
-        for (long i = i0; i < n8; i += (long)gridDim.x * 256) {
+        for (long i = i0; i < n8; i += nb * 256) {
             f32x4 pp[2], gg[2], mm[2], vv[2];
 #pragma unroll
             for (int h = 0; h < 2; ++h) {
@@ -65,7 +56,7 @@
         }
         i0 += n8 * 2;
     }
-    for (long i = i0; i < n4; i += (long)gridDim.x * 256) {
+    for (long i = i0; i < n4; i += nb * 256) {
         f32x4 pp = *(const f32x4*)(p + i * 4);
         const f32x4 gg = *(const f32x4*)(g + i * 4);
         f32x4 mm = *(const f32x4*)(m + i * 4);
@@ -88,7 +79,7 @@
             *(dg_bf16x4_t*)(p16 + 2 * pstride + i * 4) = l;
         }
     }
-    if (blockIdx.x == 0 && threadIdx.x == 0) {
+    if (bid == 0 && threadIdx.x == 0) {
         for (long e = n4 * 4; e < n; ++e) {
             float a = p[e], b = m[e], c = v[e];
             adam_one(a, g[e], b, c, gscale, wd, omb1, b2, omb2, bc2_sqrt, eps, step_size);
@@ -104,6 +95,20 @@
             }
         }
     }
+}
+
+template <int P16>
+__global__ __launch_bounds__(256) void adam_step_kernel(float* __restrict__ p, const float* __restrict__ g,
+                                                        float* __restrict__ m, float* __restrict__ v, long n,
+                                                        const double* __restrict__ state, float b1, float b2, float eps,
+                                                        float wd, float gscale, __bf16* __restrict__ p16, long pstride,
+                                                        const double* __restrict__ ctl) {
+    if (ctl != nullptr) {
+        if (ctl[3] != 0.0) return;
+        gscale = (float)ctl[2];
+    }
+    adam_range<P16>(p, g, m, v, n, (float)state[1], (float)state[2], 1.f - b1, b2, 1.f - b2, eps, wd, gscale, p16, pstride, (long)blockIdx.x,
+                    (long)gridDim.x);
 }
 
 extern "C" int dg_adam_advance(double* state, double lr, double beta1, double beta2, dg_stream_t stream) {
@@ -380,3 +385,181 @@
     DG_CHECK_LAUNCH("adam_step_c");
     return DG_OK;
 }
+
+#include "x3_table.h"
+template <int TJ>
+__global__ __launch_bounds__(4 * TJ) void adam_step_x3t_kernel(float* __restrict__ p, const float* __restrict__ g, float* __restrict__ m,
+                                                            float* __restrict__ v, const double* __restrict__ state, float b1, float b2,
+                                                            float eps, float wd, float gscale, __bf16* __restrict__ p3,
+                                                            __bf16* __restrict__ p3t, long plane, const double* __restrict__ ctl,
+                                                            X3TransposeTable t) {
+    constexpr int TPR = TJ / 16;
+    __shared__ unsigned tile[3][64][TJ / 2 + 1];
+    typedef __bf16 bf16x8_a __attribute__((ext_vector_type(8)));
+    if (ctl != nullptr) {
+        if (ctl[3] != 0.0) return;
+        gscale = (float)ctl[2];
+    }
+    const float step_size = (float)state[1];
+    const float bc2_sqrt = (float)state[2];
+    const float omb1 = 1.f - b1, omb2 = 1.f - b2;
+    int wi = 0;
+    while (wi + 1 < t.n && (int)blockIdx.x >= t.tile0[wi + 1]) ++wi;
+    const int K = t.K[wi], J = t.J[wi];
+    const long base = t.off[wi];
+    const int tj = J / TJ;
+    const int b = blockIdx.x - t.tile0[wi];
+    const int k0 = (b / tj) * 64, j0 = (b % tj) * TJ;
+    const int lk = threadIdx.x / TPR, lv = threadIdx.x % TPR;
+    const int sq = threadIdx.x & 7, sjp = threadIdx.x >> 3;
+    f32x4 pp[2][2], gg[2][2], mm[2][2], vv[2][2];
+#pragma unroll
+    for (int h = 0; h < 2; ++h) {
+        const long e = base + (long)(k0 + lk) * J + j0 + (lv + TPR * h) * 8;
+#pragma unroll
+        for (int q = 0; q < 2; ++q) {
+            pp[h][q] = *(const f32x4*)(p + e + 4 * q);
+            gg[h][q] = *(const f32x4*)(g + e + 4 * q);
+            mm[h][q] = *(const f32x4*)(m + e + 4 * q);
+            vv[h][q] = *(const f32x4*)(v + e + 4 * q);
+        }
+    }
+#pragma unroll
+    for (int h = 0; h < 2; ++h) {
+        const long e = base + (long)(k0 + lk) * J + j0 + (lv + TPR * h) * 8;
+        dg_bf16x4_t hh[2], md[2], ll[2];
+#pragma unroll
+        for (int q = 0; q < 2; ++q) {
+#pragma unroll
+            for (int j = 0; j < 4; ++j) {
+                float a = pp[h][q][j], bb = mm[h][q][j], c = vv[h][q][j];
+                adam_one(a, gg[h][q][j], bb, c, gscale, wd, omb1, b2, omb2, bc2_sqrt, eps, step_size);
+                pp[h][q][j] = a; mm[h][q][j] = bb; vv[h][q][j] = c;
+            }
+            *(f32x4*)(p + e + 4 * q) = pp[h][q];
+            *(f32x4*)(m + e + 4 * q) = mm[h][q];
+            *(f32x4*)(v + e + 4 * q) = vv[h][q];
+            dg_split3(pp[h][q], hh[q], md[q], ll[q]);
+        }
+        const bf16x8_a pl3[3] = {__builtin_shufflevector(hh[0], hh[1], 0, 1, 2, 3, 4, 5, 6, 7),
+                                 __builtin_shufflevector(md[0], md[1], 0, 1, 2, 3, 4, 5, 6, 7),
+                                 __builtin_shufflevector(ll[0], ll[1], 0, 1, 2, 3, 4, 5, 6, 7)};
+#pragma unroll
+        for (int pl = 0; pl < 3; ++pl) {
+            *(bf16x8_a*)(p3 + pl * plane + e) = pl3[pl];
+            const u32x4 w = __builtin_bit_cast(u32x4, pl3[pl]);
+#pragma unroll
+            for (int i = 0; i < 4; ++i) tile[pl][lk][(lv + TPR * h) * 4 + i] = w[i];
+        }
+    }
+    __syncthreads();
+#pragma unroll
+    for (int pl = 0; pl < 3; ++pl) {
+        unsigned w[8];
+#pragma unroll
+        for (int i = 0; i < 8; ++i) w[i] = tile[pl][8 * sq + i][sjp];
+        u32x4 lo, hi;
+#pragma unroll
+        for (int i = 0; i < 4; ++i) {
+            lo[i] = (w[2 * i] & 0xffffu) | (w[2 * i + 1] << 16);
+            hi[i] = (w[2 * i] >> 16) | (w[2 * i + 1] & 0xffff0000u);
+        }
+        unsigned short* d = (unsigned short*)p3t + pl * plane + base + (long)(j0 + 2 * sjp) * K + k0 + 8 * sq;
+        *(u32x4*)d = lo;
+        *(u32x4*)(d + K) = hi;
+    }
+}
+
+#define DG_ADAM_RANGES_MAX 64
+struct AdamRangeTable {
+    int n;
+    int blk0[DG_ADAM_RANGES_MAX + 1];
+    long off[DG_ADAM_RANGES_MAX], len[DG_ADAM_RANGES_MAX];
+};
+__global__ __launch_bounds__(256) void adam_step_ranges_x3_kernel(float* __restrict__ p, const float* __restrict__ g, float* __restrict__ m,
+                                                                  float* __restrict__ v, const double* __restrict__ state, float b1,
+                                                                  float b2, float eps, float wd, float gscale, __bf16* __restrict__ p3,
+                                                                  long plane, const double* __restrict__ ctl, AdamRangeTable t) {
+    if (ctl != nullptr) {
+        if (ctl[3] != 0.0) return;
+        gscale = (float)ctl[2];
+    }
+    int ri = 0;
+    while (ri + 1 < t.n && (int)blockIdx.x >= t.blk0[ri + 1]) ++ri;
+    const long o = t.off[ri];
+    adam_range<3>(p + o, g + o, m + o, v + o, t.len[ri], (float)state[1], (float)state[2], 1.f - b1, b2, 1.f - b2, eps, wd, gscale, p3 + o,
+                  plane, (long)(blockIdx.x - t.blk0[ri]), (long)(t.blk0[ri + 1] - t.blk0[ri]));
+}
+
+extern "C" int dg_adam_step_group_x3(float* p, const float* g, float* m, float* v, size_t numel, const double* state, float beta1,
+                                     float beta2, float eps, float weight_decay, float grad_scale, const double* ctl, void* p_planes,
+                                     void* pt_planes, size_t plane_elems, const int64_t* w_off, const int* w_K, const int* w_J, int n_w,
+                                     const int64_t* r_off, const int64_t* r_len, int n_r, dg_stream_t stream) {
+    DG_CHECK_ARG(p && g && m && v && state && p_planes, "dg_adam_step_group_x3: null pointer");
+    DG_CHECK_ARG(n_w >= 0 && n_r >= 0 && (n_w == 0 || (pt_planes && w_off && w_K && w_J)) && (n_r == 0 || (r_off && r_len)),
+                 "dg_adam_step_group_x3: %d weights, %d ranges, or a null table", n_w, n_r);
+    DG_CHECK_ARG(plane_elems >= numel && plane_elems % 8 == 0, "dg_adam_step_group_x3: plane distance %zu for %zu parameters", plane_elems,
+                 numel);
+    DG_CHECK_ARG((((size_t)p | (size_t)g | (size_t)m | (size_t)v | (size_t)p_planes | (size_t)pt_planes) & 15) == 0,
+                 "dg_adam_step_group_x3: buffers must be 16-byte aligned");
+    int64_t end = 0;
+    for (int i = 0; i < n_w; ++i) {
+        const int K = w_K[i], J = w_J[i];
+        DG_CHECK_ARG(K >= 64 && J >= 64 && K % 64 == 0 && J % 64 == 0 && w_off[i] % 8 == 0 && w_off[i] >= end &&
+                         (size_t)(w_off[i] + (int64_t)K * J) <= numel,
+                     "dg_adam_step_group_x3: weight %d (K=%d, J=%d, offset %ld): K and J multiples of 64, offset a multiple of 8, ascending, "
+                     "inside %zu parameters", i, K, J, (long)w_off[i], numel);
+        end = w_off[i] + (int64_t)K * J;
+    }
+    end = 0;
+    for (int i = 0; i < n_r; ++i) {
+        DG_CHECK_ARG(r_len[i] >= 0 && r_off[i] % 8 == 0 && r_off[i] >= end && (size_t)(r_off[i] + r_len[i]) <= numel,
+                     "dg_adam_step_group_x3: range %d (offset %ld, %ld parameters): offset a multiple of 8, ascending, inside %zu parameters", i,
+                     (long)r_off[i], (long)r_len[i], numel);
+        end = r_off[i] + r_len[i];
+    }
+    const hipStream_t s = (hipStream_t)stream;
+    for (int TJ = 128; TJ >= 64; TJ -= 64) {
+        X3TransposeTable t;
+        t.n = 0;
+        long tiles = 0;
+        for (int i = 0; i <= n_w; ++i) {
+            if (i < n_w && (w_J[i] % 128 == 0) == (TJ == 128)) {
+                t.tile0[t.n] = (int)tiles;
+                t.K[t.n] = w_K[i]; t.J[t.n] = w_J[i]; t.off[t.n] = w_off[i];
+                tiles += (long)(w_K[i] / 64) * (w_J[i] / TJ);
+                ++t.n;
+            }
+            if (t.n == 0 || (i < n_w && t.n < DG_X3T_MAX)) continue;
+            DG_CHECK_ARG(tiles <= 0x7fffffffL, "dg_adam_step_group_x3: %ld tiles in one launch", tiles);
+            t.tile0[t.n] = (int)tiles;
+            if (TJ == 128)
+                hipLaunchKernelGGL(adam_step_x3t_kernel<128>, dim3((unsigned)tiles), dim3(512), 0, s, p, g, m, v, state, beta1, beta2, eps,
+                                   weight_decay, grad_scale, (__bf16*)p_planes, (__bf16*)pt_planes, (long)plane_elems, ctl, t);
+            else
+                hipLaunchKernelGGL(adam_step_x3t_kernel<64>, dim3((unsigned)tiles), dim3(256), 0, s, p, g, m, v, state, beta1, beta2, eps,
+                                   weight_decay, grad_scale, (__bf16*)p_planes, (__bf16*)pt_planes, (long)plane_elems, ctl, t);
+            DG_CHECK_LAUNCH("adam_step_x3t");
+            t.n = 0;
+            tiles = 0;
+        }
+    }
+    for (int i0 = 0; i0 < n_r; i0 += DG_ADAM_RANGES_MAX) {
+        AdamRangeTable t;
+        t.n = 0;
+        int blocks = 0;
+        for (int i = i0; i < n_r && t.n < DG_ADAM_RANGES_MAX; ++i) {
+            if (r_len[i] == 0) continue;
+            t.blk0[t.n] = blocks;
+            t.off[t.n] = r_off[i]; t.len[t.n] = r_len[i];
+            blocks += flat_grid((size_t)r_len[i] / 2);
+            ++t.n;
+        }
+        if (t.n == 0) continue;
+        t.blk0[t.n] = blocks;
+        hipLaunchKernelGGL(adam_step_ranges_x3_kernel, dim3(blocks), dim3(256), 0, s, p, g, m, v, state, beta1, beta2, eps, weight_decay,
+                           grad_scale, (__bf16*)p_planes, (long)plane_elems, ctl, t);
+        DG_CHECK_LAUNCH("adam_step_ranges_x3");
+    }
+    return DG_OK;
+}
diff --git a/discogan_modernized_amd/csrc/x3_table.h b/discogan_modernized_amd/csrc/x3_table.h
--- /dev/null
+++ b/discogan_modernized_amd/csrc/x3_table.h
@@ -0,0 +1,8 @@
+#pragma once
+#define DG_X3T_MAX 48
+struct X3TransposeTable {
+    int n;
+    int tile0[DG_X3T_MAX + 1];
+    int K[DG_X3T_MAX], J[DG_X3T_MAX];
+    long off[DG_X3T_MAX];
+};
diff --git a/discogan_modernized_amd/functional.py b/discogan_modernized_amd/functional.py
--- a/discogan_modernized_amd/functional.py
+++ b/discogan_modernized_amd/functional.py
@@ -27,11 +27,30 @@
 FUSE_C3_DGRAD_ACT = __import__("os").environ.get("DG_FUSE_C3_DGRAD_ACT", "1") != "0"
 
 
-def _flat_grad_of(param):
+def _flat_grad_of(param, contiguous=False):
     fg = getattr(param, "_dg_flat_grad", None)
-    if fg is not None and param.grad is fg:
-        return fg
-    return None
+    if fg is None or param.grad is not fg:
+        return None, True
+    fresh = getattr(param, "_dg_grad_unwritten", False)
+    if fresh:
+        param._dg_grad_unwritten = False
+    if contiguous and not fg.is_contiguous():
+        if fresh:
+            fg.zero_()
+        return None, True
+    return fg, not fresh
+
+
+def _flat_grad_pair(pa, pb):
+    (fa, acc_a), (fb, acc_b) = _flat_grad_of(pa), _flat_grad_of(pb)
+    if fa is None or fb is None:
+        for f, acc in ((fa, acc_a), (fb, acc_b)):
+            if f is not None and not acc:
+                f.zero_()
+        return None, None, True
+    if acc_a != acc_b:
+        (fb if acc_a else fa).zero_()
+    return fa, fb, acc_a or acc_b
 
 
 FINAL_PASS = False
@@ -88,9 +107,9 @@
     wg = (x, dy) if transposed else (dy, x)
     dw = None
     if ctx.needs_input_grad[1]:
-        fg = _flat_grad_of(w)
+        fg, acc = _flat_grad_of(w)
         if fg is not None:
-            ops.conv_wgrad(*wg, stride, pad, out=fg, accumulate=True)
+            ops.conv_wgrad(*wg, stride, pad, out=fg, accumulate=acc)
             _final(ctx.final, w)
         else:
             dw = ops.conv_wgrad(*wg, stride, pad)
@@ -148,9 +167,9 @@
             dx = ops.c3_dgrad(g, w, ops.ACT_NONE, act_out=y, in_act=act, slope=slope) if fuse else ops.c3_dgrad(g, w, ops.ACT_NONE)
         dw = None
         if ctx.needs_input_grad[1]:
-            fg = _flat_grad_of(ctx.wref)
-            if fg is not None and fg.is_contiguous():
-                ops.c3_wgrad(g, x, out=fg, accumulate=True, **fuse)
+            fg, acc = _flat_grad_of(ctx.wref, contiguous=True)
+            if fg is not None:
+                ops.c3_wgrad(g, x, out=fg, accumulate=acc, **fuse)
                 _final(ctx.final, ctx.wref)
             else:
                 dw = ops.c3_wgrad(g, x, **fuse)
@@ -176,9 +195,9 @@
         dx = ops.c3_fwd(g, w, ops.ACT_NONE) if ctx.needs_input_grad[0] else None
         dw = None
         if ctx.needs_input_grad[1]:
-            fg = _flat_grad_of(ctx.wref)
-            if fg is not None and fg.is_contiguous():
-                ops.c3_wgrad(x, g, out=fg, accumulate=True)
+            fg, acc = _flat_grad_of(ctx.wref, contiguous=True)
+            if fg is not None:
+                ops.c3_wgrad(x, g, out=fg, accumulate=acc)
                 _final(ctx.final, ctx.wref)
             else:
                 dw = ops.c3_wgrad(x, g)
@@ -216,9 +235,10 @@
         if not training:
             raise RuntimeError("BatchNormActFn: backward in eval mode is not supported")
         need_p = ctx.needs_input_grad[1] or ctx.needs_input_grad[2]
-        fg, fb = _flat_grad_of(ctx.prefs[0]), _flat_grad_of(ctx.prefs[1])
-        if need_p and fg is not None and fb is not None:
-            dy, _, _ = ops.bn_act_bwd(dz, y, saved, gamma, beta, act, slope, out_grads=(fg, fb), planes_cm=ctx.dy_cm, planes_only=ctx.dy_po)
+        fg, fb, acc = _flat_grad_pair(ctx.prefs[0], ctx.prefs[1]) if need_p else (None, None, True)
+        if fg is not None:
+            dy, _, _ = ops.bn_act_bwd(dz, y, saved, gamma, beta, act, slope, out_grads=(fg, fb), planes_cm=ctx.dy_cm, planes_only=ctx.dy_po,
+                                      accumulate=acc)
             _final(ctx.final, ctx.prefs[0], ctx.prefs[1])
             return (dy,) + (None,) * 15
         dy, dgamma, dbeta = ops.bn_act_bwd(dz, y, saved, gamma, beta, act, slope, need_param_grads=need_p, planes_cm=ctx.dy_cm,
@@ -253,17 +273,18 @@
         dz = ops.c3_fwd(g, w, ops.ACT_NONE) if ctx.needs_input_grad[0] or need_p else None
         dw = None
         if ctx.needs_input_grad[11]:
-            fg = _flat_grad_of(ctx.wref)
-            if fg is not None and fg.is_contiguous():
-                ops.c3_wgrad_bn(y, saved, gamma, beta, g, out=fg, accumulate=True, bn_act=bn_act)
+            fg, acc = _flat_grad_of(ctx.wref, contiguous=True)
+            if fg is not None:
+                ops.c3_wgrad_bn(y, saved, gamma, beta, g, out=fg, accumulate=acc, bn_act=bn_act)
                 _final(ctx.final, ctx.wref)
             else:
                 dw = ops.c3_wgrad_bn(y, saved, gamma, beta, g, bn_act=bn_act)
         if dz is None:
             return none[:11] + (dw,) + none[12:]
-        fgm, fb = _flat_grad_of(ctx.prefs[0]), _flat_grad_of(ctx.prefs[1])
-        if need_p and fgm is not None and fb is not None:
-            dy, _, _ = ops.bn_act_bwd(dz, y, saved, gamma, beta, bn_act, 0.0, out_grads=(fgm, fb), planes_cm=dy_cm, planes_only=dy_po)
+        fgm, fb, acc = _flat_grad_pair(ctx.prefs[0], ctx.prefs[1]) if need_p else (None, None, True)
+        if fgm is not None:
+            dy, _, _ = ops.bn_act_bwd(dz, y, saved, gamma, beta, bn_act, 0.0, out_grads=(fgm, fb), planes_cm=dy_cm, planes_only=dy_po,
+                                      accumulate=acc)
             _final(ctx.final, ctx.prefs[0], ctx.prefs[1])
             return (dy,) + none[1:11] + (dw,) + none[12:]
         dy, dgamma, dbeta = ops.bn_act_bwd(dz, y, saved, gamma, beta, bn_act, 0.0, need_param_grads=need_p, planes_cm=dy_cm, planes_only=dy_po)
@@ -396,9 +417,14 @@
 
 
 def _flat_grads_of(params):
-    fgs = [_flat_grad_of(p) for p in params]
-    if any(f is None for f in fgs):
-        raise RuntimeError("grouped launches need parameters whose .grad is the optimiser's flat gradient view (optim.Adam)")
+    fgs = []
+    for p in params:
+        fg, acc = _flat_grad_of(p)
+        if fg is None:
+            raise RuntimeError("grouped launches need parameters whose .grad is the optimiser's flat gradient view (optim.Adam)")
+        if not acc:
+            fg.zero_()
+        fgs.append(fg)
     return fgs
 
 
diff --git a/discogan_modernized_amd/model.py b/discogan_modernized_amd/model.py
--- a/discogan_modernized_amd/model.py
+++ b/discogan_modernized_amd/model.py
@@ -46,6 +46,7 @@
             if flat is not None:
                 flat.zero_()
                 p.grad = flat
+                p._dg_grad_unwritten = False
             elif p.grad is not None:
                 if set_to_none:
                     p.grad = None
diff --git a/discogan_modernized_amd/ops.py b/discogan_modernized_amd/ops.py
--- a/discogan_modernized_amd/ops.py
+++ b/discogan_modernized_amd/ops.py
@@ -808,7 +808,8 @@
     return _bn_publish(form, z, extra, cm, po)
 
 
-def bn_act_bwd(dz, y, saved, gamma, beta, act, slope=0.2, need_param_grads=True, out_grads=None, planes_cm=False, planes_only=False):
+def bn_act_bwd(dz, y, saved, gamma, beta, act, slope=0.2, need_param_grads=True, out_grads=None, planes_cm=False, planes_only=False,
+               accumulate=True):
     _check_dev(dz, y, allow16=True)
     dz = as_nhwc(dz)
     y = as_nhwc(y)
@@ -817,7 +818,7 @@
     acc = 0
     if out_grads is not None:
         dgamma, dbeta = out_grads
-        acc = 1
+        acc = int(bool(accumulate))
     else:
         dgamma = torch.empty(c, device=y.device, dtype=torch.float32) if need_param_grads else None
         dbeta = torch.empty(c, device=y.device, dtype=torch.float32) if need_param_grads else None
@@ -1017,6 +1018,32 @@
                                                  eps, weight_decay, grad_scale, _stream()), "dg_adam_step_flat")
 
 
+ADAM_FUSED_T = _env_flag("DG_ADAM_FUSED_T", True)
+LAZY_ZERO_GRAD = _env_flag("DG_LAZY_ZERO_GRAD", True)
+
+
+def adam_group_x3_table(weights, ranges):
+    import ctypes as C
+    nw, nr = len(weights), len(ranges)
+    return (nw, (C.c_int64 * max(nw, 1))(*[w[0] for w in weights]), (C.c_int * max(nw, 1))(*[w[1] for w in weights]),
+            (C.c_int * max(nw, 1))(*[w[2] for w in weights]),
+            nr, (C.c_int64 * max(nr, 1))(*[r[0] for r in ranges]), (C.c_int64 * max(nr, 1))(*[r[1] - r[0] for r in ranges]))
+
+
+def adam_step_group_x3(p, g, m, v, state, beta1, beta2, eps, weight_decay, grad_scale, p3, p3t, table, ctl=None):
+    _check_dev(p, g, m, v)
+    if ctl is not None:
+        _check_ctl(ctl, "adam_step_group_x3")
+    nw, w_off, w_k, w_j, nr, r_off, r_len = table
+    assert p3.shape == (3, p.numel()) and p3.stride(1) == 1 and (nw == 0 or (p3t.shape == p3.shape and p3t.stride(0) == p3.stride(0)))
+    nbytes = 40.0 * sum(int(w_k[i]) * int(w_j[i]) for i in range(nw)) + 34.0 * sum(int(r_len[i]) for i in range(nr))
+    with _hbm("adam", nbytes):
+        _lib.check(_lib.load().dg_adam_step_group_x3(_ptr(p), _ptr(g), _ptr(m), _ptr(v), p.numel(), _ptr(state), beta1, beta2, eps,
+                                                     weight_decay, grad_scale, _ptr(ctl), _ptr(p3), _ptr(p3t) if nw else None,
+                                                     p3.stride(0), w_off, w_k, w_j, nw, r_off, r_len, nr, _stream()),
+                   "dg_adam_step_group_x3")
+
+
 GRAD_STATS_MAX_GRID = 4096
 
 
diff --git a/discogan_modernized_amd/optim.py b/discogan_modernized_amd/optim.py
--- a/discogan_modernized_amd/optim.py
+++ b/discogan_modernized_amd/optim.py
@@ -31,6 +31,7 @@
         self.state = torch.zeros(4, device=dev, dtype=torch.float64)
         self.offsets = offs
         self.ctl = None
+        self._unwritten = False
         with torch.no_grad():
             for p, off in zip(self.params, offs):
                 n = p.numel()
@@ -59,6 +60,19 @@
                  if p.dim() == 4 and tuple(p.shape[2:]) == (4, 4) and p.shape[0] > 1 and ops.is_krsc(p)]
         self.flat_p3t = torch.zeros((3, self.numel), device=self.flat_p.device, dtype=torch.bfloat16) if convs else None
         self._x3t_table = ops.x3_transpose_table(convs)
+        tiled = [c for c in convs if c[1] % 64 == 0 and c[2] % 64 == 0 and c[0] % 8 == 0]
+        tiled_offs = {c[0] for c in tiled}
+        rest = []
+        for p, off in zip(self.params, self.offsets):
+            if off in tiled_offs:
+                continue
+            end = off + (p.numel() + _ALIGN - 1) // _ALIGN * _ALIGN
+            if rest and rest[-1][1] == off:
+                rest[-1][1] = end
+            else:
+                rest.append([off, end])
+        self._adam_group_table = ops.adam_group_x3_table(tiled, rest)
+        self._x3t_rest_table = ops.x3_transpose_table([c for c in convs if c[0] not in tiled_offs])
         conv_offs = {c[0] for c in convs}
         for p, off in zip(self.params, self.offsets):
             p._dg_x3 = (self.flat_p3, off, self.flat_p3t if off in conv_offs else None)
@@ -90,20 +104,47 @@
             if self.flat_p3t is not None:
                 ops.x3_transpose_planes(self.flat_p3, self.flat_p3t, self._x3t_table)
 
-    def zero_grad(self, set_to_none: bool = True):
-        self.flat_g.zero_()
+    def zero_grad(self, set_to_none: bool = True, lazy: bool = False):
+        if lazy and ops.LAZY_ZERO_GRAD:
+            self._unwritten = True
+        else:
+            self.flat_g.zero_()
+            self._unwritten = False
         for p in self.params:
+            p._dg_grad_unwritten = self._unwritten
             if p.grad is not p._dg_flat_grad:
                 p.grad = p._dg_flat_grad
+
+    def fill_unwritten_grads(self, ranges=None):
+        if not self._unwritten:
+            return
+        runs = []
+        for p, off in zip(self.params, self.offsets):
+            if not getattr(p, "_dg_grad_unwritten", False):
+                continue
+            end = off + (p.numel() + _ALIGN - 1) // _ALIGN * _ALIGN
+            if ranges is not None and not any(b <= off and end <= e for b, e in ranges):
+                continue
+            p._dg_grad_unwritten = False
+            if runs and runs[-1][1] == off:
+                runs[-1][1] = end
+            else:
+                runs.append([off, end])
+        for b, e in runs:
+            self.flat_g[b:e].zero_()
+        if ranges is None:
+            self._unwritten = False
 
     def _sync_foreign_grads(self):
         for p in self.params:
             if p.grad is None:
                 p._dg_flat_grad.zero_()
                 p.grad = p._dg_flat_grad
+                p._dg_grad_unwritten = False
             elif p.grad is not p._dg_flat_grad and p.grad.data_ptr() != p._dg_flat_grad.data_ptr():
                 p._dg_flat_grad.copy_(p.grad)
                 p.grad = p._dg_flat_grad
+                p._dg_grad_unwritten = False
 
     def ranges_of(self, modules):
         ids = {id(p) for m in modules for p in m.parameters()}
@@ -121,6 +162,7 @@
     def step(self, grad_scale: float = 1.0, active=None):
         g = self.param_groups[0]
         self._sync_foreign_grads()
+        self.fill_unwritten_grads()
         ranges = active if active is not None else [(0, self.numel)]
         ctl = self.ctl
         if ctl is not None:
@@ -131,6 +173,13 @@
         ops.adam_advance(self.state, float(g["lr"]), float(g["betas"][0]), float(g["betas"][1]), ctl=ctl)
         p16 = getattr(self, "flat_p16", None)
         p3 = getattr(self, "flat_p3", None)
+        if p3 is not None and active is None and ops.ADAM_FUSED_T:
+            ops.adam_step_group_x3(self.flat_p, self.flat_g, self.exp_avg, self.exp_avg_sq, self.state, float(g["betas"][0]),
+                                   float(g["betas"][1]), float(g["eps"]), float(g["weight_decay"]), float(grad_scale), p3,
+                                   self.flat_p3t, self._adam_group_table, ctl=ctl)
+            if self._x3t_rest_table[0]:
+                ops.x3_transpose_planes(p3, self.flat_p3t, self._x3t_rest_table)
+            return
         for b, e in ranges:
             ops.adam_step_flat(self.flat_p[b:e], self.flat_g[b:e], self.exp_avg[b:e], self.exp_avg_sq[b:e], self.state,
                                float(g["betas"][0]), float(g["betas"][1]), float(g["eps"]), float(g["weight_decay"]),
diff --git a/discogan_modernized_amd/trainer.py b/discogan_modernized_amd/trainer.py
--- a/discogan_modernized_amd/trainer.py
+++ b/discogan_modernized_amd/trainer.py
@@ -400,6 +400,7 @@
     def _exchange_and_step_ranges(self, opt, ranges, kind):
         from . import ops
         g = opt.param_groups[0]
+        opt.fill_unwritten_grads(ranges)
         for b, e in ranges:
             scale = 1.0
             if self.xg is not None:
@@ -420,10 +421,10 @@
         if self.skip_dead_work:
             if dstep and self._ev_dis_ready is not None and self._cap is None:
                 torch.cuda.current_stream(self.device).wait_event(self._ev_dis_ready)
-            (self.optim_dis if dstep else self.optim_gen).zero_grad()
+            (self.optim_dis if dstep else self.optim_gen).zero_grad(lazy=True)
         else:
-            self.optim_gen.zero_grad()
-            self.optim_dis.zero_grad()
+            self.optim_gen.zero_grad(lazy=not dstep)
+            self.optim_dis.zero_grad(lazy=dstep)
         from . import ops as _ops
         self.ctx.prec = {"f32": _ops.PREC_F32, "bf16": _ops.PREC_BF16, "f32x3": _ops.PREC_F32X3}[self.mfma_dtype]
         self.ctx.shadow, self.ctx.act16, self.ctx.x3 = bool(self.bf16_shadow), self.act_dtype == "bf16", bool(self.x3_planes)
@@ -489,6 +490,7 @@
     def _exchange(self, opt, kind):
         if self.xg is None:
             return 1.0
+        opt.fill_unwritten_grads()
         if self.time_comm:
             e0, e1 = torch.cuda.Event(enable_timing=True), torch.cuda.Event(enable_timing=True)
             e0.record()
@@ -522,6 +524,8 @@
             return out
         if do_step:
             self.apply_step(iters)
+        else:
+            opt.fill_unwritten_grads()
         return out
 
     def apply_step(self, iters):
@@ -562,6 +566,7 @@
         else:
             out = self._fwd_bwd(A, B, iters, need_losses)
         if not do_step:
+            opt.fill_unwritten_grads()
             return out
         if dstep or not self._dec_done:
             self.apply_step(iters)
@@ -820,6 +825,7 @@
     def finish(self):
         tr = self.tr
         main = torch.cuda.current_stream(tr.device)
+        self.opt.fill_unwritten_grads()
         for b in self.buckets:
             if not b["done"]:
                 self._launch(b, main, early=False, active=self.active)
diff --git a/include/discogan_hip.h b/include/discogan_hip.h
--- a/include/discogan_hip.h
+++ b/include/discogan_hip.h
@@ -243,6 +243,10 @@
                          void* p_planes, size_t plane_elems, dg_stream_t s);
 int dg_x3_transpose_planes(const void* src_planes, void* dst_planes, size_t plane_elems, const int64_t* w_off, const int* w_K,
                            const int* w_J, int n, dg_stream_t s);
+int dg_adam_step_group_x3(float* p, const float* g, float* m, float* v, size_t numel, const double* state, float beta1, float beta2,
+                          float eps, float weight_decay, float grad_scale, const double* ctl, void* p_planes, void* pt_planes,
+                          size_t plane_elems, const int64_t* w_off, const int* w_K, const int* w_J, int n_w, const int64_t* r_off,
+                          const int64_t* r_len, int n_r, dg_stream_t s);
 int dg_bn_act_fwd_x3(const float* y, float* z, void* z_planes, size_t plane_elems, int plane_layout, int M, int C, const float* saved,
                      const float* gamma, const float* beta, int act, float slope, dg_stream_t stream);
 int dg_bn_act_bwd_x3(const float* dz, const float* y, float* dy, void* dy_planes, size_t plane_elems, int plane_layout, int M, int C,
```

Result: faster. 297.8 images/s, median of 6 (+1.1%).
